# MundyRepo/MuNDy

Hardware: AMD Instinct MI355X
Metric: timesteps/sec, 10^6 spherocylinders, frictionless LCP contact (BBPGD) (higher is better)
Workload: dtype f64; 1 GPU; configs[2]: 1M spherocylinders r=0.5 L=2 at 40% volume fraction, random packing, AABB+0.1 neighbour list, frictionless LCP tol 1e-05; bodies_per_gpu=1000000, bodies_total=1000000, contacts_per_gpu=7621833, contacts_total=7621833, parallelism=single GPU (N > 1: the same system, hilbert domain decomposition with RCCL halo)

## Files before the change

include/mundy_hip.h:

```cpp
#ifndef MUNDY_HIP_H_
#define MUNDY_HIP_H_

#include <stddef.h>
#include <stdint.h>

#ifdef __cplusplus
extern "C" {
#endif

typedef void* mhip_stream_t;

enum {
  MHIP_SUCCESS = 0,
  MHIP_ERR_INVALID_ARGUMENT = 1,
  MHIP_ERR_LOGIC = 2,
  MHIP_ERR_RUNTIME = 3,
  MHIP_ERR_HIP = 4,
  MHIP_ERR_NO_DEVICE = 5
};

const char* mhip_last_error(void);
int mhip_version(void);
int mhip_set_tracing(int enable);
int mhip_device_info(int* device_count, char* arch_name, size_t arch_name_len);
// ... 105 lines not shown
                                mhip_stream_t stream);
int mhip_crosslinkers_renumber(mhip_crosslinkers_t handle, const int32_t* new_of_old, mhip_stream_t stream);
int mhip_crosslinkers_destroy(mhip_crosslinkers_t handle);

#define MHIP_PERIPHERY_SPHERE 0
#define MHIP_PERIPHERY_ELLIPSOID 1
#define MHIP_PERIPHERY_ELLIPSOID_FAST 2
typedef struct mhip_periphery {
  int shape;
  double center[3];
  double quat[4];
  double radii[3];
  double k;
} mhip_periphery;
int mhip_periphery_force(const mhip_periphery* periphery, size_t n, const double* center, const double* radius,
                         double* force, int accumulate, int* colliding ,
                         double* max_overlap , mhip_stream_t stream);

typedef struct mhip_active_springs* mhip_active_springs_t;
int mhip_active_springs_create(mhip_active_springs_t* handle, size_t n, size_t m, const int32_t* pairs ,
                               double sigma, double kon, double koff, const uint64_t* keys ,
                               const uint64_t* counters , mhip_stream_t stream);
int mhip_active_springs_sample(mhip_active_springs_t handle, int* switches , mhip_stream_t stream);
int mhip_active_springs_force(mhip_active_springs_t handle, const double* center, double* force, int accumulate,
                              int* active , mhip_stream_t stream);
int mhip_active_springs_advance(mhip_active_springs_t handle, double dt, mhip_stream_t stream);
int mhip_active_springs_get_state(mhip_active_springs_t handle, int32_t* state, double* next_time, double* elapsed,
                                  uint64_t* counters, mhip_stream_t stream);
int mhip_active_springs_set_state(mhip_active_springs_t handle, const int32_t* state, const double* next_time,
                                  const double* elapsed, const uint64_t* counters, mhip_stream_t stream);
int mhip_active_springs_renumber(mhip_active_springs_t handle, const int32_t* new_of_old, mhip_stream_t stream);
int mhip_active_springs_destroy(mhip_active_springs_t handle);

int mhip_compute_aabb_mixed(size_t n, const int32_t* kind, const double* center, const double* quat,
                            const double* shape, double* aabb, double* bounding_radius, mhip_stream_t stream);
int mhip_compute_aabb_mixed_conservative(size_t n, const int32_t* kind, const double* center, const double* quat,
                                         const double* shape, double* aabb, double* bounding_radius,
                                         mhip_stream_t stream);
int mhip_contact_mixed(size_t c, const int32_t* pairs, const int32_t* kind, const double* center, const double* quat,
                       const double* shape, double* sep, double* normal, double* cp1, double* cp2, double* ra,
                       double* rb, size_t* class_counts , mhip_stream_t stream);
int mhip_contact_mixed_set_contraction(int on);
int mhip_contact_mixed_set_sphere_ellipsoid_route(int route);
int mhip_contact_mixed_last_evaluations(unsigned long long evaluations[3] , mhip_stream_t stream);
int mhip_ellipsoid_last_evaluations(unsigned long long* evaluations , mhip_stream_t stream);
int mhip_contact_mixed_periodic(size_t c, const int32_t* pairs, const int32_t* kind, const double* center,
                                const double* quat, const double* shape, const double* box , double* sep,
                                double* normal, double* cp1, double* cp2, double* ra, double* rb,
                                size_t* class_counts , mhip_stream_t stream);

enum { MHIP_SEARCH_SPHERES = 0, MHIP_SEARCH_AABB = 1 };
enum { MHIP_SEARCH_METHOD_AUTO = 0, MHIP_SEARCH_METHOD_GRID = 1, MHIP_SEARCH_METHOD_MORTON_LBVH = 2 };

typedef struct mhip_broadphase* mhip_broadphase_t;

typedef struct {
  int search_kind;
  int symmetric;
  double buffer;
  int periodic;
  double box[3];
  int method;
  int include_self;
  double cell[9];
} mhip_broadphase_config;

int mhip_broadphase_create(mhip_broadphase_t* handle);
int mhip_broadphase_destroy(mhip_broadphase_t handle);
int mhip_broadphase_build(mhip_broadphase_t handle, const mhip_broadphase_config* config , size_t n,
                          const double* aabb, const double* center, const double* bounding_radius,
                          size_t* num_pairs , mhip_stream_t stream);
int mhip_broadphase_get_pairs(mhip_broadphase_t handle, int32_t* pairs, int32_t* row_ptr, int32_t* col,
                              mhip_stream_t stream);
int mhip_broadphase_set_sets(mhip_broadphase_t handle, size_t n, const unsigned char* is_source,
                             const unsigned char* is_target, mhip_stream_t stream);
int mhip_broadphase_set_exclusions(mhip_broadphase_t handle, size_t n, const int32_t* ex_ptr, const int32_t* ex_idx,
                                   size_t num_entries, mhip_stream_t stream);
int mhip_broadphase_set_identities(mhip_broadphase_t handle, size_t n, const uint64_t* entity_id,
                                   const int32_t* owner_rank, mhip_stream_t stream);
int mhip_broadphase_get_ident_pairs(mhip_broadphase_t handle, uint64_t* source_id, int32_t* source_proc,
                                    uint64_t* target_id, int32_t* target_proc, mhip_stream_t stream);
int mhip_broadphase_method_used(mhip_broadphase_t handle, int* method );
int mhip_broadphase_minimum_image_complete(mhip_broadphase_t handle, int* complete );
int mhip_links_export_coo(mhip_broadphase_t handle, uint64_t first_link_id, int source_rank, int target_rank,
                          uint64_t* link_id, uint64_t* linked_entity_ids, unsigned char* linked_entity_ranks,
                          mhip_stream_t stream);
int mhip_links_export_crs(mhip_broadphase_t handle, uint64_t first_link_id, unsigned bucket_capacity,
                          unsigned* num_connected_links, unsigned* sparse_connectivity_offsets,
                          uint64_t* sparse_connectivity, uint64_t* bucket_begin, mhip_stream_t stream);
int mhip_broadphase_needs_rebuild(mhip_broadphase_t handle, size_t n, const double* center, int* flag ,
                                  mhip_stream_t stream);

enum { MHIP_SPACE_UNCONSTRAINED = 0, MHIP_SPACE_LOWER_BOUND = 1, MHIP_SPACE_UPPER_BOUND = 2, MHIP_SPACE_BOUNDED = 3 };
enum { MHIP_RESIDUAL_PROJECTED_DIFF = 0, MHIP_RESIDUAL_PROJECTED_GRADIENT = 1 };

typedef struct {
  int kind;
  double lower_bound, upper_bound;
} mhip_space;

typedef struct {
  unsigned max_iters;
  double tol;
  int residual_kind;
} mhip_pgd_config;

typedef struct {
  unsigned num_iters;
  double residual;
  int converged;
} mhip_solve_result;

int mhip_deep_copy(size_t n, double* dst, const double* src, mhip_stream_t stream);
int mhip_fill(size_t n, double* dst, double value, mhip_stream_t stream);
int mhip_axpby(size_t n, double alpha, const double* x, double beta, double* y, mhip_stream_t stream);
int mhip_wrapped_axpbyz(size_t n, double alpha, const double* x, double beta, const double* y, double* z,
                        const mhip_space* space , mhip_stream_t stream);
int mhip_diff_dot2(size_t n, const double* x, const double* y, double* result , mhip_stream_t stream);
int mhip_diff_dot4(size_t n, const double* x1, const double* x2, const double* y1, const double* y2,
                   double* result , mhip_stream_t stream);
int mhip_residual(size_t n, int residual_kind, const double* x, const double* grad, const mhip_space* space ,
                  double* result , mhip_stream_t stream);
int mhip_bb_step(size_t n, const double* x_old, const double* g_old, const double* x, const double* g,
                 double* result , mhip_stream_t stream);
int mhip_gemv(size_t n, const double* A, const double* x, double* y, mhip_stream_t stream);

typedef struct mhip_contact_op* mhip_contact_op_t;

int mhip_contact_op_create(mhip_contact_op_t* handle, size_t num_constraints, size_t num_bodies, const int32_t* pairs,
                           const double* normal, const double* ra, const double* rb, const double* mob_trans,
                           const double* mob_rot, double dt, const double* priority, mhip_stream_t stream);
int mhip_contact_op_create_rods(mhip_contact_op_t* handle, size_t num_constraints, size_t num_bodies,
                                const int32_t* pairs, const double* normal, const double* arc_s, const double* arc_t,
                                const double* seg, const double* mob_trans, const double* mob_rot, double dt,
                                const double* priority, mhip_stream_t stream);
int mhip_contact_op_refresh(mhip_contact_op_t handle, const double* normal, const double* ra, const double* rb,
                            mhip_stream_t stream);
int mhip_contact_op_refresh_rods(mhip_contact_op_t handle, const double* normal, const double* arc_s,
                                 const double* arc_t, const double* seg, mhip_stream_t stream);
int mhip_contact_op_destroy(mhip_contact_op_t handle);
int mhip_release_cached_workspaces(void);
int mhip_contact_op_apply(mhip_contact_op_t handle, const double* x, double* y, mhip_stream_t stream);
int mhip_contact_op_body_sweep(mhip_contact_op_t handle, const double* x, mhip_stream_t stream);
int mhip_contact_op_body_sweep_vector(mhip_contact_op_t handle, const double* force, mhip_stream_t stream);
int mhip_contact_op_constraint_rate(mhip_contact_op_t handle, const double* velocity, double* sep_dot,
                                    mhip_stream_t stream);
int mhip_contact_op_sizes(mhip_contact_op_t handle, size_t* num_constraints, size_t* num_bodies);
int mhip_contact_op_set_work_mapping(mhip_contact_op_t handle, int xcd_tile, int lanes_per_body);
int mhip_contact_op_set_drift_source(mhip_contact_op_t op, int source);
int mhip_contact_op_get_drift_source(mhip_contact_op_t op, int* source );
int mhip_contact_op_set_tiering(mhip_contact_op_t handle, int mode);
int mhip_contact_op_tier_stats(mhip_contact_op_t handle, size_t* tiered_iterations, double* mean_hot_fraction,
                               size_t* renumberings, size_t* wakeups);
int mhip_contact_op_set_profiling(mhip_contact_op_t handle, int enable);
int mhip_contact_op_get_profile(mhip_contact_op_t handle, double* body_ms, double* constraint_ms, size_t* iterations);
int mhip_contact_op_body_velocity(mhip_contact_op_t handle, const double** velocity );

int mhip_bbpgd_solve_dense(size_t n, const double* A, const double* q, const mhip_space* space ,
                           const mhip_pgd_config* config , double* x, double* g, double* x_tmp,
                           double* g_tmp, mhip_solve_result* result , mhip_stream_t stream);
int mhip_bbpgd_solve_contact(mhip_contact_op_t op, const double* q, const mhip_space* space ,
                             const mhip_pgd_config* config , double* x, double* g, double* x_tmp,
                             double* g_tmp, mhip_solve_result* result , mhip_stream_t stream);

int mhip_bbpgd_solve_contact_friction(mhip_contact_op_t op, const double* sep, double mu,
                                      const mhip_pgd_config* config , double* p, double* g,
                                      mhip_solve_result* result , mhip_stream_t stream);
int mhip_apgd_solve_contact_friction(mhip_contact_op_t op, const double* sep, double mu,
                                      const mhip_pgd_config* config , double* p, double* g,
                                      mhip_solve_result* result , mhip_stream_t stream);
#define MHIP_BBPGD_REDUCTION_WIDTH 5
int mhip_contact_op_set_partition(mhip_contact_op_t handle, size_t body_first, size_t body_count,
                                  const unsigned char* counted_contacts, double* velocity);
int mhip_bbpgd_stage_begin(mhip_contact_op_t op, const double* q, const mhip_space* space ,
                           const mhip_pgd_config* config , double* x, double* g, double* x_tmp,
                           double* g_tmp, mhip_stream_t stream);
int mhip_bbpgd_stage_body(mhip_contact_op_t op, int init, mhip_stream_t stream);
int mhip_bbpgd_stage_constraint(mhip_contact_op_t op, int init, double* local, mhip_stream_t stream);
int mhip_bbpgd_stage_constraint_range(mhip_contact_op_t op, int init, size_t c_first, size_t c_count,
                                      mhip_stream_t stream);
int mhip_bbpgd_stage_reduce(mhip_contact_op_t op, int init, double* local, mhip_stream_t stream);
int mhip_bbpgd_stage_finalize(mhip_contact_op_t op, int init, const double* gathered, int nparts,
                              mhip_stream_t stream);
int mhip_bbpgd_stage_poll(mhip_contact_op_t op, mhip_solve_result* result , int* done ,
                          mhip_stream_t stream);
int mhip_bbpgd_stage_snapshot_active(mhip_contact_op_t op, mhip_stream_t stream);
int mhip_bbpgd_stage_end(mhip_contact_op_t op, mhip_solve_result* result , mhip_stream_t stream);
int mhip_solve_small_cqpp_batch(size_t batch, int n, const double* A, const double* q,
                                const mhip_space* space , const mhip_pgd_config* config ,
                                double* x, double* grad, unsigned* num_iters, double* residual, int* converged,
                                mhip_stream_t stream);
int mhip_scrap_bbpgd_solve_contact(mhip_contact_op_t op, const double* sep, double max_allowable_overlap,
                                   unsigned max_iterations, double* lam, double* lam_tmp, double* g, double* g_tmp,
                                   mhip_solve_result* result , double* max_speed ,
                                   mhip_stream_t stream);
int mhip_bbpgd_solve_contact_unfused(mhip_contact_op_t op, const double* q, const mhip_space* space ,
                                     const mhip_pgd_config* config , double* x, double* g, double* x_tmp,
                                     double* g_tmp, mhip_solve_result* result , mhip_stream_t stream);

int mhip_select_contacts(size_t c, const double* sep, double cutoff, int32_t* kept_index, size_t* count_out ,
                         mhip_stream_t stream);
int mhip_filter_pairs_owned(size_t c, const int32_t* pairs_in, size_t first, size_t count, int32_t* pairs_out,
                            unsigned char* counted_out, size_t* count_out , mhip_stream_t stream);
int mhip_partition_pairs_owned(size_t c, const int32_t* pairs_in, size_t first, size_t count, int32_t* pairs_out,
                               unsigned char* counted_out, size_t* interior_out ,
                               size_t* count_out , mhip_stream_t stream);
int mhip_select_aabb_overlap(size_t n, const double* aabb, double buffer, const double* box6 ,
                             int32_t* idx_out, size_t* count_out , mhip_stream_t stream);
int mhip_aabb_chunk_bounds(size_t n, const double* aabb, double buffer, int nchunks, double* boxes,
                           mhip_stream_t stream);
int mhip_select_aabb_overlap_any(size_t n, const double* aabb, double buffer, int nboxes, const double* boxes,
                                 int32_t* idx_out, size_t* count_out , mhip_stream_t stream);
int mhip_aabb_bounds(size_t n, const double* aabb, double buffer, double* out6 , mhip_stream_t stream);

int mhip_integrate_euler(size_t n, double dt, const double* velocity, double* center, double* quat,
                         mhip_stream_t stream);

int mhip_periodic_sep(size_t n, const double* box, const double* p1, const double* p2, double* out,
                      mhip_stream_t stream);
int mhip_wrap_rigid(size_t n, const double* box, double* center, mhip_stream_t stream);

int mhip_unit_cell_inverse(const double* cell, double* cell_inv);
int mhip_periodic_sep_triclinic(size_t n, const double* cell, const double* p1, const double* p2, double* out,
                                mhip_stream_t stream);
int mhip_wrap_rigid_triclinic(size_t n, const double* cell, double* center, mhip_stream_t stream);
int mhip_shift_image_triclinic(size_t n, const double* cell, const double* p, const int32_t* images, double* out,
                               mhip_stream_t stream);
int mhip_contact_spheres_triclinic(size_t c, const int32_t* pairs, const double* center, const double* radius,
                                   const double* cell, double* sep, double* normal, mhip_stream_t stream);

int mhip_morton_order(size_t n, const double* center, const double* lo , double cell_size, int32_t* perm,
                      mhip_stream_t stream);
int mhip_curve_order(size_t n, const double* center, const double* lo , const double* hi ,
                     int level, const int32_t* key_table, int32_t* perm, mhip_stream_t stream);
int mhip_curve_keys(size_t n, const double* center, const double* lo , const double* hi ,
                    int level, const int32_t* key_table, uint32_t* keys, mhip_stream_t stream);
int mhip_sort_by_key_u64(size_t n, const uint64_t* keys, int32_t* perm, mhip_stream_t stream);
int mhip_gather_rows(size_t n, size_t width, const int32_t* perm, const double* src, double* dst, mhip_stream_t stream);
int mhip_copy_strided(size_t n, size_t width, const double* src, size_t src_stride, double* dst, size_t dst_stride,
                      mhip_stream_t stream);


typedef struct mhip_comm* mhip_comm_t;
#define MHIP_COMM_ID_BYTES 128
typedef int (*mhip_comm_exchange_fn)(void* user, int nsend, const int* send_peer, const double* const* send_buf,
                                     const size_t* send_count, int nrecv, const int* recv_peer, double* const* recv_buf,
                                     const size_t* recv_count);
typedef int (*mhip_comm_all_gather_fn)(void* user, const double* send, size_t count, double* recv );

int mhip_comm_unique_id(unsigned char* id );
int mhip_comm_create_rccl(mhip_comm_t* comm, const unsigned char* id , int rank, int world);
int mhip_comm_create_host(mhip_comm_t* comm, int rank, int world, mhip_comm_exchange_fn exchange,
                          mhip_comm_all_gather_fn all_gather, void* user);
int mhip_comm_destroy(mhip_comm_t comm);
int mhip_comm_info(mhip_comm_t comm, int* rank, int* world, int* is_rccl);
int mhip_comm_mailbox_open(mhip_comm_t comm, int* opened , mhip_stream_t stream);
int mhip_comm_mailbox_close(mhip_comm_t comm);
int mhip_comm_halo_ipc_enable(mhip_comm_t comm, int on);
int mhip_comm_set_exchange_timeout(mhip_comm_t comm, double seconds);
int mhip_comm_inject_fault(mhip_comm_t comm, unsigned at_poll);
int mhip_comm_halo_ipc_active(mhip_comm_t comm, int* active );
int mhip_comm_all_gather(mhip_comm_t comm, const double* send, size_t count, double* recv, mhip_stream_t stream);
int mhip_comm_exchange_start(mhip_comm_t comm, int nsend, const int* send_peer, const double* const* send_buf,
                             const size_t* send_count, int nrecv, const int* recv_peer, double* const* recv_buf,
                             const size_t* recv_count, mhip_stream_t stream);
int mhip_comm_exchange_finish(mhip_comm_t comm, mhip_stream_t stream);

typedef struct mhip_velocity_halo {
  double* velocity;
  int num_send_peers;
  const int* send_peer;
  const size_t* send_rows;
  const int32_t* send_index;
  int num_recv_peers;
  const int* recv_peer;
  const size_t* recv_first_row;
  const size_t* recv_rows;
} mhip_velocity_halo;
typedef struct mhip_ghost_layout {
  size_t num_ghost_lo, num_owned, num_ghost_hi;
  size_t num_sent;
  mhip_velocity_halo halo;
} mhip_ghost_layout;
int mhip_ghost_layout_from_counts(int world, int rank, size_t n_owned, const size_t* counts ,
                                  size_t* num_ghost_lo, size_t* num_ghost_hi, int* num_send, int* send_peer,
                                  size_t* send_rows, int* num_recv, int* recv_peer, size_t* recv_first_row,
                                  size_t* recv_rows);
int mhip_ghost_plan(mhip_comm_t comm, size_t n, const double* aabb, double buffer,
                    mhip_ghost_layout* layout , mhip_stream_t stream);
int mhip_ghost_exchange(mhip_comm_t comm, size_t width, const double* records ,
                        double* local , mhip_stream_t stream);

int mhip_hilbert_key_table(int level, int32_t* table );
int mhip_body_work_weights(size_t c, const int32_t* pairs, size_t first, size_t count, double* weights ,
                           mhip_stream_t stream);
int mhip_compose_keys_u64(size_t n, const uint32_t* major, const double* minor, int shift, uint64_t* out,
                          mhip_stream_t stream);
int mhip_fill_sequence(size_t n, double first, double* dst, mhip_stream_t stream);
int mhip_curve_cut(mhip_comm_t comm, size_t n, const uint32_t* keys, const double* weights , size_t ncell,
                   int64_t* splitters , mhip_stream_t stream);
int mhip_migrate_plan(mhip_comm_t comm, size_t n, const uint32_t* keys, const int64_t* splitters ,
                      size_t* n_new, size_t* num_sent , size_t* num_received ,
                      mhip_stream_t stream);
int mhip_migrate_exchange(mhip_comm_t comm, size_t width, const double* records ,
                          double* out , mhip_stream_t stream);
typedef struct mhip_dist_profile {
// ... 20 lines not shown
```

mundy_amd/capi.py:

```python
import ctypes as C
import os

_HERE = os.path.dirname(os.path.abspath(__file__))
LIB_PATH = os.path.join(_HERE, "lib", "libmundy_hip.so")

SUCCESS, ERR_INVALID_ARGUMENT, ERR_LOGIC, ERR_RUNTIME, ERR_HIP, ERR_NO_DEVICE = range(6)
SEARCH_SPHERES, SEARCH_AABB = 0, 1
SEARCH_METHOD_AUTO, SEARCH_METHOD_GRID, SEARCH_METHOD_MORTON_LBVH = 0, 1, 2
SPACE_UNCONSTRAINED, SPACE_LOWER_BOUND, SPACE_UPPER_BOUND, SPACE_BOUNDED = 0, 1, 2, 3
RESIDUAL_PROJECTED_DIFF, RESIDUAL_PROJECTED_GRADIENT = 0, 1
SPRING_HOOKEAN, SPRING_FENE = 0, 1
PERIPHERY_SPHERE, PERIPHERY_ELLIPSOID, PERIPHERY_ELLIPSOID_FAST = 0, 1, 2


class MhipError(RuntimeError):
    """HIP runtime failure or missing device (MHIP_ERR_HIP / MHIP_ERR_NO_DEVICE)."""


class BroadphaseConfig(C.Structure):
    _fields_ = [("search_kind", C.c_int), ("symmetric", C.c_int), ("buffer", C.c_double), ("periodic", C.c_int),
                ("box", C.c_double * 3), ("method", C.c_int), ("include_self", C.c_int), ("cell", C.c_double * 9)]


class Space(C.Structure):
    _fields_ = [("kind", C.c_int), ("lower_bound", C.c_double), ("upper_bound", C.c_double)]


class PgdConfig(C.Structure):
    _fields_ = [("max_iters", C.c_uint), ("tol", C.c_double), ("residual_kind", C.c_int)]


class SolveResult(C.Structure):
    _fields_ = [("num_iters", C.c_uint), ("residual", C.c_double), ("converged", C.c_int)]


class HertzFrictionParams(C.Structure):
    _fields_ = [("mu", C.c_double), ("normal_damping", C.c_double), ("tangential_damping", C.c_double),
                ("density", C.c_double), ("dt", C.c_double)]


class Periphery(C.Structure):
    _fields_ = [("shape", C.c_int), ("center", C.c_double * 3), ("quat", C.c_double * 4), ("radii", C.c_double * 3),
                ("k", C.c_double)]


class VelocityHalo(C.Structure):
    _fields_ = [("velocity", C.c_void_p), ("num_send_peers", C.c_int), ("send_peer", C.POINTER(C.c_int)),
                ("send_rows", C.POINTER(C.c_size_t)), ("send_index", C.c_void_p), ("num_recv_peers", C.c_int),
                ("recv_peer", C.POINTER(C.c_int)), ("recv_first_row", C.POINTER(C.c_size_t)),
                ("recv_rows", C.POINTER(C.c_size_t))]


class GhostLayout(C.Structure):
    _fields_ = [("num_ghost_lo", C.c_size_t), ("num_owned", C.c_size_t), ("num_ghost_hi", C.c_size_t),
                ("num_sent", C.c_size_t), ("halo", VelocityHalo)]


class DistProfile(C.Structure):
    _fields_ = [("body_ms", C.c_double), ("constraint_ms", C.c_double), ("halo_wait_ms", C.c_double),
                ("timed_iterations", C.c_size_t), ("halo_post_ms", C.c_double), ("record_ms", C.c_double),
                ("halo_path", C.c_int), ("record_path", C.c_int)]


EXCHANGE_FN = C.CFUNCTYPE(C.c_int, C.c_void_p, C.c_int, C.POINTER(C.c_int), C.POINTER(C.c_void_p),
                          C.POINTER(C.c_size_t), C.c_int, C.POINTER(C.c_int), C.POINTER(C.c_void_p),
                          C.POINTER(C.c_size_t))
ALL_GATHER_FN = C.CFUNCTYPE(C.c_int, C.c_void_p, C.c_void_p, C.c_size_t, C.c_void_p)
COMM_ID_BYTES = 128

_vp, _sz, _d, _i = C.c_void_p, C.c_size_t, C.c_double, C.c_int

SIGNATURES = {
    "mhip_device_info": [C.POINTER(C.c_int), C.c_char_p, _sz],
    "mhip_malloc": [C.POINTER(_vp), _sz],
    "mhip_free": [_vp],
    "mhip_memcpy_h2d": [_vp, _vp, _sz, _vp],
    "mhip_memcpy_d2h": [_vp, _vp, _sz, _vp],
    "mhip_stream_synchronize": [_vp],
    "mhip_compute_aabb_spheres": [_sz, _vp, _vp, _vp, _vp],
    "mhip_compute_aabb_spherocylinders": [_sz, _vp, _vp, _vp, _vp, _vp, _vp],
    "mhip_compute_aabb_ellipsoids": [_sz, _vp, _vp, _vp, _vp, _vp],
    "mhip_compute_aabb_ellipsoids_conservative": [_sz, _vp, _vp, _vp, _vp, _vp],
    "mhip_compute_aabb_segments": [_sz, _vp, _vp, _vp],
    "mhip_bounding_radius_spherocylinders": [_sz, _vp, _vp, _vp, _vp],
    "mhip_bounding_radius_ellipsoids": [_sz, _vp, _vp, _vp],
    "mhip_spherocylinder_segments": [_sz, _vp, _vp, _vp, _vp, _vp, _vp],
    "mhip_distance_sphere_sphere": [_sz, _vp, _vp, _vp, _vp, _vp, _vp, _vp],
    "mhip_distance_point_segment": [_sz, _vp, _vp, _vp, _vp, _vp, _vp, _vp, _vp],
    "mhip_distance_point_sphere": [_sz, _vp, _vp, _vp, _vp, _vp, _vp],
    "mhip_distance_segment_sphere": [_sz] + [_vp] * 9,
    "mhip_distance_segment_segment": [_sz, _vp, _vp, _vp, _vp, _vp, _vp, _vp, _vp, _vp, _vp, _vp],
    "mhip_distance_ellipsoid_ellipsoid": [_sz] + [_vp] * 12,
    "mhip_distance_point_ellipsoid": [_sz] + [_vp] * 8,
    "mhip_contact_ellipsoids": [_sz] + [_vp] * 11,
    "mhip_compute_aabb_mixed": [_sz] + [_vp] * 7,
    "mhip_compute_aabb_mixed_conservative": [_sz] + [_vp] * 7,
    "mhip_contact_mixed": [_sz] + [_vp] * 11 + [C.POINTER(_sz), _vp],
    "mhip_contact_mixed_set_contraction": [_i],
    "mhip_contact_mixed_set_sphere_ellipsoid_route": [_i],
    "mhip_contact_mixed_last_evaluations": [C.POINTER(C.c_ulonglong), _vp],
    "mhip_ellipsoid_last_evaluations": [C.POINTER(C.c_ulonglong), _vp],
    "mhip_contact_mixed_periodic": [_sz] + [_vp] * 5 + [C.POINTER(_d)] + [_vp] * 6 + [C.POINTER(_sz), _vp],
    "mhip_contact_spherocylinders_periodic": [_sz, _vp, _vp, _vp, C.POINTER(_d)] + [_vp] * 9,
    "mhip_hertz_contact_force": [_sz, _sz, _vp, _vp, _vp, _vp, _d, _vp, _d, _vp, _vp, _vp],
    "mhip_hertz_friction_force": [_sz, _sz] + [_vp] * 8 + [_d, _vp, _d, _vp, C.POINTER(HertzFrictionParams), _vp, _vp, _vp,
                                  _vp],
    "mhip_contact_history_carry": [_sz, _vp, _vp, _vp, _sz, _sz, _vp, _vp, C.POINTER(_sz), _vp],
    "mhip_select_dividing": [_sz, _vp, _d, _vp, C.POINTER(_sz), _vp],
    "mhip_divide_grow_spherocylinders": [_sz, _sz, _vp, _d, _d, C.POINTER(_d), _vp, _vp, _vp, _vp, _vp],
    "mhip_aabb_moved": [_sz, _vp, _vp, _d, C.POINTER(_i), _vp],
    "mhip_springs_create": [C.POINTER(_vp), _sz, _sz, _vp, _i, _vp, _d, _vp, _d, _vp],
    "mhip_springs_force": [_vp, _vp, _vp, _vp, _vp, _vp],
    "mhip_springs_destroy": [_vp],
    "mhip_crosslinkers_create": [C.POINTER(_vp), _sz, _sz, _vp, _vp, _vp, _i, _d, _d, _d, _d, _d, _d, _vp],
    "mhip_crosslinkers_set_candidates": [_vp, _vp, _vp, _sz, _vp, _vp],
    "mhip_crosslinkers_kmc_step": [_vp, _vp, _d, _vp, _vp, _vp, _vp, _vp],
    "mhip_crosslinkers_force": [_vp, _vp, _vp, _i, _vp, _vp, _vp],
    "mhip_crosslinkers_get_state": [_vp, _vp, _vp, _vp],
    "mhip_crosslinkers_set_state": [_vp, _vp, _vp, _vp],
    "mhip_crosslinkers_renumber": [_vp, _vp, _vp],
    "mhip_crosslinkers_destroy": [_vp],
    "mhip_periphery_force": [C.POINTER(Periphery), _sz, _vp, _vp, _vp, _i, _vp, _vp, _vp],
    "mhip_active_springs_create": [C.POINTER(_vp), _sz, _sz, _vp, _d, _d, _d, _vp, _vp, _vp],
    "mhip_active_springs_sample": [_vp, _vp, _vp],
    "mhip_active_springs_force": [_vp, _vp, _vp, _i, _vp, _vp],
    "mhip_active_springs_advance": [_vp, _d, _vp],
    "mhip_active_springs_get_state": [_vp, _vp, _vp, _vp, _vp, _vp],
    "mhip_active_springs_set_state": [_vp, _vp, _vp, _vp, _vp, _vp],
    "mhip_active_springs_renumber": [_vp, _vp, _vp],
    "mhip_active_springs_destroy": [_vp],
    "mhip_philox4x32_10": [_sz, _vp, _vp, C.c_uint32, _vp, _vp],
    "mhip_brownian_velocity": [_sz, _vp, _vp, _d, _d, _vp, _vp, _vp],
    "mhip_drag_velocity": [_sz, _vp, _vp, _vp, _vp],
    "mhip_contact_spheres": [_sz, _vp, _vp, _vp, C.POINTER(_d), _vp, _vp, _vp],
    "mhip_contact_spherocylinders": [_sz, _vp, _vp, _vp, _vp, _vp, _vp, _vp, _vp, _vp, _vp, _vp, _vp],
    "mhip_broadphase_create": [C.POINTER(_vp)],
    "mhip_broadphase_destroy": [_vp],
    "mhip_broadphase_build": [_vp, C.POINTER(BroadphaseConfig), _sz, _vp, _vp, _vp, C.POINTER(_sz), _vp],
    "mhip_broadphase_get_pairs": [_vp, _vp, _vp, _vp, _vp],
    "mhip_broadphase_needs_rebuild": [_vp, _sz, _vp, C.POINTER(_i), _vp],
    "mhip_select_contacts": [_sz, _vp, _d, _vp, C.POINTER(_sz), _vp],
    "mhip_curve_keys": [_sz, _vp, C.POINTER(_d), C.POINTER(_d), _i, _vp, _vp, _vp],
    "mhip_sort_by_key_u64": [_sz, _vp, _vp, _vp],
    "mhip_broadphase_set_sets": [_vp, _sz, _vp, _vp, _vp],
    "mhip_broadphase_set_exclusions": [_vp, _sz, _vp, _vp, _sz, _vp],
    "mhip_broadphase_set_identities": [_vp, _sz, _vp, _vp, _vp],
    "mhip_broadphase_get_ident_pairs": [_vp, _vp, _vp, _vp, _vp, _vp],
    "mhip_broadphase_method_used": [_vp, C.POINTER(_i)],
    "mhip_broadphase_minimum_image_complete": [_vp, C.POINTER(_i)],
    "mhip_links_export_coo": [_vp, C.c_uint64, _i, _i, _vp, _vp, _vp, _vp],
    "mhip_links_export_crs": [_vp, C.c_uint64, C.c_uint, _vp, _vp, _vp, _vp, _vp],
    "mhip_deep_copy": [_sz, _vp, _vp, _vp],
    "mhip_fill": [_sz, _vp, _d, _vp],
    "mhip_axpby": [_sz, _d, _vp, _d, _vp, _vp],
    "mhip_wrapped_axpbyz": [_sz, _d, _vp, _d, _vp, _vp, C.POINTER(Space), _vp],
    "mhip_diff_dot2": [_sz, _vp, _vp, C.POINTER(_d), _vp],
    "mhip_diff_dot4": [_sz, _vp, _vp, _vp, _vp, C.POINTER(_d), _vp],
    "mhip_residual": [_sz, _i, _vp, _vp, C.POINTER(Space), C.POINTER(_d), _vp],
    "mhip_bb_step": [_sz, _vp, _vp, _vp, _vp, C.POINTER(_d), _vp],
    "mhip_gemv": [_sz, _vp, _vp, _vp, _vp],
    "mhip_contact_op_create": [C.POINTER(_vp), _sz, _sz, _vp, _vp, _vp, _vp, _vp, _vp, _d, _vp, _vp],
    "mhip_contact_op_create_rods": [C.POINTER(_vp), _sz, _sz, _vp, _vp, _vp, _vp, _vp, _vp, _vp, _d, _vp, _vp],
    "mhip_contact_op_refresh": [_vp, _vp, _vp, _vp, _vp],
    "mhip_contact_op_refresh_rods": [_vp, _vp, _vp, _vp, _vp, _vp],
    "mhip_contact_op_destroy": [_vp],
    "mhip_contact_op_apply": [_vp, _vp, _vp, _vp],
    "mhip_contact_op_body_sweep": [_vp, _vp, _vp],
    "mhip_contact_op_body_sweep_vector": [_vp, _vp, _vp],
    "mhip_contact_op_constraint_rate": [_vp, _vp, _vp, _vp],
    "mhip_contact_op_body_velocity": [_vp, C.POINTER(_vp)],
    "mhip_contact_op_set_profiling": [_vp, _i],
    "mhip_contact_op_set_tiering": [_vp, _i],
    "mhip_contact_op_tier_stats": [_vp, C.POINTER(_sz), C.POINTER(_d), C.POINTER(_sz), C.POINTER(_sz)],
    "mhip_contact_op_set_work_mapping": [_vp, _i, _i],
    "mhip_bbpgd_stage_snapshot_active": [_vp, _vp],
    "mhip_contact_op_get_profile": [_vp, C.POINTER(_d), C.POINTER(_d), C.POINTER(_sz)],
    "mhip_bbpgd_solve_dense": [_sz, _vp, _vp, C.POINTER(Space), C.POINTER(PgdConfig), _vp, _vp, _vp, _vp,
                               C.POINTER(SolveResult), _vp],
    "mhip_bbpgd_solve_contact": [_vp, _vp, C.POINTER(Space), C.POINTER(PgdConfig), _vp, _vp, _vp, _vp,
                                 C.POINTER(SolveResult), _vp],
    "mhip_bbpgd_solve_contact_friction": [_vp, _vp, _d, C.POINTER(PgdConfig), _vp, _vp, C.POINTER(SolveResult), _vp],
    "mhip_apgd_solve_contact_friction": [_vp, _vp, _d, C.POINTER(PgdConfig), _vp, _vp, C.POINTER(SolveResult), _vp],
    "mhip_solve_small_cqpp_batch": [_sz, _i, _vp, _vp, C.POINTER(Space), C.POINTER(PgdConfig), _vp, _vp, _vp, _vp,
                                    _vp, _vp],
    "mhip_scrap_bbpgd_solve_contact": [_vp, _vp, _d, C.c_uint, _vp, _vp, _vp, _vp, C.POINTER(SolveResult),
                                       C.POINTER(_d), _vp],
    "mhip_contact_op_set_partition": [_vp, _sz, _sz, _vp, _vp],
    "mhip_bbpgd_stage_begin": [_vp, _vp, C.POINTER(Space), C.POINTER(PgdConfig), _vp, _vp, _vp, _vp, _vp],
    "mhip_bbpgd_stage_body": [_vp, _i, _vp],
    "mhip_bbpgd_stage_constraint": [_vp, _i, _vp, _vp],
    "mhip_bbpgd_stage_constraint_range": [_vp, _i, _sz, _sz, _vp],
    "mhip_bbpgd_stage_reduce": [_vp, _i, _vp, _vp],
    "mhip_bbpgd_stage_finalize": [_vp, _i, _vp, _i, _vp],
    "mhip_bbpgd_stage_poll": [_vp, C.POINTER(SolveResult), C.POINTER(_i), _vp],
    "mhip_bbpgd_stage_end": [_vp, C.POINTER(SolveResult), _vp],
    "mhip_filter_pairs_owned": [_sz, _vp, _sz, _sz, _vp, _vp, C.POINTER(_sz), _vp],
    "mhip_partition_pairs_owned": [_sz, _vp, _sz, _sz, _vp, _vp, C.POINTER(_sz), C.POINTER(_sz), _vp],
    "mhip_select_aabb_overlap": [_sz, _vp, _d, C.POINTER(_d), _vp, C.POINTER(_sz), _vp],
    "mhip_aabb_chunk_bounds": [_sz, _vp, _d, _i, _vp, _vp],
    "mhip_select_aabb_overlap_any": [_sz, _vp, _d, _i, _vp, _vp, C.POINTER(_sz), _vp],
    "mhip_aabb_bounds": [_sz, _vp, _d, C.POINTER(_d), _vp],
    "mhip_bbpgd_solve_contact_unfused": [_vp, _vp, C.POINTER(Space), C.POINTER(PgdConfig), _vp, _vp, _vp, _vp,
                                         C.POINTER(SolveResult), _vp],
    "mhip_periodic_sep": [_sz, C.POINTER(_d), _vp, _vp, _vp, _vp],
    "mhip_wrap_rigid": [_sz, C.POINTER(_d), _vp, _vp],
    "mhip_unit_cell_inverse": [C.POINTER(_d), C.POINTER(_d)],
    "mhip_periodic_sep_triclinic": [_sz, C.POINTER(_d), _vp, _vp, _vp, _vp],
    "mhip_wrap_rigid_triclinic": [_sz, C.POINTER(_d), _vp, _vp],
    "mhip_shift_image_triclinic": [_sz, C.POINTER(_d), _vp, _vp, _vp, _vp],
    "mhip_contact_spheres_triclinic": [_sz, _vp, _vp, _vp, C.POINTER(_d), _vp, _vp, _vp],
    "mhip_integrate_euler": [_sz, _d, _vp, _vp, _vp, _vp],
    "mhip_morton_order": [_sz, _vp, C.POINTER(_d), _d, _vp, _vp],
    "mhip_set_tracing": [_i],
    "mhip_curve_order": [_sz, _vp, C.POINTER(_d), C.POINTER(_d), _i, _vp, _vp, _vp],
    "mhip_gather_rows": [_sz, _sz, _vp, _vp, _vp, _vp],
    "mhip_copy_strided": [_sz, _sz, _vp, _sz, _vp, _sz, _vp],
    "mhip_contact_op_sizes": [_vp, C.POINTER(_sz), C.POINTER(_sz)],
    "mhip_contact_op_set_drift_source": [_vp, _i],
    "mhip_contact_op_get_drift_source": [_vp, C.POINTER(_i)],
    "mhip_comm_unique_id": [C.c_char_p],
    "mhip_comm_create_rccl": [C.POINTER(_vp), C.c_char_p, _i, _i],
    "mhip_comm_create_host": [C.POINTER(_vp), _i, _i, EXCHANGE_FN, ALL_GATHER_FN, _vp],
    "mhip_comm_destroy": [_vp],
    "mhip_comm_info": [_vp, C.POINTER(_i), C.POINTER(_i), C.POINTER(_i)],
    "mhip_comm_mailbox_open": [_vp, C.POINTER(_i), _vp],
    "mhip_comm_mailbox_close": [_vp],
    "mhip_comm_halo_ipc_enable": [_vp, _i],
    "mhip_comm_set_exchange_timeout": [_vp, C.c_double],
    "mhip_comm_inject_fault": [_vp, C.c_uint],
    "mhip_comm_halo_ipc_active": [_vp, C.POINTER(_i)],
    "mhip_comm_all_gather": [_vp, _vp, _sz, _vp, _vp],
    "mhip_comm_exchange_start": [_vp, _i, C.POINTER(_i), C.POINTER(_vp), C.POINTER(_sz), _i, C.POINTER(_i),
                                 C.POINTER(_vp), C.POINTER(_sz), _vp],
    "mhip_comm_exchange_finish": [_vp, _vp],
    "mhip_ghost_layout_from_counts": [_i, _i, _sz, C.POINTER(_sz), C.POINTER(_sz), C.POINTER(_sz), C.POINTER(_i),
                                      C.POINTER(_i), C.POINTER(_sz), C.POINTER(_i), C.POINTER(_i), C.POINTER(_sz),
                                      C.POINTER(_sz)],
    "mhip_ghost_plan": [_vp, _sz, _vp, _d, C.POINTER(GhostLayout), _vp],
    "mhip_ghost_exchange": [_vp, _sz, _vp, _vp, _vp],
    "mhip_hilbert_key_table": [_i, _vp],
    "mhip_body_work_weights": [_sz, _vp, _sz, _sz, _vp, _vp],
    "mhip_compose_keys_u64": [_sz, _vp, _vp, _i, _vp, _vp],
    "mhip_fill_sequence": [_sz, _d, _vp, _vp],
    "mhip_curve_cut": [_vp, _sz, _vp, _vp, _sz, _vp, _vp],
    "mhip_migrate_plan": [_vp, _sz, _vp, _vp, C.POINTER(_sz), C.POINTER(_sz), C.POINTER(_sz), _vp],
    "mhip_migrate_exchange": [_vp, _sz, _vp, _vp, _vp],
    "mhip_bbpgd_solve_contact_distributed": [_vp, _vp, C.POINTER(VelocityHalo), _sz, _vp, C.POINTER(Space),
                                             C.POINTER(PgdConfig), _vp, _vp, _vp, _vp, C.c_uint,
                                             C.POINTER(SolveResult), C.POINTER(DistProfile), _vp],
}
OTHER_SYMBOLS = {"mhip_last_error": ([], C.c_char_p), "mhip_version": ([], C.c_int),
                 "mhip_release_cached_workspaces": ([], C.c_int)}

_lib = None


def load():
    global _lib
    if _lib is None:
        if not os.path.exists(LIB_PATH):
            raise MhipError("%s is missing: run `python -m mundy_amd.build` (or __graft_entry__.build()); "
                            "mundy_amd has no CPU fallback" % LIB_PATH)
        import torch
        lib = C.CDLL(LIB_PATH)
        for name, argtypes in SIGNATURES.items():
            fn = getattr(lib, name)
            fn.argtypes = argtypes
            fn.restype = C.c_int
        for name, (argtypes, restype) in OTHER_SYMBOLS.items():
            fn = getattr(lib, name)
            fn.argtypes = argtypes
            fn.restype = restype
        _lib = lib
    return _lib


def check(status):
    if status == SUCCESS:
        return
    msg = load().mhip_last_error().decode()
    if status == ERR_INVALID_ARGUMENT:
        raise ValueError(msg)
    if status == ERR_LOGIC:
        raise AssertionError(msg)
    if status == ERR_RUNTIME:
        raise RuntimeError(msg)
    raise MhipError(msg)
```

mundy_amd/csrc/convex.hip:

```cpp
#include <cstdlib>
#include <mutex>
#include <type_traits>
#include <vector>

#include "mhip_internal.hpp"

namespace mhip {

constexpr unsigned kProfileStride = 8;
constexpr double kSmallStep = 1e-6;
constexpr double kBBEps = 1e-15 * 10;
constexpr double kLowest = -1.7976931348623157e308;

#ifndef MHIP_STREAM_UNROLL
#define MHIP_STREAM_UNROLL 4
#endif
#ifndef MHIP_STREAM_GRID
#define MHIP_STREAM_GRID 1048576
#endif
constexpr int kStreamUnroll = MHIP_STREAM_UNROLL;
__device__ inline size_t stream_first() { return blockIdx.x * (size_t)(kBlock * kStreamUnroll) + threadIdx.x; }
template <int MODE>
__device__ inline double axpby_value(double alpha, double x, double beta, double y) {
  if (MODE == 0) return alpha * x + beta * y;
// ... 666 lines not shown
                const double2 a2 = pl2[slot];
                dd_add(Tdd, V3{a1.y, a2.x, a2.y});
              }
              if (KIN == KIN_ROD) dd_add(Tdd, a1.y * f);
            }
          }
          __syncthreads();
        }
      } else {
        for (int32_t k0 = ab + sub; k0 < ae; k0 += G * U) {
          int32_t kc[U];
#pragma unroll
          for (int u = 0; u < U; ++u) kc[u] = (k0 + u * G < ae) ? k0 + u * G : -1;
          process(op.aent, op.arec, kc, true);
        }
      }
    }
    const int32_t head = (end - beg < 64) ? end - beg : 64;
    unsigned long long mm = kEarlySnap ? mask_early : op.body_mask[b];
    if (head < 64) mm &= (1ull << head) - 1ull;
    if (op.aptr != nullptr) mm &= ~(kEarlySnap ? snap_early : op.snap_mask[b]);
    if (FLAT && !has_body) mm = 0ull;
    int32_t kk[U];
#pragma unroll
    for (int u = 0; u < U; ++u) kk[u] = -1;
    int rank = 0, nm = 0;
    while (mm) {
      const int bit = __ffsll(static_cast<long long>(mm)) - 1;
      mm &= mm - 1ull;
      if ((rank++ & (G - 1)) != sub) continue;
#pragma unroll
      for (int u = 0; u < U; ++u)
        if (nm == u) kk[u] = beg + bit;
      if (++nm == U) {
        process(op.inc, op.half, kk, true);
        nm = 0;
#pragma unroll
        for (int u = 0; u < U; ++u) kk[u] = -1;
      }
    }
    if (nm) process(op.inc, op.half, kk, true);
    full_from = beg + head;
  }
  if (FLAT && !has_body) return;
  for (int32_t k0 = full_from + sub; k0 < end; k0 += G * U) {
    int32_t kk[U];
#pragma unroll
    for (int u = 0; u < U; ++u) kk[u] = (k0 + u * G < end) ? k0 + u * G : -1;
    process(op.inc, op.half, kk, false);
  }
#pragma unroll
  for (int off = G / 2; off > 0; off >>= 1) {
    dd_add(Fdd.x, dd_shfl_xor(Fdd.x, off));
    dd_add(Fdd.y, dd_shfl_xor(Fdd.y, off));
    dd_add(Fdd.z, dd_shfl_xor(Fdd.z, off));
    if (KIN != KIN_TRANS) {
      dd_add(Tdd.x, dd_shfl_xor(Tdd.x, off));
      dd_add(Tdd.y, dd_shfl_xor(Tdd.y, off));
      dd_add(Tdd.z, dd_shfl_xor(Tdd.z, off));
    }
  }
  if (track_regs) {
#pragma unroll
    for (int off = G / 2; off > 0; off >>= 1) {
      dF = dF + V3{__shfl_xor(dF.x, off, 64), __shfl_xor(dF.y, off, 64), __shfl_xor(dF.z, off, 64)};
      if (KIN != KIN_TRANS) dS = dS + V3{__shfl_xor(dS.x, off, 64), __shfl_xor(dS.y, off, 64), __shfl_xor(dS.z, off, 64)};
    }
  }
  if (sub != 0) return;
  if (track_rows && !kEarlyTail) {
    const double* vel_old = op.vel_alt ? ((vel_new == op.vel) ? op.vel_alt : op.vel) : op.vel;
    const double2* vo = reinterpret_cast<const double2*>(vel_old + 6 * b);
    o0 = vo[0];
    o1 = vo[1];
    o2 = vo[2];
  }
  const V3 F = dd_value(Fdd), T = dd_value(Tdd);
  double2* v = reinterpret_cast<double2*>(vel_new + 6 * b);
  V3 W{0.0, 0.0, 0.0};
  if (KIN == KIN_RIGID) W = V3{mr * T.x, mr * T.y, mr * T.z};
  if (KIN == KIN_ROD) {
    const V3 tq = cross(axis, T);
    const V3 w{mr * tq.x, mr * tq.y, mr * tq.z};
    if (!(MODE == X_SOLVE && PACKED)) store3(op.omega, b, w);
    W = cross(w, axis);
  }
  const V3 Ub{mt * F.x, mt * F.y, mt * F.z};
  v[0] = make_double2(Ub.x, Ub.y);
  v[1] = make_double2(Ub.z, W.x);
  v[2] = make_double2(W.y, W.z);
  if (track) {
    double d;
    if constexpr (track_regs) {
      d = mt * (fabs(dF.x) + fabs(dF.y) + fabs(dF.z));
      if (KIN == KIN_ROD) {
        const V3 tq = cross(axis, dS);
        const V3 dZ = cross(V3{mr * tq.x, mr * tq.y, mr * tq.z}, axis);
        d += 0.5 * (fabs(dZ.x) + fabs(dZ.y) + fabs(dZ.z));
      }
      if (KIN == KIN_RIGID) d += op.arm_max[b] * mr * (fabs(dS.x) + fabs(dS.y) + fabs(dS.z));
    } else {
      d = fabs(Ub.x - o0.x) + fabs(Ub.y - o0.y) + fabs(Ub.z - o1.x);
      const double dw = fabs(W.x - o1.y) + fabs(W.y - o2.x) + fabs(W.z - o2.y);
      if (KIN == KIN_ROD) d += 0.5 * dw;
      if (KIN == KIN_RIGID) d += op.arm_max[b] * dw;
    }
    const double D = (kEarlyTail ? drift_old : op.drift[b]) + op.dt * d;
    op.drift[b] = D;
    if (op.fire_at != nullptr && !(D < (kEarlyTail ? fire_thr : op.fire_at[b])))
      op.fired[atomicAdd(&op.tier_counters[1], 1ull)] = static_cast<int32_t>(b);
  }
}

constexpr int kRed = MHIP_BBPGD_REDUCTION_WIDTH;
static_assert(kRed == 5, "record layout: max, num.hi, num.lo, den.hi, den.lo");
__device__ inline void store_partial(double* __restrict__ p, size_t stride, size_t slot, double rmax, DD num, DD den) {
  p[slot] = rmax;
  p[stride + slot] = num.hi;
  p[2 * stride + slot] = num.lo;
  p[3 * stride + slot] = den.hi;
  p[4 * stride + slot] = den.lo;
}

template <int KIN>
__device__ inline double contact_dt_sdot(const OpView& op, const double* __restrict__ vel, size_t c, int2 ij) {
  const V3 n = load3(op.normal, c);
  const double2* vi2 = reinterpret_cast<const double2*>(vel + 6 * (size_t)ij.x);
  const double2* vj2 = reinterpret_cast<const double2*>(vel + 6 * (size_t)ij.y);
  const double2 a0 = vi2[0], a1 = vi2[1], b0 = vj2[0], b1 = vj2[1];
  V3 vi{a0.x, a0.y, a1.x}, vj{b0.x, b0.y, b1.x};
  if (KIN == KIN_RIGID) {
    const double2 a2 = vi2[2], b2 = vj2[2];
    vi = vi + cross(V3{a1.y, a2.x, a2.y}, load3(op.ra, c));
    vj = vj + cross(V3{b1.y, b2.x, b2.y}, load3(op.rb, c));
  }
  if (KIN == KIN_ROD) {
    const double2 a2 = vi2[2], b2 = vj2[2];
    const double ci = rod_arm_coef(op.arc_s[c]), cj = rod_arm_coef(op.arc_t[c]);
    vi = vi + ci * V3{a1.y, a2.x, a2.y};
    vj = vj + cj * V3{b1.y, b2.x, b2.y};
  }
  const double sdot = -n.x * (vi.x - vj.x) - n.y * (vi.y - vj.y) - n.z * (vi.z - vj.z);
  return op.dt * sdot;
}

struct TierCheck {
  size_t H, I;
  double* wake;
  int32_t* list;
  unsigned long long* counters;
  const int32_t* fired;
  double* fire_at;
  unsigned blocks;
};

template <int KIN>
__device__ __forceinline__ void tier_evaluate(const OpView& op, const double* __restrict__ vel,
                                              const double* __restrict__ xt, double* __restrict__ xn,
                                              const double* __restrict__ q, const Space& sp, double step,
                                              bool step_is_zero, int resid_kind, size_t c, double& rmax, DD& num,
                                              DD& den) {
  const int2 ij = op.pairs[c];
  double x_old = 0.0, g_old = 0.0;
  const double xc = iterate_x<X_SOLVE, true>(c, xt, nullptr, step, step_is_zero, sp, &x_old, &g_old);
  const double y = contact_dt_sdot<KIN>(op, vel, c, ij);
  const double g = 1.0 * q[c] + 1.0 * y;
  reinterpret_cast<double2*>(xn)[c] = make_double2(xc, g);
  if (op.body_mask != nullptr && sp.kind == MHIP_SPACE_LOWER_BOUND && sp.lo == 0.0) {
    const bool was = !(x_old == 0.0 && g_old >= 0.0 && g_old <= 1.7976931348623157e308);
    const bool now = !(xc == 0.0 && g >= 0.0 && g <= 1.7976931348623157e308);
    if (was != now) {
      const unsigned pi = op.pos[2 * c], pj = op.pos[2 * c + 1];
      if (pi < 64u) atomicXor(&op.body_mask[ij.x], 1ull << pi);
      if (pj < 64u) atomicXor(&op.body_mask[ij.y], 1ull << pj);
    }
  }
  if (op.counted == nullptr || op.counted[c]) {
    const double r = residual_term(resid_kind, xc, g, sp);
    if (r > rmax) rmax = r;
    const double dx = xc - x_old;
    dd_add(num, dx * dx);
    dd_add(den, dx * (g - g_old));
  }
}

constexpr int kTierRoundClaims = 8;
constexpr int kTierQueue = kTierRoundClaims * kBlock;
template <int KIN>
__device__ __forceinline__ void tier_service(const OpView& op, const SolverState* __restrict__ st, double* __restrict__ X0,
                                             double* __restrict__ X1, const double* __restrict__ q, const Space& sp,
                                             int resid_kind, double* __restrict__ partials, const TierCheck& tc,
                                             unsigned block, size_t slot, double* scratch, int32_t* queue,
                                             unsigned* queued) {
  if (st->done) return;
  const double* xt = X0;
  double* xn = X1;
  if (st->flips & 1u) {
    xt = X1; xn = X0;
  }
  const double step = st->step;
  const double* vel = op.vel;
  if (op.vel_alt && !(st->flips & 1u)) vel = op.vel_alt;
  const bool step_is_zero = fabs(-step) < kZeroTol;
  double rmax = 0.0;
  DD num{0.0, 0.0}, den{0.0, 0.0};
  const size_t awake = static_cast<size_t>(tc.counters[2]);
  const size_t share = (awake + tc.blocks - 1) / tc.blocks;
  const size_t old_lo = block * share < awake ? block * share : awake;
  unsigned n_old = static_cast<unsigned>((old_lo + share < awake ? old_lo + share : awake) - old_lo);
  const size_t count = static_cast<size_t>(tc.counters[1]);
  const double ninf = -__builtin_huge_val();
  size_t f0 = block * (size_t)blockDim.x;
  for (;;) {
    const bool have = f0 + threadIdx.x < count;
    const size_t b = have ? static_cast<size_t>(tc.fired[f0 + threadIdx.x]) : 0;
    const double D = have ? op.drift[b] : 0.0;
    int32_t k = have ? op.inc_ptr[b] : 0;
    const int32_t kend = have ? op.inc_ptr[b + 1] : 0;
    double left = __builtin_huge_val();
    do {
      if (threadIdx.x == 0) *queued = 0u;
      __syncthreads();
      for (int claims = 0; k < kend && claims < kTierRoundClaims; ++k) {
        const int32_t e = op.inc[k];
        const size_t c = static_cast<size_t>(e >> 1);
        if (c < tc.H || c >= tc.I) continue;
        double* thr = tc.wake + 2 * (c - tc.H);
        const double mine = thr[e & 1];
        if (!(thr[0] > ninf)) continue;
        if (D < mine) {
          if (mine < left) left = mine;
          continue;
        }
        const unsigned long long old = atomicExch(reinterpret_cast<unsigned long long*>(thr),
                                                  static_cast<unsigned long long>(__double_as_longlong(ninf)));
        if (__longlong_as_double(static_cast<long long>(old)) > ninf) {
          thr[1] = ninf;
          tc.list[atomicAdd(&tc.counters[0], 1ull)] = static_cast<int32_t>(c);
          queue[atomicAdd(queued, 1u)] = static_cast<int32_t>(c);
          ++claims;
        }
      }
      __syncthreads();
      const unsigned total = n_old + *queued;
      for (unsigned i = threadIdx.x; i < total; i += blockDim.x) {
        const int32_t c = i < n_old ? tc.list[old_lo + i] : queue[i - n_old];
        tier_evaluate<KIN>(op, vel, xt, xn, q, sp, step, step_is_zero, resid_kind, static_cast<size_t>(c), rmax, num,
                           den);
      }
      n_old = 0;
    } while (__syncthreads_or(k < kend));
    if (have) tc.fire_at[b] = left;
    f0 += (size_t)tc.blocks * blockDim.x;
    if (f0 >= count) break;
  }
  const double m = block_max(rmax, scratch);
  const DD s1 = block_sum(num, scratch);
  const DD s2 = block_sum(den, scratch);
  if (threadIdx.x == 0) store_partial(partials, op.part_stride, slot, m, s1, s2);
}

template <int MODE, int KIN, bool PACKED>
__global__ void __launch_bounds__(kBlock, (KIN == KIN_RIGID ? 6 : 7))
    k_constraint(OpView op, const SolverState* __restrict__ st, double* __restrict__ X0, double* __restrict__ X1,
                 double* __restrict__ G0, double* __restrict__ G1, const double* __restrict__ q, Space sp,
                 int resid_kind, double* __restrict__ partials, TierCheck check = TierCheck{}) {
  __shared__ double scratch[2 * kBlock / 64];
  const unsigned nblk = gridDim.x - check.blocks;
  if (blockIdx.x < check.blocks) {
    if (MODE == X_SOLVE && PACKED) {
      __shared__ int32_t queue[kTierQueue];
      __shared__ unsigned queued;
      tier_service<KIN>(op, st, X0, X1, q, sp, resid_kind, partials, check, blockIdx.x,
                        op.part_offset + nblk + blockIdx.x, scratch, queue, &queued);
    }
    return;
  }
  const unsigned bid = blockIdx.x - check.blocks;
  const double* xt = X0;
  const double* gt = G0;
  double* xn = X1;
  double* gn = G1;
  double step = 0.0;
  if (MODE == X_SOLVE) {
    if (st->done) return;
    if (st->flips & 1u) {
      xt = X1; gt = G1; xn = X0; gn = G0;
    }
    step = st->step;
  }
  if (MODE == X_INIT) gn = G0;
  if (MODE == X_INIT && PACKED) {
    xt = G0;
    xn = X0;
  }
  const double* vel = op.vel;
  if (MODE == X_SOLVE && op.vel_alt && !(st->flips & 1u)) vel = op.vel_alt;
  const bool step_is_zero = fabs(-step) < kZeroTol;
  double rmax = kLowest;
  DD num{0.0, 0.0}, den{0.0, 0.0};
  const size_t ntiles = (op.c_end - op.c_first + kBlock - 1) / kBlock;
  for (size_t lin = bid; lin < ntiles; lin += nblk) {
    const size_t c = op.c_first + xcd_tile(lin, ntiles, op.xcd_aware) * kBlock + threadIdx.x;
    if (c >= op.c_end) continue;
    constexpr bool NTC = (MHIP_NT & 2) != 0 && MODE == X_SOLVE && PACKED;
    const int2 ij = ld_s<NTC>(op.pairs + c);
    const double2 pold = iterate_load<MODE, PACKED, NTC>(c, xt, gt);
    const V3 n = ld_s3<NTC>(op.normal, c);
    double arc_i = 0.0, arc_j = 0.0;
    V3 arm_i{0.0, 0.0, 0.0}, arm_j{0.0, 0.0, 0.0};
    if (KIN == KIN_ROD) {
      arc_i = ld_s<NTC>(op.arc_s + c);
      arc_j = ld_s<NTC>(op.arc_t + c);
    }
    if (KIN == KIN_RIGID) {
      arm_i = ld_s3<NTC>(op.ra, c);
      arm_j = ld_s3<NTC>(op.rb, c);
    }
    const double qc = (MODE != X_APPLY) ? ld_s<NTC>(q + c) : 0.0;
    const double2* vi2 = reinterpret_cast<const double2*>(vel + 6 * (size_t)ij.x);
    const double2* vj2 = reinterpret_cast<const double2*>(vel + 6 * (size_t)ij.y);
    const double2 a0 = vi2[0], a1 = vi2[1], b0 = vj2[0], b1 = vj2[1];
    double2 a2 = make_double2(0.0, 0.0), b2 = make_double2(0.0, 0.0);
    if (KIN != KIN_TRANS) {
      a2 = vi2[2];
      b2 = vj2[2];
    }
    const double x_old = (MODE == X_SOLVE) ? pold.x : 0.0, g_old = (MODE == X_SOLVE) ? pold.y : 0.0;
    const double xc = iterate_value<MODE>(pold, step, step_is_zero, sp);
    V3 vi{a0.x, a0.y, a1.x}, vj{b0.x, b0.y, b1.x};
    if (KIN == KIN_RIGID) {
      vi = vi + cross(V3{a1.y, a2.x, a2.y}, arm_i);
      vj = vj + cross(V3{b1.y, b2.x, b2.y}, arm_j);
    }
    if (KIN == KIN_ROD) {
      const double ci = rod_arm_coef(arc_i), cj = rod_arm_coef(arc_j);
      vi = vi + ci * V3{a1.y, a2.x, a2.y};
      vj = vj + cj * V3{b1.y, b2.x, b2.y};
    }
    const double sdot = -n.x * (vi.x - vj.x) - n.y * (vi.y - vj.y) - n.z * (vi.z - vj.z);
    const double y = op.dt * sdot;
    if (MODE == X_APPLY) {
      gn[c] = y;
    } else {
      const double g = 1.0 * qc + 1.0 * y;
      if (PACKED) {
        reinterpret_cast<double2*>(xn)[c] = make_double2(xc, g);
        if (op.body_mask != nullptr && sp.kind == MHIP_SPACE_LOWER_BOUND && sp.lo == 0.0) {
          const bool was = (MODE == X_INIT) ? false : !(x_old == 0.0 && g_old >= 0.0 && g_old <= 1.7976931348623157e308);
          const bool now = !(xc == 0.0 && g >= 0.0 && g <= 1.7976931348623157e308);
          if (was != now) {
            const unsigned pi = op.pos[2 * c], pj = op.pos[2 * c + 1];
            if (pi < 64u) atomicXor(&op.body_mask[ij.x], 1ull << pi);
            if (pj < 64u) atomicXor(&op.body_mask[ij.y], 1ull << pj);
          }
        }
      } else {
        gn[c] = g;
        if (MODE == X_SOLVE) xn[c] = xc;
      }
      if (op.counted == nullptr || op.counted[c]) {
        const double r = residual_term(resid_kind, xc, g, sp);
        if (r > rmax) rmax = r;
        if (MODE == X_SOLVE) {
          const double dx = xc - x_old;
          dd_add(num, dx * dx);
          dd_add(den, dx * (g - g_old));
        }
      }
    }
  }
  if (MODE != X_APPLY) {
    const double m = block_max(rmax, scratch);
    const DD s1 = block_sum(num, scratch);
    const DD s2 = block_sum(den, scratch);
    if (threadIdx.x == 0) {
      const size_t stride = op.part_stride ? op.part_stride : nblk;
      store_partial(partials, stride, op.part_offset + bid, m, s1, s2);
    }
  }
}

constexpr int kFinalBlock = 1024;
__device__ inline void reduce_records(int nparts, const double* __restrict__ partials, size_t si, size_t sk,
                                      double* scratch, double& rmax, DD& num, DD& den) {
  rmax = kLowest;
  num = DD{0.0, 0.0};
  den = DD{0.0, 0.0};
  for (int i = threadIdx.x; i < nparts; i += blockDim.x) {
    const double* r = partials + i * si;
    if (r[0] > rmax) rmax = r[0];
    dd_add(num, DD{r[sk], r[2 * sk]});
    dd_add(den, DD{r[3 * sk], r[4 * sk]});
  }
  rmax = block_max(rmax, scratch);
  num = block_sum(num, scratch);
  den = block_sum(den, scratch);
}

constexpr int kFoldGroups = 64;
__global__ void __launch_bounds__(kBlock) k_fold_partials(int nparts, size_t stride,
                                                         const double* __restrict__ partials,
                                                         const SolverState* __restrict__ st, int check_done,
                                                         double* __restrict__ folded) {
  __shared__ double scratch[2 * kBlock / 64];
  if (check_done && st->done) return;
  const int per = (nparts + gridDim.x - 1) / gridDim.x;
  const int lo = blockIdx.x * per, hi = (lo + per < nparts) ? lo + per : nparts;
  double rmax;
  DD num, den;
  reduce_records(hi > lo ? hi - lo : 0, partials + lo, 1, stride, scratch, rmax, num, den);
  if (threadIdx.x == 0) store_partial(folded, gridDim.x, blockIdx.x, rmax, num, den);
}

template <int MODE>
__device__ inline void finalize_state(SolverState* __restrict__ st, double rmax, DD numdd, DD dendd, int resid_kind,
                                      double tol, unsigned max_iters, int tiered,
                                      unsigned long long* __restrict__ tier_counters);
template <int MODE>
__global__ void __launch_bounds__(kFinalBlock) k_finalize(int nparts, const double* __restrict__ partials, size_t si,
                                                         size_t sk, SolverState* __restrict__ st, int resid_kind,
                                                         double tol, unsigned max_iters, int tiered = 0,
                                                         unsigned long long* __restrict__ tier_counters = nullptr) {
  __shared__ double scratch[2 * kFinalBlock / 64];
  if (MODE == X_SOLVE && st->done) return;
  double rmax;
  DD numdd, dendd;
  reduce_records(nparts, partials, si, sk, scratch, rmax, numdd, dendd);
  if (threadIdx.x != 0) return;
  finalize_state<MODE>(st, rmax, numdd, dendd, resid_kind, tol, max_iters, tiered, tier_counters);
}
template <int MODE>
__device__ inline void finalize_state(SolverState* __restrict__ st, double rmax, DD numdd, DD dendd, int resid_kind,
                                      double tol, unsigned max_iters, int tiered,
                                      unsigned long long* __restrict__ tier_counters) {
  if (tier_counters) {
    tier_counters[1] = 0;
    tier_counters[2] = tier_counters[0];
  }
  const double num = dd_value(numdd);
  double den = dd_value(dendd);
  const double res = (resid_kind == MHIP_RESIDUAL_PROJECTED_DIFF) ? rmax / kSmallStep : rmax;
  st->residual = res;
  if (MODE == X_INIT) {
    st->step = 1.0 / res;
    st->iter = 0;
    st->flips = 0;
    st->converged = (res <= tol) ? 1 : 0;
    st->converged_at_init = st->converged;
    st->done = (st->converged || max_iters == 0) ? 1 : 0;
    st->num = 0.0;
    st->den = 0.0;
  } else {
    if (res <= tol) {
      st->converged = 1;
      st->done = 1;
      return;
    }
// ... 777 lines not shown
    if (c >= op.C) continue;
    const int2 ij = op.pairs[c];
    const V3 n = load3(op.normal, c);
    V3 y, gy, pk;
    const V3 p = apgd_iterate(B, a, c, n, mu, &y, &gy, &pk);
    const double2* vi2 = reinterpret_cast<const double2*>(op.vel + 6 * (size_t)ij.x);
    const double2* vj2 = reinterpret_cast<const double2*>(op.vel + 6 * (size_t)ij.y);
    const double2 a0 = vi2[0], a1 = vi2[1], a2 = vi2[2], b0 = vj2[0], b1 = vj2[1], b2 = vj2[2];
    const V3 vi = V3{a0.x, a0.y, a1.x} + cross(V3{a1.y, a2.x, a2.y}, load3(op.ra, c));
    const V3 vj = V3{b0.x, b0.y, b1.x} + cross(V3{b1.y, b2.x, b2.y}, load3(op.rb, c));
    const double q = sep[c];
    const V3 g{op.dt * (vj.x - vi.x) + q * n.x, op.dt * (vj.y - vi.y) + q * n.y, op.dt * (vj.z - vi.z) + q * n.z};
    store_pg(Pn, c, p, g);
    if (op.counted == nullptr || op.counted[c]) {
      const V3 w = project_cone(V3{p.x - kSmallStep * g.x, p.y - kSmallStep * g.y, p.z - kSmallStep * g.z}, n, mu);
      const double r = fmax(fabs(p.x - w.x), fmax(fabs(p.y - w.y), fabs(p.z - w.z)));
      if (r > rmax) rmax = r;
      const V3 d = p - y;
      dd_add(sa, dot(d, g - gy));
      dd_add(sb, dot(d, d));
      dd_add(sr, dot(gy, p - pk));
    }
  }
  const double m = block_max(rmax, scratch);
  const DD s1 = block_sum(sa, scratch);
  const DD s2 = block_sum(sb, scratch);
  const DD s3 = block_sum(sr, scratch);
  if (threadIdx.x == 0) {
    const size_t stride = gridDim.x, slot = blockIdx.x;
    partials[slot] = m;
    partials[stride + slot] = s1.hi;
    partials[2 * stride + slot] = s1.lo;
    partials[3 * stride + slot] = s2.hi;
    partials[4 * stride + slot] = s2.lo;
    partials[5 * stride + slot] = s3.hi;
    partials[6 * stride + slot] = s3.lo;
  }
}
__global__ void k_apgd_begin(const SolverState* __restrict__ st, ApgdState* __restrict__ as) {
  as->L = st->residual;
  if (!(as->L > 0.0)) as->L = 1.0;
  as->theta = 1.0;
  as->beta = 0.0;
  as->cur = 0;
  as->prev = 0;
  as->nxt = 1;
  as->rejected = 0;
}
__global__ void __launch_bounds__(kFinalBlock)
    k_apgd_finalize(int nparts, const double* __restrict__ partials, SolverState* __restrict__ st,
                    ApgdState* __restrict__ as, double tol, unsigned max_iters) {
  __shared__ double scratch[2 * kFinalBlock / 64];
  if (st->done) return;
  double rmax = kLowest;
  DD sa{0.0, 0.0}, sb{0.0, 0.0}, sr{0.0, 0.0};
  for (int i = threadIdx.x; i < nparts; i += blockDim.x) {
    if (partials[i] > rmax) rmax = partials[i];
    dd_add(sa, DD{partials[(size_t)nparts + i], partials[2 * (size_t)nparts + i]});
    dd_add(sb, DD{partials[3 * (size_t)nparts + i], partials[4 * (size_t)nparts + i]});
    dd_add(sr, DD{partials[5 * (size_t)nparts + i], partials[6 * (size_t)nparts + i]});
  }
  rmax = block_max(rmax, scratch);
  sa = block_sum(sa, scratch);
  sb = block_sum(sb, scratch);
  sr = block_sum(sr, scratch);
  if (threadIdx.x != 0) return;
  const double A = dd_value(sa), Bq = dd_value(sb), R = dd_value(sr);
  st->iter += 1;
  if (A > as->L * Bq) {
    as->L *= 2.0;
    as->rejected += 1;
    if (st->iter >= max_iters) st->done = 1;
    return;
  }
  const double res = rmax / kSmallStep;
  st->residual = res;
  st->step = 1.0 / as->L;
  const int accepted = as->nxt;
  if (res <= tol) {
    st->converged = 1;
    st->done = 1;
    as->cur = accepted;
    return;
  }
  const double th = as->theta;
  double th1 = (-(th * th) + th * sqrt(th * th + 4.0)) / 2.0;
  double beta = th * (1.0 - th) / (th * th + th1);
  if (R > 0.0) {
    beta = 0.0;
    th1 = 1.0;
  }
  as->theta = th1;
  as->beta = beta;
  as->L *= 0.9;
  const int old_cur = as->cur;
  as->prev = old_cur;
  as->cur = accepted;
  as->nxt = 3 - old_cur - accepted;
  st->flips += 1;
  if (st->iter >= max_iters) st->done = 1;
}
__global__ void __launch_bounds__(kBlock)
    k_finish_friction_apgd(size_t C, const SolverState* __restrict__ st, const ApgdState* __restrict__ as, ApgdBufs B,
                           double* __restrict__ p, double* __restrict__ g) {
  const double* cur = st->converged_at_init ? B.P[0] : B.P[as->cur];
  for (size_t c = blockIdx.x * (size_t)blockDim.x + threadIdx.x; c < C; c += (size_t)gridDim.x * blockDim.x) {
    const PG s = load_pg(cur, c);
    store3(p, c, s.p);
    store3(g, c, s.g);
  }
}

}

using namespace mhip;

struct mhip_contact_op {
  OpView view{};
  bool rot = false;
  int kin = KIN_TRANS;
  hipStream_t last_stream = nullptr;
  DeviceBuffer inc_ptr, inc, cursor, vel, partials, state, scanws, half, axis, omega, vel_out;
  DeviceBuffer iterate;
  DeviceBuffer rate_rows;
  DeviceBuffer body_mask, pos;
  DeviceBuffer sort_tmp, sort_list;
  DeviceBuffer aptr, aent, arec, snap_mask, acnt;
  int device = -1;
  int tiering = 1;
  int drift_source = 0;
  int lanes_per_body = 2;
  SolverState* host_state = nullptr;
  struct Stage {
    const double* q = nullptr;
    double *x = nullptr, *g = nullptr, *x_tmp = nullptr, *g_tmp = nullptr;
    Space sp{0, 0, 0};
    mhip_pgd_config cfg{0, 0, 0};
    bool active = false;
    unsigned part_used = 0;
    double *P0 = nullptr, *P1 = nullptr;
    const double* q_cur = nullptr;
    size_t interior = 0;
    bool interior_known = false, pause_on_bad_step = false;
    unsigned polls = 0, iter_at_poll = 0, snap_at = 0;
  } stage;
  struct Tier {
    bool active = false;
    bool tracking = false;
    bool disabled = false;
    unsigned polled_at = 0;
    double* saved_vel = nullptr;
    int set = 0;
    size_t H = 0;
    size_t I = 0;
    bool pingpong = false;
    DeviceBuffer geo[2], iter[2], misc, vel2, drift, arm, xprev;
    OpView saved{};
    size_t tiered_iterations = 0, retiers = 0, wakeups = 0;
    unsigned service_blocks = 32;
    double hot_sum = 0.0;
  } tier;
  bool profile = false;
  std::vector<hipEvent_t> events;
  double body_ms = 0.0, constraint_ms = 0.0;
  size_t timed_iterations = 0;
};

namespace {

template <int V> using Const = std::integral_constant<int, V>;
template <int V, int... Rest, class F>
void pick(int v, F&& f) {
  if constexpr (sizeof...(Rest) == 0) f(Const<V>{});
  else if (v == V) f(Const<V>{});
  else pick<Rest...>(v, f);
}
template <class F>
void with_kin(const mhip_contact_op* op, F&& f) { pick<KIN_ROD, KIN_RIGID, KIN_TRANS>(op->kin, f); }

constexpr size_t kRowDriftMaxBodies = 1750000;
static int op_drift_source(const mhip_contact_op* op) {
  if (op->kin == KIN_RIGID || op->lanes_per_body != 2) return 1;
  if (op->drift_source == 1 || op->drift_source == 2) return op->drift_source;
  return op->view.N > kRowDriftMaxBodies ? 2 : 1;
}
int op_launch_body(mhip_contact_op* op, int mode, const double* X0, const double* X1, const double* G0,
                   const double* G1, Space sp, hipStream_t s, bool packed = false) {
  if (op->view.N == 0) return MHIP_SUCCESS;
  const int G = (op->lanes_per_body == 1 || op->lanes_per_body == 2 || op->lanes_per_body == 8 || op->lanes_per_body == 16) ? op->lanes_per_body : 4;
  if (op->view.body_count == 0) return MHIP_SUCCESS;
  const unsigned grid = (grid_exact(op->view.body_count * (size_t)G) + 7u) & ~7u;
  op->last_stream = s;
  const SolverState* st = op->state.as<SolverState>();
  int flatp = MHIP_KBODY_FLAT;
  if (MHIP_KBODY_FLAT == 2 && packed && mode == X_SOLVE && op->view.aptr != nullptr) {
    const int32_t known = op->host_state ? *reinterpret_cast<const int32_t*>(op->host_state + 1) : 0;
    const double entries = known > 0 ? static_cast<double>(known) : 2.0 * static_cast<double>(op->view.C);
    const double per_group = entries / static_cast<double>(op->view.body_count) * (kBlock / (double)G);
    if (per_group > MHIP_KBODY_FLAT3_ABOVE * 2 * kBlock) flatp = 3;
  }
  const bool regs = op_drift_source(op) == 2;
  pick<X_APPLY, X_INIT, X_SOLVE>(mode, [&](auto m) { with_kin(op, [&](auto kin) { pick<1, 2, 8, 16, 4>(G, [&](auto g) {
    constexpr int M = decltype(m)::value, K = decltype(kin)::value, GG = decltype(g)::value;
    constexpr int UU = (GG == 4 || GG == 8) ? 4 : 2;
    auto launch = [&](auto pk, auto track, auto fp) {
      k_body<M, K, GG, UU, decltype(pk)::value, decltype(track)::value, decltype(fp)::value>
          <<<grid, kBlock, 0, s>>>(op->view, st, X0, X1, G0, G1, sp);
    };
    if constexpr (M == X_SOLVE) {
      if (packed) {
        pick<0, MHIP_KBODY_FLAT, 3>(op->view.aptr != nullptr ? flatp : 0, [&](auto fp) {
          if (op->view.drift == nullptr) return launch(std::true_type{}, Const<0>{}, fp);
          if constexpr (GG == 2 && K != KIN_RIGID) {
            if (regs) return launch(std::true_type{}, Const<2>{}, fp);
          }
          launch(std::true_type{}, Const<1>{}, fp);
        });
        return;
      }
    }
    launch(std::false_type{}, Const<0>{}, Const<0>{});
  }); }); });
  MHIP_LAUNCH_CHECK();
  return MHIP_SUCCESS;
}

int op_launch_constraint(mhip_contact_op* op, int mode, double* X0, double* X1, double* G0, double* G1,
                         const double* q, Space sp, int resid_kind, unsigned grid, hipStream_t s,
                         bool packed = false) {
  if (op->view.C == 0) return MHIP_SUCCESS;
  const SolverState* st = op->state.as<SolverState>();
  double* parts = op->partials.as<double>();
  pick<X_APPLY, X_INIT, X_SOLVE>(mode, [&](auto m) { with_kin(op, [&](auto kin) {
    constexpr int M = decltype(m)::value, K = decltype(kin)::value;
    auto launch = [&](auto pk) {
      k_constraint<M, K, decltype(pk)::value>
          <<<grid, kBlock, 0, s>>>(op->view, st, X0, X1, G0, G1, q, sp, resid_kind, parts);
    };
    if constexpr (M != X_APPLY) {
      if (packed) return launch(std::true_type{});
    }
    launch(std::false_type{});
  }); });
  MHIP_LAUNCH_CHECK();
  return MHIP_SUCCESS;
}

#ifndef MHIP_FOLD_ABOVE
#define MHIP_FOLD_ABOVE 4096
#endif
#ifndef MHIP_FOLD_BLOCK
#define MHIP_FOLD_BLOCK 128
#endif
inline void fold_partials(unsigned& nparts, size_t& stride, double*& parts, const SolverState* st, int check_done,
                          hipStream_t s) {
  if (nparts <= MHIP_FOLD_ABOVE) return;
  double* folded = parts + kRed * stride;
  k_fold_partials<<<kFoldGroups, kBlock, 0, s>>>((int)nparts, stride, parts, st, check_done, folded);
  parts = folded;
  nparts = kFoldGroups;
  stride = kFoldGroups;
}
inline unsigned final_block(size_t n) { return n <= 256 ? 64u : (n <= 2048 ? 256u : (unsigned)kFinalBlock); }
constexpr unsigned kStageStride = 2 * 32768;
constexpr int kMaxConstraintGrid = 32768;
unsigned constraint_grid(size_t C) {
  const size_t g = (C + kBlock - 1) / kBlock;
  return static_cast<unsigned>(g == 0 ? 1 : (g > (size_t)kMaxConstraintGrid ? kMaxConstraintGrid : g));
}

int op_snapshot_active(mhip_contact_op* op, hipStream_t s) {
  OpView& v = op->view;
  if (v.body_mask == nullptr || v.C == 0 || v.body_count == 0) return MHIP_SUCCESS;
  const size_t N = v.N, C = v.C, cnt = v.body_count;
  const int hw = (op->kin == KIN_RIGID) ? 6 : (op->kin == KIN_ROD ? 4 : 3);
  if (int e = op->aptr.reserve((N + 2) * sizeof(int32_t))) return e;
  if (int e = op->acnt.reserve((N + 2) * sizeof(int32_t))) return e;
  if (int e = op->aent.reserve((2 * C + 2) * sizeof(int32_t))) return e;
  if (int e = op->arec.reserve((2 * C + 2) * hw * sizeof(double))) return e;
  if (int e = op->snap_mask.reserve((N + 2) * sizeof(unsigned long long))) return e;
  int32_t* local = op->cursor.as<int32_t>();
  k_active_count<<<grid_for(cnt), kBlock, 0, s>>>(v.body_first, cnt, v.inc_ptr, v.body_mask, op->acnt.as<int32_t>());
  MHIP_LAUNCH_CHECK();
  if (int e = exclusive_scan_i32(op->acnt.as<int32_t>(), local, cnt, op->scanws.ptr, s)) return e;
  pick<6, 4, 3>(hw, [&](auto h) {
    k_active_fill_flat<decltype(h)::value><<<grid_exact(cnt), kBlock, 0, s>>>(
        v.body_first, cnt, v.inc_ptr, v.inc, v.half, v.body_mask, local, op->aptr.as<int32_t>(), op->aent.as<int32_t>(),
        op->arec.as<double>(), op->snap_mask.as<unsigned long long>());
  });
  MHIP_LAUNCH_CHECK();
  if (op->host_state != nullptr)
    MHIP_HIP(hipMemcpyAsync(reinterpret_cast<int32_t*>(op->host_state + 1), op->aptr.as<int32_t>() + v.body_first + cnt,
                            sizeof(int32_t), hipMemcpyDeviceToHost, s));
  v.aptr = op->aptr.as<int32_t>();
  v.aent = op->aent.as<int32_t>();
  v.arec = op->arec.as<double>();
  v.snap_mask = op->snap_mask.as<unsigned long long>();
  return MHIP_SUCCESS;
}
constexpr unsigned kSnapshotAfter = 8;

constexpr double kTierMinGap = 1e-9;
constexpr size_t kTierMinContacts = 1500000;
#ifndef MHIP_TIER_RETIER_PERCENT
#define MHIP_TIER_RETIER_PERCENT 4
#endif
constexpr unsigned kTierHorizon = 64;
#ifndef MHIP_TIER_SHARE
#define MHIP_TIER_SHARE 0.45
#endif
constexpr double kTierShare = MHIP_TIER_SHARE;
#ifndef MHIP_TIER_SERVICE_BLOCKS
#define MHIP_TIER_SERVICE_BLOCKS 32
#endif
constexpr unsigned kTierFireBlocks = MHIP_TIER_SERVICE_BLOCKS;

struct TierGeo {
  int2* pairs;
  double *normal, *arc_s, *arc_t, *q, *ra, *rb;
  int32_t* orig;
  unsigned char* pos;
};
inline size_t tier_align(size_t b) { return (b + 255) & ~static_cast<size_t>(255); }
inline size_t tier_geo_bytes(size_t C, bool arms) {
  return tier_align(C * 8) + tier_align(3 * C * 8) + 3 * tier_align(C * 8) + tier_align(C * 4) + tier_align(2 * C) +
         (arms ? 2 * tier_align(3 * C * 8) : 0) + 256;
}
inline TierGeo tier_geo_at(void* base, size_t C) {
  char* p = static_cast<char*>(base);
  TierGeo g;
  g.pairs = reinterpret_cast<int2*>(p); p += tier_align(C * 8);
  g.normal = reinterpret_cast<double*>(p); p += tier_align(3 * C * 8);
  g.arc_s = reinterpret_cast<double*>(p); p += tier_align(C * 8);
  g.arc_t = reinterpret_cast<double*>(p); p += tier_align(C * 8);
  g.q = reinterpret_cast<double*>(p); p += tier_align(C * 8);
  g.orig = reinterpret_cast<int32_t*>(p); p += tier_align(C * 4);
  g.pos = reinterpret_cast<unsigned char*>(p); p += tier_align(2 * C);
  g.ra = reinterpret_cast<double*>(p); p += tier_align(3 * C * 8);
  g.rb = reinterpret_cast<double*>(p);
  return g;
}
struct TierMisc {
  int32_t *flags, *rank, *new_of, *list, *fired;
  double* wake[2];
  double *budget, *drift_prev, *fire_at;
  unsigned long long* counters;
};
inline size_t tier_misc_bytes(size_t C, size_t N) {
  return 4 * tier_align((C + 2) * 4) + tier_align((N + 2) * 4) + 2 * tier_align((2 * C + 4) * 8) +
         3 * tier_align((N + 2) * 8) + 256;
}
inline TierMisc tier_misc_at(void* base, size_t C, size_t N) {
  char* p = static_cast<char*>(base);
  TierMisc m;
  m.flags = reinterpret_cast<int32_t*>(p); p += tier_align((C + 2) * 4);
  m.rank = reinterpret_cast<int32_t*>(p); p += tier_align((C + 2) * 4);
  m.new_of = reinterpret_cast<int32_t*>(p); p += tier_align((C + 2) * 4);
  m.list = reinterpret_cast<int32_t*>(p); p += tier_align((C + 2) * 4);
  m.fired = reinterpret_cast<int32_t*>(p); p += tier_align((N + 2) * 4);
  m.wake[0] = reinterpret_cast<double*>(p); p += tier_align((2 * C + 4) * 8);
  m.wake[1] = reinterpret_cast<double*>(p); p += tier_align((2 * C + 4) * 8);
  m.budget = reinterpret_cast<double*>(p); p += tier_align((N + 2) * 8);
  m.drift_prev = reinterpret_cast<double*>(p); p += tier_align((N + 2) * 8);
  m.fire_at = reinterpret_cast<double*>(p); p += tier_align((N + 2) * 8);
  m.counters = reinterpret_cast<unsigned long long*>(p);
  return m;
}

__global__ void __launch_bounds__(kBlock) k_tier_budget(size_t N, const double* __restrict__ drift,
                                                       double* __restrict__ drift_prev, double scale,
                                                       double* __restrict__ budget) {
  for (size_t b = blockIdx.x * (size_t)blockDim.x + threadIdx.x; b < N; b += (size_t)gridDim.x * blockDim.x) {
    const double d = drift[b];
    budget[b] = scale * (d - drift_prev[b]);
    drift_prev[b] = d;
  }
}
__global__ void __launch_bounds__(kBlock) k_tier_arm_max(size_t N, const int32_t* __restrict__ inc_ptr,
                                                        const double* __restrict__ half, double* __restrict__ arm_max) {
  for (size_t b = blockIdx.x * (size_t)blockDim.x + threadIdx.x; b < N; b += (size_t)gridDim.x * blockDim.x) {
    double m = 0.0;
    for (int32_t k = inc_ptr[b]; k < inc_ptr[b + 1]; ++k) {
      const double* H = half + static_cast<size_t>(k) * 6;
      const double r = sqrt(H[3] * H[3] + H[4] * H[4] + H[5] * H[5]);
      if (r > m) m = r;
    }
    arm_max[b] = m * (1.0 + 1e-12);
  }
}
__global__ void __launch_bounds__(kBlock)
    k_tier_classify(size_t C, const int2* __restrict__ pairs, const double2* __restrict__ Pcur,
                    const double2* __restrict__ Pprev, const double* __restrict__ budget,
                    const double* __restrict__ drift, const double* __restrict__ wake_old, size_t H_old,
                    int32_t* __restrict__ flags) {
  for (size_t c = blockIdx.x * (size_t)blockDim.x + threadIdx.x; c < C; c += (size_t)gridDim.x * blockDim.x) {
    const int2 ij = pairs[c];
    const double need_i = budget[ij.x], need_j = budget[ij.y];
    bool cold;
    if (c >= H_old && wake_old[2 * (c - H_old)] > -1.7976931348623157e308) {
      cold = wake_old[2 * (c - H_old)] - drift[ij.x] > need_i && wake_old[2 * (c - H_old) + 1] - drift[ij.y] > need_j;
    } else {
      const double2 a = Pcur[c], b = Pprev[c];
      cold = a.x == 0.0 && b.x == 0.0 && a.y > kTierMinGap && a.y <= 1.7976931348623157e308 && kTierShare * a.y > need_i &&
             kTierShare * a.y > need_j;
    }
    flags[c] = cold ? 0 : 1;
  }
}
template <int KIN>
__global__ void __launch_bounds__(kBlock)
    k_tier_permute(size_t C, size_t I, size_t H, int cur_is_p1, const int2* __restrict__ pairs, const double* __restrict__ normal,
                   const double* __restrict__ arc_s, const double* __restrict__ arc_t, const double* __restrict__ ra,
                   const double* __restrict__ rb, const double* __restrict__ q, const int32_t* __restrict__ orig,
                   const unsigned char* __restrict__ pos, TierGeo dst,
                   const double2* __restrict__ P0s, const double2* __restrict__ P1s, double2* __restrict__ P0d,
                   double2* __restrict__ P1d, const int32_t* __restrict__ flags, const int32_t* __restrict__ rank,
                   int32_t* __restrict__ new_of, const double* __restrict__ wake_old, size_t H_old,
                   double* __restrict__ wake_new, const double* __restrict__ drift, double* __restrict__ fire_at) {
  for (size_t c = blockIdx.x * (size_t)blockDim.x + threadIdx.x; c < C; c += (size_t)gridDim.x * blockDim.x) {
    const bool fixed = c >= I;
    const bool hot = fixed || flags[c] != 0;
    const size_t r = fixed ? 0 : static_cast<size_t>(rank[c]);
    const size_t nc = fixed ? c : (hot ? r : H + (c - r));
    new_of[c] = static_cast<int32_t>(nc);
    const int2 ij = pairs[c];
    dst.pairs[nc] = ij;
    store3(dst.normal, nc, load3(normal, c));
    if (KIN == KIN_ROD) {
      dst.arc_s[nc] = arc_s[c];
      dst.arc_t[nc] = arc_t[c];
    }
    if (KIN == KIN_RIGID) {
      store3(dst.ra, nc, load3(ra, c));
      store3(dst.rb, nc, load3(rb, c));
    }
    dst.q[nc] = q[c];
    dst.orig[nc] = orig ? orig[c] : static_cast<int32_t>(c);
    dst.pos[2 * nc] = pos[2 * c];
    dst.pos[2 * nc + 1] = pos[2 * c + 1];
    double2 a0 = P0s[c], a1 = P1s[c];
    if (!hot) {
      const bool asleep = c >= H_old && wake_old[2 * (c - H_old)] > -1.7976931348623157e308;
      double ti, tj;
      if (asleep) {
        ti = wake_old[2 * (c - H_old)];
        tj = wake_old[2 * (c - H_old) + 1];
      } else {
        const double g = cur_is_p1 ? a1.y : a0.y;
        ti = drift[ij.x] + kTierShare * g;
        tj = drift[ij.y] + kTierShare * g;
        a0 = a1 = make_double2(0.0, g);
      }
      wake_new[2 * (nc - H)] = ti;
      wake_new[2 * (nc - H) + 1] = tj;
      atomicMin(reinterpret_cast<unsigned long long*>(fire_at + ij.x), static_cast<unsigned long long>(__double_as_longlong(ti)));
      atomicMin(reinterpret_cast<unsigned long long*>(fire_at + ij.y), static_cast<unsigned long long>(__double_as_longlong(tj)));
    }
    P0d[nc] = a0;
    P1d[nc] = a1;
  }
}
__global__ void __launch_bounds__(kBlock) k_tier_remap_inc(size_t n, int32_t* __restrict__ inc,
                                                          const int32_t* __restrict__ map) {
  for (size_t k = blockIdx.x * (size_t)blockDim.x + threadIdx.x; k < n; k += (size_t)gridDim.x * blockDim.x) {
    const int32_t e = inc[k];
    inc[k] = (map[e >> 1] << 1) | (e & 1);
  }
}
template <int KIN>
__global__ void __launch_bounds__(kBlock)
    k_tier_refresh_sleepers(OpView op , size_t H, size_t I, int cur_is_1, const double* __restrict__ vcur,
                            const double* __restrict__ vprev, const double* __restrict__ q,
                            const double* __restrict__ wake, double2* __restrict__ P0, double2* __restrict__ P1) {
  double2* Pcur = cur_is_1 ? P1 : P0;
  double2* Pprev = cur_is_1 ? P0 : P1;
  for (size_t c = H + blockIdx.x * (size_t)blockDim.x + threadIdx.x; c < I; c += (size_t)gridDim.x * blockDim.x) {
    if (!(wake[2 * (c - H)] > -1.7976931348623157e308)) continue;
    const int2 ij = op.pairs[c];
    Pcur[c] = make_double2(0.0, 1.0 * q[c] + 1.0 * contact_dt_sdot<KIN>(op, vcur, c, ij));
    Pprev[c] = make_double2(0.0, 1.0 * q[c] + 1.0 * contact_dt_sdot<KIN>(op, vprev, c, ij));
  }
}
__global__ void __launch_bounds__(kBlock) k_tier_prev_x(size_t n, const double2* __restrict__ Pprev,
                                                       double* __restrict__ x) {
  for (size_t i = blockIdx.x * (size_t)blockDim.x + threadIdx.x; i < n; i += (size_t)gridDim.x * blockDim.x) x[i] = Pprev[i].x;
}
__global__ void __launch_bounds__(kBlock)
    k_tier_finish(size_t n, const SolverState* __restrict__ st, const double2* __restrict__ P0,
                  const double2* __restrict__ P1, const int32_t* __restrict__ orig, double* __restrict__ x,
                  double* __restrict__ g, double* __restrict__ x_tmp, double* __restrict__ g_tmp) {
  const bool p = st->flips & 1u;
  const double2 *cur, *old;
  if (st->converged_at_init) { cur = P0; old = P0; }
  else if (st->converged) { cur = p ? P0 : P1; old = p ? P1 : P0; }
  else { cur = p ? P1 : P0; old = cur; }
  for (size_t i = blockIdx.x * (size_t)blockDim.x + threadIdx.x; i < n; i += (size_t)gridDim.x * blockDim.x) {
    const double2 a = cur[i], b = old[i];
    const size_t o = static_cast<size_t>(orig[i]);
    x[o] = a.x; g[o] = a.y; x_tmp[o] = b.x; g_tmp[o] = b.y;
  }
}
__global__ void __launch_bounds__(kBlock)
    k_tier_scatter_pairs(size_t n, const double2* __restrict__ P0, const double2* __restrict__ P1,
                         const int32_t* __restrict__ orig, double2* __restrict__ Q0, double2* __restrict__ Q1) {
  for (size_t i = blockIdx.x * (size_t)blockDim.x + threadIdx.x; i < n; i += (size_t)gridDim.x * blockDim.x) {
    const size_t o = static_cast<size_t>(orig[i]);
    Q0[o] = P0[i];
    Q1[o] = P1[i];
  }
}

bool tier_problem_kind(const Space& sp, int resid_kind) {
  return sp.kind == MHIP_SPACE_LOWER_BOUND && sp.lo == 0.0 && resid_kind == MHIP_RESIDUAL_PROJECTED_DIFF;
}
bool tier_eligible(const mhip_contact_op* op, const Space& sp, int resid_kind) {
  const OpView& v = op->view;
  return (v.C >= kTierMinContacts || op->tiering >= 2) && v.body_mask != nullptr && v.counted == nullptr &&
         v.body_first == 0 && v.body_count == v.N && tier_problem_kind(sp, resid_kind);
}

unsigned tier_service_blocks(size_t awake) {
  const size_t want = kTierFireBlocks + 8 * (awake / (8 * 2 * kBlock));
  return static_cast<unsigned>(want < 256 ? want : 256);
}

struct TierPairs {
  double *P0, *P1;
  const double* q;
};

int tier_update(mhip_contact_op* op, TierPairs& cur, unsigned iters_done, unsigned next_period, size_t I, bool pingpong,
                hipStream_t s) {
  mhip_contact_op::Tier& t = op->tier;
  OpView& v = op->view;
  const size_t C = v.C, N = v.N;
  if (I > C) I = C;
  if (int e = t.misc.reserve(tier_misc_bytes(C, N))) return e;
  if (int e = op->scanws.reserve(scan_workspace_bytes(C + 2) + 64)) return e;
  const TierMisc m = tier_misc_at(t.misc.ptr, C, N);
  const bool cur_is_p1 = op->host_state->flips & 1u;
  if (!t.tracking) {
    if (int e = t.vel2.reserve((6 * N + 8) * sizeof(double))) return e;
    if (int e = t.drift.reserve((N + 8) * sizeof(double))) return e;
    MHIP_HIP(hipMemsetAsync(t.drift.ptr, 0, N * sizeof(double), s));
    MHIP_HIP(hipMemsetAsync(m.drift_prev, 0, N * sizeof(double), s));
    if (pingpong && cur_is_p1)
      MHIP_HIP(hipMemcpyAsync(t.vel2.ptr, v.vel, 6 * N * sizeof(double), hipMemcpyDeviceToDevice, s));
    if (op->kin == KIN_RIGID) {
      if (int e = t.arm.reserve((N + 8) * sizeof(double))) return e;
      k_tier_arm_max<<<grid_for(N), kBlock, 0, s>>>(N, v.inc_ptr, v.half, t.arm.as<double>());
      MHIP_LAUNCH_CHECK();
      v.arm_max = t.arm.as<double>();
    }
    t.saved_vel = v.vel;
    t.pingpong = pingpong;
    v.vel_alt = pingpong ? t.vel2.as<double>() : nullptr;
    v.drift = t.drift.as<double>();
    t.tracking = true;
    t.polled_at = iters_done;
    return MHIP_SUCCESS;
  }
  const unsigned last_period = iters_done - t.polled_at;
  const unsigned min_window = iters_done / 2 < kTierHorizon / 2 ? iters_done / 2 : kTierHorizon / 2;
  if (last_period == 0 || last_period < min_window) return MHIP_SUCCESS;
  t.polled_at = iters_done;
  const unsigned horizon = next_period > kTierHorizon ? next_period : kTierHorizon;
  const double scale = static_cast<double>(horizon) / static_cast<double>(last_period);
  k_tier_budget<<<grid_for(N), kBlock, 0, s>>>(N, t.drift.as<double>(), m.drift_prev, scale, m.budget);
  MHIP_LAUNCH_CHECK();
  const double2* Pc = reinterpret_cast<const double2*>(cur_is_p1 ? cur.P1 : cur.P0);
  const double2* Pp = reinterpret_cast<const double2*>(cur_is_p1 ? cur.P0 : cur.P1);
  const double* wake_old = t.active ? m.wake[t.set] : m.wake[0];
  const size_t H_old = t.active ? t.H : C;
  if (I == 0) return MHIP_SUCCESS;
  k_tier_classify<<<grid_for(I), kBlock, 0, s>>>(I, v.pairs, Pc, Pp, m.budget, t.drift.as<double>(), wake_old, H_old,
                                                 m.flags);
  MHIP_LAUNCH_CHECK();
  if (int e = exclusive_scan_i32(m.flags, m.rank, I, op->scanws.ptr, s)) return e;
  int32_t H32 = 0;
  unsigned long long awake = 0;
  MHIP_HIP(hipMemcpyAsync(&H32, m.rank + I, sizeof(int32_t), hipMemcpyDeviceToHost, s));
  if (t.active) MHIP_HIP(hipMemcpyAsync(&awake, m.counters, sizeof(awake), hipMemcpyDeviceToHost, s));
  MHIP_HIP(hipStreamSynchronize(s));
  const size_t H = static_cast<size_t>(H32);
#ifdef MHIP_TIER_DEBUG
  fprintf(stderr, "compact active entries at the last snapshot but one: %d of %zu half edges\n",
          *reinterpret_cast<const int32_t*>(op->host_state + 1), 2 * C);
  fprintf(stderr, "tier_update: iter %u last_period %u next %u scale %.2f  H %zu of I %zu (%.3f)  active %d awake %llu\n",
          iters_done, last_period, next_period, scale, H, I, (double)H / (double)I, (int)t.active, awake);
#endif
  if (t.active) {
    t.service_blocks = tier_service_blocks(static_cast<size_t>(awake));
    if (100 * H >= (100 - MHIP_TIER_RETIER_PERCENT) * (t.H + static_cast<size_t>(awake))) return MHIP_SUCCESS;
  } else if (10 * H > 9 * I) {
    return MHIP_SUCCESS;
  }
  const int dst_set = t.active ? (t.set ^ 1) : 0;
  if (int e = t.geo[dst_set].reserve(tier_geo_bytes(C, op->kin == KIN_RIGID))) return e;
  if (int e = t.iter[dst_set].reserve(2 * (C + 1) * sizeof(double2))) return e;
  const TierGeo dst = tier_geo_at(t.geo[dst_set].ptr, C);
  double2* P0d = t.iter[dst_set].as<double2>();
  double2* P1d = P0d + C;
  const int32_t* orig_src = nullptr;
  if (t.active)
    orig_src = tier_geo_at(t.geo[t.set].ptr, C).orig;
  else
    t.saved = v;
  if (int e = mhip_fill(N, m.fire_at, __builtin_huge_val(), reinterpret_cast<mhip_stream_t>(s))) return e;
  with_kin(op, [&](auto kin) {
    k_tier_permute<decltype(kin)::value><<<grid_for(C), kBlock, 0, s>>>(
        C, I, H, cur_is_p1 ? 1 : 0, v.pairs, v.normal, v.arc_s, v.arc_t, v.ra, v.rb, cur.q, orig_src, v.pos, dst,
        reinterpret_cast<const double2*>(cur.P0), reinterpret_cast<const double2*>(cur.P1), P0d, P1d, m.flags, m.rank,
        m.new_of, wake_old, H_old, m.wake[dst_set], t.drift.as<double>(), m.fire_at);
  });
  MHIP_LAUNCH_CHECK();
  k_tier_remap_inc<<<grid_for(2 * C), kBlock, 0, s>>>(2 * C, op->inc.as<int32_t>(), m.new_of);
  MHIP_LAUNCH_CHECK();
  MHIP_HIP(hipMemsetAsync(m.counters, 0, 4 * sizeof(unsigned long long), s));
  v.pairs = dst.pairs;
  v.normal = dst.normal;
  v.arc_s = dst.arc_s;
  v.arc_t = dst.arc_t;
  if (op->kin == KIN_RIGID) {
    v.ra = dst.ra;
    v.rb = dst.rb;
  }
  v.pos = dst.pos;
  v.fire_at = m.fire_at;
  v.fired = m.fired;
  v.tier_counters = m.counters;
  cur.P0 = reinterpret_cast<double*>(P0d);
  cur.P1 = reinterpret_cast<double*>(P1d);
  cur.q = dst.q;
  t.wakeups += static_cast<size_t>(awake);
  t.active = true;
  t.service_blocks = kTierFireBlocks;
  t.set = dst_set;
  t.H = H;
  t.I = I;
  t.retiers += 1;
  return MHIP_SUCCESS;
}

int tier_stop_tracking(mhip_contact_op* op, hipStream_t s) {
  mhip_contact_op::Tier& t = op->tier;
  if (!t.tracking) return MHIP_SUCCESS;
  const SolverState& hs = *op->host_state;
  const unsigned curv = (hs.converged && !hs.converged_at_init) ? ((hs.flips + 1u) & 1u) : (hs.flips & 1u);
  if (t.pingpong && curv == 1u)
    MHIP_HIP(hipMemcpyAsync(t.saved_vel, t.vel2.ptr, 6 * op->view.N * sizeof(double), hipMemcpyDeviceToDevice, s));
  op->view.vel_alt = nullptr;
  op->view.drift = nullptr;
  t.tracking = false;
  return MHIP_SUCCESS;
}

int tier_release(mhip_contact_op* op, TierPairs& cur, bool final, double* P0, double* P1, const double* q_caller,
                 double* x, double* g, double* x_tmp, double* g_tmp, hipStream_t s) {
  mhip_contact_op::Tier& t = op->tier;
  if (!t.active) return tier_stop_tracking(op, s);
  OpView& v = op->view;
  const size_t C = v.C, N = v.N;
  const TierMisc m = tier_misc_at(t.misc.ptr, C, N);
  const TierGeo geo = tier_geo_at(t.geo[t.set].ptr, C);
  const SolverState* st = op->state.as<SolverState>();
  double2* T0 = reinterpret_cast<double2*>(cur.P0);
  double2* T1 = reinterpret_cast<double2*>(cur.P1);
  if (t.H < t.I) {
    const SolverState& hs = *op->host_state;
    const bool conv = hs.converged && !hs.converged_at_init;
    const unsigned cur1 = conv ? ((hs.flips + 1u) & 1u) : (hs.flips & 1u);
    const double *vcur, *vprev;
    if (t.pingpong) {
      vcur = cur1 ? v.vel_alt : v.vel;
      vprev = cur1 ? v.vel : v.vel_alt;
    } else {
      if (int e = t.vel2.reserve((10 * N + 16) * sizeof(double))) return e;
      if (int e = t.xprev.reserve((C + 2) * sizeof(double))) return e;
      k_tier_prev_x<<<grid_for(C), kBlock, 0, s>>>(C, cur1 ? T0 : T1, t.xprev.as<double>());
      MHIP_LAUNCH_CHECK();
      double* rows = t.vel2.as<double>();
      double* const keep_vel = v.vel;
      double* const keep_omega = v.omega;
      double* const keep_drift = v.drift;
      const int32_t* const keep_aptr = v.aptr;
      v.vel = rows;
      v.omega = rows + 6 * N;
      v.drift = nullptr;
      v.aptr = nullptr;
      const int e = op_launch_body(op, X_APPLY, t.xprev.as<double>(), t.xprev.as<double>(), nullptr, nullptr,
                                   Space{MHIP_SPACE_UNCONSTRAINED, 0.0, 0.0}, s);
      v.vel = keep_vel;
      v.omega = keep_omega;
      v.drift = keep_drift;
      v.aptr = keep_aptr;
      if (e) return e;
      vcur = v.vel;
      vprev = rows;
    }
    const unsigned grid = grid_for(t.I - t.H);
    with_kin(op, [&](auto kin) {
      k_tier_refresh_sleepers<decltype(kin)::value>
          <<<grid, kBlock, 0, s>>>(v, t.H, t.I, static_cast<int>(cur1), vcur, vprev, cur.q, m.wake[t.set], T0, T1);
    });
    MHIP_LAUNCH_CHECK();
  }
  if (final)
    k_tier_finish<<<grid_for(C), kBlock, 0, s>>>(C, st, T0, T1, geo.orig, x, g, x_tmp, g_tmp);
  else
    k_tier_scatter_pairs<<<grid_for(C), kBlock, 0, s>>>(C, T0, T1, geo.orig, reinterpret_cast<double2*>(P0),
                                                        reinterpret_cast<double2*>(P1));
  MHIP_LAUNCH_CHECK();
  k_tier_remap_inc<<<grid_for(2 * C), kBlock, 0, s>>>(2 * C, op->inc.as<int32_t>(), geo.orig);
  MHIP_LAUNCH_CHECK();
  unsigned long long awake = 0;
  MHIP_HIP(hipMemcpyAsync(&awake, m.counters, sizeof(awake), hipMemcpyDeviceToHost, s));
  MHIP_HIP(hipStreamSynchronize(s));
  t.wakeups += static_cast<size_t>(awake);
  const OpView keep = v;
  v = t.saved;
  v.xcd_aware = keep.xcd_aware;
  v.vel_alt = keep.vel_alt;
  v.drift = keep.drift;
  v.fire_at = nullptr;
  v.fired = nullptr;
  v.tier_counters = nullptr;
  v.aptr = nullptr;
  t.active = false;
  cur.P0 = P0;
  cur.P1 = P1;
  cur.q = q_caller;
  return tier_stop_tracking(op, s);
}

int op_launch_constraint_tiered(mhip_contact_op* op, const TierPairs& cur, Space sp, int resid_kind, unsigned* nparts,
                                hipStream_t s) {
  mhip_contact_op::Tier& t = op->tier;
  const size_t C = op->view.C, N = op->view.N;
  const SolverState* st = op->state.as<SolverState>();
  double* parts = op->partials.as<double>();
  const TierMisc m = tier_misc_at(t.misc.ptr, C, N);
  const unsigned ghot = t.H ? constraint_grid(t.H) : 0u;
  const unsigned gcheck = t.H < t.I ? t.service_blocks : 0u;
  OpView hot = op->view;
  hot.c_first = 0; hot.c_end = t.H; hot.part_offset = 0; hot.part_stride = kStageStride;
  const TierCheck tc{t.H, t.I, m.wake[t.set], m.list, m.counters, m.fired, m.fire_at, gcheck};
  if (ghot + gcheck) {
    with_kin(op, [&](auto kin) {
      k_constraint<X_SOLVE, decltype(kin)::value, true><<<ghot + gcheck, kBlock, 0, s>>>(
          hot, st, cur.P0, cur.P1, nullptr, nullptr, cur.q, sp, resid_kind, parts, tc);
    });
    MHIP_LAUNCH_CHECK();
  }
  *nparts = ghot + gcheck;
  return MHIP_SUCCESS;
}

int check_config(const mhip_pgd_config* cfg) {
  MHIP_REQUIRE(cfg != nullptr, MHIP_ERR_INVALID_ARGUMENT, "config must not be null");
  MHIP_REQUIRE(cfg->residual_kind == MHIP_RESIDUAL_PROJECTED_DIFF ||
                   cfg->residual_kind == MHIP_RESIDUAL_PROJECTED_GRADIENT,
               MHIP_ERR_INVALID_ARGUMENT, "unknown residual kind %d", cfg->residual_kind);
  return MHIP_SUCCESS;
}

template <int M>
void finalize_sweep(mhip_contact_op* op, unsigned cgrid, const mhip_pgd_config* cfg, hipStream_t s) {
  SolverState* st = op->state.as<SolverState>();
  unsigned np = cgrid;
  size_t ps = cgrid;
  double* pp = op->partials.as<double>();
  fold_partials(np, ps, pp, st, M == X_INIT ? 0 : 1, s);
  k_finalize<M><<<1, final_block(np), 0, s>>>((int)np, pp, 1, ps, st, cfg->residual_kind, cfg->tol, cfg->max_iters);
}

template <class Iteration>
int poll_loop(mhip_contact_op* op, unsigned max_iters, hipStream_t s, const Iteration& iteration) {
  unsigned enqueued = 0, chunk = 8;
  for (;;) {
    MHIP_HIP(hipMemcpyAsync(op->host_state, op->state.ptr, sizeof(SolverState), hipMemcpyDeviceToHost, s));
    MHIP_HIP(hipStreamSynchronize(s));
    if (op->host_state->done || enqueued >= max_iters) return MHIP_SUCCESS;
    const unsigned todo = (max_iters - enqueued < chunk) ? max_iters - enqueued : chunk;
    for (unsigned k = 0; k < todo; ++k)
      if (int e = iteration(enqueued + k)) return e;
    MHIP_LAUNCH_CHECK();
    enqueued += todo;
    if (chunk < 64) chunk *= 2;
  }
}

int solve_result(mhip_contact_op* op, hipStream_t s, mhip_solve_result* result) {
  MHIP_HIP(hipStreamSynchronize(s));
  result->num_iters = op->host_state->iter;
  result->residual = op->host_state->residual;
  result->converged = op->host_state->converged;
  return MHIP_SUCCESS;
}

int check_friction_args(mhip_contact_op* op, const double* sep, double mu, const mhip_pgd_config* config, const double* p,
                        const double* g, mhip_solve_result* result) {
  MHIP_REQUIRE(op != nullptr && result != nullptr, MHIP_ERR_INVALID_ARGUMENT, "null handle / result");
  if (int e = check_config(config)) return e;
  MHIP_REQUIRE(config->residual_kind == MHIP_RESIDUAL_PROJECTED_DIFF, MHIP_ERR_INVALID_ARGUMENT,
               "the friction extension supports the projected-difference residual only");
  MHIP_REQUIRE(mu >= 0.0 && mu == mu, MHIP_ERR_INVALID_ARGUMENT, "friction coefficient must be >= 0, got %g", mu);
  MHIP_REQUIRE(op->kin == KIN_RIGID, MHIP_ERR_INVALID_ARGUMENT,
               "friction needs the vector-arm operator (mhip_contact_op_create with ra, rb, mob_rot)");
  if (op->view.C == 0) {
    result->num_iters = 0;
    result->residual = kLowest / kSmallStep;
    result->converged = 1;
    return MHIP_SUCCESS;
  }
  MHIP_REQUIRE(sep && p && g, MHIP_ERR_INVALID_ARGUMENT, "solver vectors must not be null");
  MHIP_REQUIRE(p != g, MHIP_ERR_INVALID_ARGUMENT, "solver vectors must not alias");
  MHIP_REQUIRE((reinterpret_cast<uintptr_t>(op->view.half) & 15) == 0, MHIP_ERR_RUNTIME, "misaligned records");
  return MHIP_SUCCESS;
}

template <class Apply>
int solve_generic(size_t n, const Apply& apply, const double* q, Space sp, const mhip_pgd_config* cfg, double* x,
                  double* g, double* x_tmp, double* g_tmp, mhip_solve_result* result, hipStream_t s) {
  double res = 0.0;
  if (int e = launch_copy(n, x_tmp, x, s)) return e;
  if (int e = apply(x_tmp, g_tmp)) return e;
  if (int e = launch_axpby(n, 1.0, q, 1.0, g_tmp, s)) return e;
  if (int e = reduce_to_host<2>(n, x_tmp, g_tmp, nullptr, nullptr, cfg->residual_kind, sp, &res, s)) return e;
  if (cfg->residual_kind == MHIP_RESIDUAL_PROJECTED_DIFF) res = res / kSmallStep;
  double step = 1.0 / res;
  unsigned iter = 0;
  bool converged = (res <= cfg->tol);
  if (converged)
    if (int e = launch_copy(n, g, g_tmp, s)) return e;
  while (!(converged || iter >= cfg->max_iters)) {
    if (int e = launch_wrapped_axpbyz(n, 1.0, x_tmp, -step, g_tmp, x, sp, s)) return e;
    if (int e = apply(x, g)) return e;
    if (int e = launch_axpby(n, 1.0, q, 1.0, g, s)) return e;
    if (int e = reduce_to_host<2>(n, x, g, nullptr, nullptr, cfg->residual_kind, sp, &res, s)) return e;
    if (cfg->residual_kind == MHIP_RESIDUAL_PROJECTED_DIFF) res = res / kSmallStep;
    if (res <= cfg->tol) {
      converged = true;
      break;
    }
    double num = 0.0, den = 0.0;
    if (int e = reduce_to_host<0>(n, x, x_tmp, nullptr, nullptr, 0, sp, &num, s)) return e;
    if (int e = reduce_to_host<1>(n, x, x_tmp, g, g_tmp, 0, sp, &den, s)) return e;
    den += kBBEps * (fabs(den) < kBBEps);
    step = num / den;
    if (int e = launch_copy(n, x_tmp, x, s)) return e;
    if (int e = launch_copy(n, g_tmp, g, s)) return e;
    ++iter;
  }
  MHIP_HIP(hipStreamSynchronize(s));
  result->num_iters = iter;
  result->residual = res;
  result->converged = converged ? 1 : 0;
  return MHIP_SUCCESS;
}

}

#define REQ(p) MHIP_REQUIRE((p) != nullptr || n == 0, MHIP_ERR_INVALID_ARGUMENT, "%s: %s is null", __func__, #p)

namespace mhip {
void stage_state_words(mhip_contact_op_t op, const unsigned** flips, const int** done) {
  const SolverState* st = op->state.as<SolverState>();
  *flips = &st->flips;
  *done = &st->done;
}
int stage_reduce_exchange_finalize(mhip_contact_op_t op, int init, const MailboxArgs& mb, hipStream_t s) {
  MHIP_REQUIRE(op != nullptr && op->stage.active, MHIP_ERR_RUNTIME, "mhip_bbpgd_stage_begin has not been called");
  MHIP_REQUIRE(mb.peers != nullptr && mb.width == kRed && mb.world >= 1 && mb.world <= kMailboxMaxWorld,
               MHIP_ERR_INVALID_ARGUMENT, "mailbox of %d ranks, record width %d", mb.world, mb.width);
  const unsigned np = op->stage.part_used;
  const size_t ps = kStageStride;
  double* pp = op->partials.as<double>();
  const auto& cfg = op->stage.cfg;
  SolverState* st = op->state.as<SolverState>();
  unsigned* ticket = reinterpret_cast<unsigned*>(op->state.as<char>() + sizeof(SolverState) + 16);
  if (init)
    k_fold_finalize<X_INIT><<<kFoldGroups, MHIP_FOLD_BLOCK, 0, s>>>((int)np, ps, pp, pp + kRed * ps, ticket, st,
                                                                     cfg.residual_kind, cfg.tol, cfg.max_iters, 0,
                                                                     nullptr, mb);
  else
    k_fold_finalize<X_SOLVE><<<kFoldGroups, MHIP_FOLD_BLOCK, 0, s>>>(
        (int)np, ps, pp, pp + kRed * ps, ticket, st, cfg.residual_kind, cfg.tol, cfg.max_iters,
        op->stage.pause_on_bad_step ? ((op->tiering == 2 && op->stage.polls >= 10) ? 2 : 1) : 0,
        op->tier.active ? op->view.tier_counters : nullptr, mb);
  MHIP_LAUNCH_CHECK();
  op->stage.part_used = 0;
  return MHIP_SUCCESS;
}
int stage_reduce_exchange(mhip_contact_op_t op, int init, double* local, const MailboxArgs& mb, hipStream_t s) {
  MHIP_REQUIRE(op != nullptr && op->stage.active, MHIP_ERR_RUNTIME, "mhip_bbpgd_stage_begin has not been called");
  MHIP_REQUIRE(local != nullptr, MHIP_ERR_INVALID_ARGUMENT, "local record is null");
  unsigned np = op->stage.part_used;
  size_t ps = kStageStride;
  double* pp = op->partials.as<double>();
// ... 363 lines not shown
  const Space none{MHIP_SPACE_UNCONSTRAINED, 0, 0};
  return op_launch_body(op, X_APPLY, x, x, nullptr, nullptr, none, as_stream(stream));
}

int mhip_contact_op_body_sweep_vector(mhip_contact_op_t op, const double* force, mhip_stream_t stream) {
  MHIP_REQUIRE(op != nullptr, MHIP_ERR_INVALID_ARGUMENT, "operator handle is null");
  MHIP_REQUIRE(op->view.C == 0 || force, MHIP_ERR_INVALID_ARGUMENT, "force must not be null");
  MHIP_REQUIRE(!op->stage.active, MHIP_ERR_RUNTIME, "a staged solve is in progress");
  if (op->view.N == 0 || op->view.body_count == 0) return MHIP_SUCCESS;
  hipStream_t s = as_stream(stream);
  op->last_stream = s;
  constexpr int G = 4;
  const unsigned grid = grid_exact(op->view.body_count * (size_t)G);
  with_kin(op, [&](auto kin) { k_body_vector<decltype(kin)::value, G><<<grid, kBlock, 0, s>>>(op->view, force); });
  MHIP_LAUNCH_CHECK();
  return MHIP_SUCCESS;
}

int mhip_contact_op_constraint_rate(mhip_contact_op_t op, const double* velocity, double* sep_dot,
                                    mhip_stream_t stream) {
  MHIP_REQUIRE(op != nullptr, MHIP_ERR_INVALID_ARGUMENT, "operator handle is null");
  MHIP_REQUIRE(op->view.C == 0 || (velocity && sep_dot), MHIP_ERR_INVALID_ARGUMENT, "velocity / sep_dot must not be null");
  MHIP_REQUIRE(!op->stage.active, MHIP_ERR_RUNTIME, "a staged solve is in progress");
  if (op->view.C == 0) return MHIP_SUCCESS;
  hipStream_t s = as_stream(stream);
  op->last_stream = s;
  OpView v = op->view;
  v.dt = 1.0;
  v.vel = const_cast<double*>(velocity);
  if (op->kin == KIN_ROD) {
    const size_t N = op->view.N;
    if (int e = op->rate_rows.reserve((6 * N + 2) * sizeof(double))) return e;
    k_rate_rows<<<grid_for(N), kBlock, 0, s>>>(N, velocity, op->axis.as<double>(), op->rate_rows.as<double>());
    v.vel = op->rate_rows.as<double>();
  }
  const Space none{MHIP_SPACE_UNCONSTRAINED, 0, 0};
  double* x0 = op->half.as<double>();
  const SolverState* st = op->state.as<SolverState>();
  double* parts = op->partials.as<double>();
  const unsigned grid = grid_for(op->view.C);
  with_kin(op, [&](auto kin) {
    k_constraint<X_APPLY, decltype(kin)::value, false>
        <<<grid, kBlock, 0, s>>>(v, st, x0, nullptr, nullptr, sep_dot, nullptr, none, 0, parts);
  });
  MHIP_LAUNCH_CHECK();
  return MHIP_SUCCESS;
}

int mhip_contact_op_sizes(mhip_contact_op_t op, size_t* num_constraints, size_t* num_bodies) {
  MHIP_REQUIRE(op != nullptr, MHIP_ERR_INVALID_ARGUMENT, "operator handle is null");
  if (num_constraints) *num_constraints = op->view.C;
  if (num_bodies) *num_bodies = op->view.N;
  return MHIP_SUCCESS;
}

int mhip_contact_op_set_work_mapping(mhip_contact_op_t op, int xcd_tile, int lanes_per_body) {
  MHIP_REQUIRE(op != nullptr, MHIP_ERR_INVALID_ARGUMENT, "operator handle is null");
  MHIP_REQUIRE(xcd_tile >= -1 && xcd_tile <= 4096, MHIP_ERR_INVALID_ARGUMENT,
               "xcd_tile must be in [0, 4096] (or -1 to keep the current value), got %d", xcd_tile);
  MHIP_REQUIRE(lanes_per_body == -1 || lanes_per_body == 1 || lanes_per_body == 2 || lanes_per_body == 4 ||
                   lanes_per_body == 8 || lanes_per_body == 16,
               MHIP_ERR_INVALID_ARGUMENT, "lanes_per_body must be 1, 2, 4, 8 or 16 (or -1 to keep), got %d", lanes_per_body);
  MHIP_REQUIRE(!op->stage.active, MHIP_ERR_RUNTIME, "a staged solve is in progress");
  if (xcd_tile >= 0) op->view.xcd_aware = xcd_tile;
  if (lanes_per_body > 0) op->lanes_per_body = lanes_per_body;
  return MHIP_SUCCESS;
}

int mhip_contact_op_set_drift_source(mhip_contact_op_t op, int source) {
  MHIP_REQUIRE(op != nullptr, MHIP_ERR_INVALID_ARGUMENT, "operator handle is null");
  MHIP_REQUIRE(source >= 0 && source <= 2, MHIP_ERR_INVALID_ARGUMENT, "drift source must be 0 (by size), 1 (rows) or 2 (registers), got %d", source);
  op->drift_source = source;
  return MHIP_SUCCESS;
}

int mhip_contact_op_get_drift_source(mhip_contact_op_t op, int* source) {
  MHIP_REQUIRE(op != nullptr && source != nullptr, MHIP_ERR_INVALID_ARGUMENT, "null argument");
  *source = op_drift_source(op);
  return MHIP_SUCCESS;
}

int mhip_contact_op_set_profiling(mhip_contact_op_t op, int enable) {
  MHIP_REQUIRE(op != nullptr, MHIP_ERR_INVALID_ARGUMENT, "operator handle is null");
  op->profile = enable != 0;
  op->body_ms = op->constraint_ms = 0.0;
  op->timed_iterations = 0;
  return MHIP_SUCCESS;
}

int mhip_contact_op_get_profile(mhip_contact_op_t op, double* body_ms, double* constraint_ms, size_t* iterations) {
  MHIP_REQUIRE(op != nullptr, MHIP_ERR_INVALID_ARGUMENT, "operator handle is null");
  if (body_ms) *body_ms = op->body_ms;
  if (constraint_ms) *constraint_ms = op->constraint_ms;
  if (iterations) *iterations = op->timed_iterations;
  return MHIP_SUCCESS;
}

int mhip_contact_op_body_velocity(mhip_contact_op_t op, const double** velocity) {
  MHIP_REQUIRE(op != nullptr && velocity != nullptr, MHIP_ERR_INVALID_ARGUMENT, "null argument");
  if (op->kin == KIN_ROD) {
    const size_t N = op->view.N;
    if (int e = op->vel_out.reserve((6 * N + 2) * sizeof(double))) return e;
    if (N > 0) {
      k_assemble_velocity<<<grid_for(N), kBlock, 0, op->last_stream>>>(N, op->view.vel, op->omega.as<double>(),
                                                                      op->vel_out.as<double>());
      MHIP_LAUNCH_CHECK();
    }
    *velocity = op->vel_out.as<double>();
    return MHIP_SUCCESS;
  }
  *velocity = op->view.vel;
  return MHIP_SUCCESS;
}

int mhip_bbpgd_solve_contact(mhip_contact_op_t op, const double* q, const mhip_space* space,
                             const mhip_pgd_config* config, double* x, double* g, double* x_tmp, double* g_tmp,
                             mhip_solve_result* result, mhip_stream_t stream) {
  TraceRange trace_range("solve_cqpp (fused BBPGD)");
  MHIP_REQUIRE(op != nullptr && result != nullptr, MHIP_ERR_INVALID_ARGUMENT, "null handle / result");
  if (int e = check_config(config)) return e;
  Space sp;
  if (int e = to_space(space, &sp)) return e;
  const size_t C = op->view.C;
  hipStream_t s = as_stream(stream);
  if (C == 0) {
    result->num_iters = 0;
    result->residual = config->residual_kind == MHIP_RESIDUAL_PROJECTED_DIFF ? kLowest / kSmallStep : kLowest;
    result->converged = 1;
    return MHIP_SUCCESS;
  }
  MHIP_REQUIRE(q && x && g && x_tmp && g_tmp, MHIP_ERR_INVALID_ARGUMENT, "solver vectors must not be null");
  MHIP_REQUIRE(x != x_tmp && g != g_tmp && x != g, MHIP_ERR_INVALID_ARGUMENT, "solver vectors must not alias");
  SolverState* st = op->state.as<SolverState>();
  double* parts = op->partials.as<double>();
  const unsigned cgrid = constraint_grid(C);
  const int rk = config->residual_kind;
  if (int e = op->iterate.reserve(2 * (C + 1) * sizeof(double2))) return e;
  double* P0 = op->iterate.as<double>();
  double* P1 = P0 + 2 * C;
  if (op->view.body_mask) MHIP_HIP(hipMemsetAsync(op->view.body_mask, 0x00, op->view.N * sizeof(unsigned long long), s));
  op->view.aptr = nullptr;
  if (int e = op_launch_body(op, X_INIT, x, x, nullptr, nullptr, sp, s)) return e;
  if (int e = op_launch_constraint(op, X_INIT, P0, P1, x, nullptr, q, sp, rk, cgrid, s, true)) return e;
  finalize_sweep<X_INIT>(op, cgrid, config, s);
  MHIP_LAUNCH_CHECK();
  unsigned enqueued = 0, chunk = 8, last_todo = 0, iter_before = 0;
  const bool prof = op->profile;
  if (prof && op->events.empty()) {
    op->events.resize(3 * 64);
    for (auto& ev : op->events) MHIP_HIP(hipEventCreate(&ev));
  }
  mhip_contact_op::Tier& tier = op->tier;
  tier.disabled = !tier_eligible(op, sp, rk) || op->tiering == 0;
  tier.tiered_iterations = tier.retiers = tier.wakeups = 0;
  tier.hot_sum = 0.0;
  TierPairs cur{P0, P1, q};
  struct TierGuard {
    mhip_contact_op* op;
    ~TierGuard() {
      if (!op->tier.active) {
        op->view.vel_alt = nullptr;
        op->view.drift = nullptr;
        op->tier.tracking = false;
        return;
      }
      op->tier.tracking = false;
      const size_t C2 = op->view.C;
      const TierGeo geo = tier_geo_at(op->tier.geo[op->tier.set].ptr, C2);
      k_tier_remap_inc<<<grid_for(2 * C2), kBlock, 0, op->last_stream>>>(2 * C2, op->inc.as<int32_t>(), geo.orig);
      (void)hipStreamSynchronize(op->last_stream);
      const int xa = op->view.xcd_aware;
      op->view = op->tier.saved;
      op->view.xcd_aware = xa;
      op->view.aptr = nullptr;
      op->tier.active = false;
    }
  } tier_guard{op};
  PollPlan plan;
  for (;;) {
    MHIP_HIP(hipMemcpyAsync(op->host_state, st, sizeof(SolverState), hipMemcpyDeviceToHost, s));
    MHIP_HIP(hipStreamSynchronize(s));
    if (prof && last_todo) {
      unsigned eff = op->host_state->iter - iter_before + ((op->host_state->converged && op->host_state->iter < config->max_iters) ? 1u : 0u);
      if (eff > last_todo) eff = last_todo;
      for (unsigned k = 0; k < eff; k += kProfileStride) {
        float a = 0.f, b = 0.f;
        MHIP_HIP(hipEventElapsedTime(&a, op->events[3 * k], op->events[3 * k + 1]));
        MHIP_HIP(hipEventElapsedTime(&b, op->events[3 * k + 1], op->events[3 * k + 2]));
        op->body_ms += a;
        op->constraint_ms += b;
        op->timed_iterations += 1;
      }
    }
    if (tier.active && last_todo) {
      unsigned ran = op->host_state->iter - iter_before + ((op->host_state->converged && op->host_state->iter < config->max_iters) ? 1u : 0u);
      if (ran > last_todo) ran = last_todo;
      tier.tiered_iterations += ran;
      tier.hot_sum += ran * (static_cast<double>(tier.H) / static_cast<double>(C));
    }
    if (op->host_state->done == 2) {
      if (int e = tier_release(op, cur, false, P0, P1, q, nullptr, nullptr, nullptr, nullptr, s)) return e;
      tier.disabled = true;
      op->host_state->done = 0;
      MHIP_HIP(hipMemcpyAsync(&st->done, &op->host_state->done, sizeof(int), hipMemcpyHostToDevice, s));
      enqueued = op->host_state->iter;
    }
    if (op->host_state->done || enqueued >= config->max_iters) break;
    if (enqueued == 0)
      if (int e = op_snapshot_active(op, s)) return e;
    const bool light = plan.light_poll();
    if (!light) {
      const size_t retiers_before = tier.retiers;
      if (!tier.disabled && (enqueued >= kSnapshotAfter || !tier.tracking)) {
        const unsigned left = config->max_iters - enqueued;
        if (int e = tier_update(op, cur, op->host_state->iter, left < chunk ? left : chunk, C, true, s)) return e;
      }
      if (enqueued >= kSnapshotAfter)
        if (int e = op_snapshot_active(op, s)) return e;
      plan.full_poll_done(enqueued, *reinterpret_cast<const int32_t*>(op->host_state + 1),
                          tier.retiers != retiers_before, !tier.disabled && !tier.active);
    }
    iter_before = op->host_state->iter;
    const unsigned stretch = plan.stretch(chunk, op->host_state->iter, op->host_state->residual, config->tol, C);
    const unsigned todo = (config->max_iters - enqueued < stretch) ? config->max_iters - enqueued : stretch;
#ifdef MHIP_TIER_DEBUG
    fprintf(stderr, "poll: iter %u residual %.3e light %d quiet %u stretch %u (regular %u) snapshot entries %d\n",
            op->host_state->iter, op->host_state->residual, (int)light, plan.quiet, stretch, chunk,
            *reinterpret_cast<const int32_t*>(op->host_state + 1));
#endif
    for (unsigned k = 0; k < todo; ++k) {
      const bool pk = prof && (k % kProfileStride == 0);
      if (pk) MHIP_HIP(hipEventRecord(op->events[3 * k], s));
      if (int e = op_launch_body(op, X_SOLVE, cur.P0, cur.P1, nullptr, nullptr, sp, s, true)) return e;
      if (pk) MHIP_HIP(hipEventRecord(op->events[3 * k + 1], s));
      unsigned np = cgrid;
      size_t ps = cgrid;
      if (tier.active) {
        if (int e = op_launch_constraint_tiered(op, cur, sp, rk, &np, s)) return e;
        ps = kStageStride;
      } else {
        if (int e = op_launch_constraint(op, X_SOLVE, cur.P0, cur.P1, nullptr, nullptr, q, sp, rk, cgrid, s, true)) return e;
      }
      if (pk) MHIP_HIP(hipEventRecord(op->events[3 * k + 2], s));
      double* pp = parts;
      if (np > MHIP_FOLD_ABOVE) {
        k_fold_finalize<X_SOLVE><<<kFoldGroups, MHIP_FOLD_BLOCK, 0, s>>>(
            (int)np, ps, pp, pp + kRed * ps, reinterpret_cast<unsigned*>(op->state.as<char>() + sizeof(SolverState) + 16),
            st, rk, config->tol, config->max_iters, tier.active ? op->tiering : 0,
            tier.active ? op->view.tier_counters : nullptr);
      } else {
        k_finalize<X_SOLVE><<<1, final_block(np), 0, s>>>((int)np, pp, 1, ps, st, rk, config->tol, config->max_iters,
                                                          tier.active ? op->tiering : 0,
                                                          tier.active ? op->view.tier_counters : nullptr);
      }
      MHIP_LAUNCH_CHECK();
    }
    enqueued += todo;
    last_todo = todo;
    if (chunk < 64) chunk *= 2;
  }
  if (tier.active) {
    if (int e = tier_release(op, cur, true, P0, P1, q, x, g, x_tmp, g_tmp, s)) return e;
  } else {
    if (int e = tier_stop_tracking(op, s)) return e;
    k_finish_packed<<<grid_for(C), kBlock, 0, s>>>(C, st, reinterpret_cast<const double2*>(P0),
                                                   reinterpret_cast<const double2*>(P1), x, g, x_tmp, g_tmp);
    MHIP_LAUNCH_CHECK();
  }
  if (op->kin == KIN_ROD)
    if (int e = op_launch_body(op, X_APPLY, x, nullptr, nullptr, nullptr, sp, s)) return e;
  return solve_result(op, s, result);
}

int mhip_contact_op_tier_stats(mhip_contact_op_t op, size_t* tiered_iterations, double* mean_hot_fraction,
                               size_t* renumberings, size_t* wakeups) {
  MHIP_REQUIRE(op != nullptr, MHIP_ERR_INVALID_ARGUMENT, "operator handle is null");
  const mhip_contact_op::Tier& t = op->tier;
  if (tiered_iterations) *tiered_iterations = t.tiered_iterations;
  if (mean_hot_fraction) *mean_hot_fraction = t.tiered_iterations ? t.hot_sum / static_cast<double>(t.tiered_iterations) : 0.0;
  if (renumberings) *renumberings = t.retiers;
  if (wakeups) *wakeups = t.wakeups;
  return MHIP_SUCCESS;
}

int mhip_contact_op_set_tiering(mhip_contact_op_t op, int mode) {
  MHIP_REQUIRE(op != nullptr, MHIP_ERR_INVALID_ARGUMENT, "operator handle is null");
  MHIP_REQUIRE(mode >= 0 && mode <= 3, MHIP_ERR_INVALID_ARGUMENT, "tiering mode must be 0 ... 3, got %d", mode);
  op->tiering = mode;
  return MHIP_SUCCESS;
}

int mhip_bbpgd_solve_contact_friction(mhip_contact_op_t op, const double* sep, double mu,
                                      const mhip_pgd_config* config, double* p, double* g,
                                      mhip_solve_result* result, mhip_stream_t stream) {
  TraceRange trace_range("solve_friction_contact (extension)");
  if (int e = check_friction_args(op, sep, mu, config, p, g, result)) return e;
  const size_t C = op->view.C;
  if (C == 0) return MHIP_SUCCESS;
  hipStream_t s = as_stream(stream);
  if (int e = op->iterate.reserve(2 * (6 * C + 2) * sizeof(double))) return e;
  double* P0 = op->iterate.as<double>();
  double* P1 = P0 + 6 * C;
  SolverState* st = op->state.as<SolverState>();
  double* parts = op->partials.as<double>();
  const unsigned cgrid = constraint_grid(C);
  const int G = 8;
  const unsigned bgrid = grid_exact(op->view.body_count * (size_t)G);
  op->last_stream = s;
  if (op->view.body_count > 0) k_body_friction<true, 8, 2><<<bgrid, kBlock, 0, s>>>(op->view, st, P0, P1, p, mu);
  k_constraint_friction<true><<<cgrid, kBlock, 0, s>>>(op->view, st, P0, P1, p, sep, mu, parts);
  finalize_sweep<X_INIT>(op, cgrid, config, s);
  MHIP_LAUNCH_CHECK();
  if (int e = poll_loop(op, config->max_iters, s, [&](unsigned) -> int {
        if (op->view.body_count > 0)
          k_body_friction<false, 8, 2><<<bgrid, kBlock, 0, s>>>(op->view, st, P0, P1, nullptr, mu);
        k_constraint_friction<false><<<cgrid, kBlock, 0, s>>>(op->view, st, P0, P1, nullptr, sep, mu, parts);
        finalize_sweep<X_SOLVE>(op, cgrid, config, s);
        return MHIP_SUCCESS;
      }))
    return e;
  k_finish_friction<<<grid_for(C), kBlock, 0, s>>>(C, st, P0, P1, p, g);
  MHIP_LAUNCH_CHECK();
  return solve_result(op, s, result);
}

int mhip_apgd_solve_contact_friction(mhip_contact_op_t op, const double* sep, double mu, const mhip_pgd_config* config,
                                     double* p, double* g, mhip_solve_result* result, mhip_stream_t stream) {
  TraceRange trace_range("solve_friction_contact, APGD (extension)");
  if (int e = check_friction_args(op, sep, mu, config, p, g, result)) return e;
  const size_t C = op->view.C;
  if (C == 0) return MHIP_SUCCESS;
  hipStream_t s = as_stream(stream);
  if (int e = op->iterate.reserve((3 * (6 * C + 2) + 16) * sizeof(double))) return e;
  ApgdBufs B;
  B.P[0] = op->iterate.as<double>();
  B.P[1] = B.P[0] + 6 * C + 2;
  B.P[2] = B.P[1] + 6 * C + 2;
  ApgdState* as = reinterpret_cast<ApgdState*>(B.P[2] + 6 * C + 2);
  SolverState* st = op->state.as<SolverState>();
  double* parts = op->partials.as<double>();
  const unsigned cgrid = constraint_grid(C);
  static_assert(kApgdRed * kMaxConstraintGrid <= kRed * (int)kStageStride, "partials buffer holds the APGD records");
  const int G = 8;
  const unsigned bgrid = grid_exact(op->view.body_count * (size_t)G);
  op->last_stream = s;
  if (op->view.body_count > 0) k_body_friction<true, 8, 2><<<bgrid, kBlock, 0, s>>>(op->view, st, B.P[0], B.P[1], p, mu);
  k_constraint_friction<true><<<cgrid, kBlock, 0, s>>>(op->view, st, B.P[0], B.P[1], p, sep, mu, parts);
  finalize_sweep<X_INIT>(op, cgrid, config, s);
  k_apgd_begin<<<1, 1, 0, s>>>(st, as);
  MHIP_LAUNCH_CHECK();
  if (int e = poll_loop(op, config->max_iters, s, [&](unsigned) -> int {
        if (op->view.body_count > 0) k_body_friction_apgd<8, 2><<<bgrid, kBlock, 0, s>>>(op->view, st, as, B, mu);
        k_constraint_friction_apgd<<<cgrid, kBlock, 0, s>>>(op->view, st, as, B, sep, mu, parts);
        k_apgd_finalize<<<1, kFinalBlock, 0, s>>>((int)cgrid, parts, st, as, config->tol, config->max_iters);
        return MHIP_SUCCESS;
      }))
    return e;
  k_finish_friction_apgd<<<grid_for(C), kBlock, 0, s>>>(C, st, as, B, p, g);
  MHIP_LAUNCH_CHECK();
  return solve_result(op, s, result);
}

int mhip_solve_small_cqpp_batch(size_t batch, int n, const double* A, const double* q, const mhip_space* space,
                                const mhip_pgd_config* config, double* x, double* grad, unsigned* num_iters,
                                double* residual, int* converged, mhip_stream_t stream) {
  if (int e = check_config(config)) return e;
  Space sp;
  if (int e = to_space(space, &sp)) return e;
  MHIP_REQUIRE(n >= 1 && n <= kSmallMax, MHIP_ERR_INVALID_ARGUMENT, "small-problem size must be in [1, %d], got %d",
               kSmallMax, n);
  if (batch == 0) return MHIP_SUCCESS;
  MHIP_REQUIRE(A && q && x && grad && num_iters && residual && converged, MHIP_ERR_INVALID_ARGUMENT,
               "null argument");
  k_small_cqpp<<<grid_exact(batch, 64), 64, 0, as_stream(stream)>>>(batch, n, A, q, sp, config->residual_kind,
                                                                   config->max_iters, config->tol, x, grad, num_iters,
                                                                   residual, converged);
  MHIP_LAUNCH_CHECK();
  return MHIP_SUCCESS;
}

int mhip_scrap_bbpgd_solve_contact(mhip_contact_op_t op, const double* sep, double max_allowable_overlap,
                                   unsigned max_iterations, double* lam, double* lam_tmp, double* g, double* g_tmp,
                                   mhip_solve_result* result, double* max_speed, mhip_stream_t stream) {
  TraceRange trace_range("resolve_collisions");
  MHIP_REQUIRE(op != nullptr && result != nullptr, MHIP_ERR_INVALID_ARGUMENT, "null handle / result");
  const size_t C = op->view.C;
  hipStream_t s = as_stream(stream);
  result->num_iters = 0;
  result->residual = -1.0;
  result->converged = 1;
  if (max_speed) *max_speed = 0.0;
  if (C == 0) return MHIP_SUCCESS;
  MHIP_REQUIRE(sep && lam && lam_tmp && g && g_tmp, MHIP_ERR_INVALID_ARGUMENT, "solver vectors must not be null");
  MHIP_REQUIRE(lam != lam_tmp && g != g_tmp && lam != g, MHIP_ERR_INVALID_ARGUMENT, "solver vectors must not alias");
  SolverState* st = op->state.as<SolverState>();
  double* parts = op->partials.as<double>();
  const unsigned cgrid = grid_for(C);
  const Space lcp{MHIP_SPACE_LOWER_BOUND, 0.0, 0.0};
  if (int e = op->iterate.reserve(2 * (C + 1) * sizeof(double2))) return e;
  double* D0 = op->iterate.as<double>();
  double* D1 = D0 + C;
  auto constraint = [&](auto init) {
    with_kin(op, [&](auto kin) {
      k_scrap_constraint<decltype(kin)::value, decltype(init)::value><<<cgrid, kBlock, 0, s>>>(
          op->view, st, lam_tmp, lam, g_tmp, g, D0, D1, sep, parts);
    });
  };
  if (int e = launch_copy(C, lam_tmp, lam, s)) return e;
  MHIP_HIP(hipMemsetAsync(st, 0, sizeof(SolverState), s));
  if (int e = op_launch_body(op, X_INIT, lam_tmp, lam, g_tmp, g, lcp, s)) return e;
  constraint(std::true_type{});
  MHIP_LAUNCH_CHECK();
  k_scrap_finalize<true><<<1, kBlock, 0, s>>>((int)cgrid, parts, st, max_allowable_overlap, max_iterations);
  MHIP_LAUNCH_CHECK();
  if (int e = poll_loop(op, max_iterations, s, [&](unsigned k) -> int {
        const double* gbody = (k == 0) ? sep : g_tmp;
        if (int e = op_launch_body(op, X_SOLVE, lam_tmp, lam, gbody, g, lcp, s)) return e;
        constraint(std::false_type{});
        MHIP_LAUNCH_CHECK();
        k_scrap_finalize<false><<<1, kBlock, 0, s>>>((int)cgrid, parts, st, max_allowable_overlap, max_iterations);
        MHIP_LAUNCH_CHECK();
        return MHIP_SUCCESS;
      }))
    return e;
  k_finish<<<grid_for(C), kBlock, 0, s>>>(C, st, lam_tmp, lam, g_tmp, g);
  MHIP_LAUNCH_CHECK();
  if (max_speed && op->view.N > 0) {
    ReduceScratch& rs = reduce_scratch();
    if (int e = rs.ensure()) return e;
    double* mp = rs.dev.as<double>();
    const unsigned g2 = grid_for(op->view.N);
    k_max_speed<<<g2, kBlock, 0, s>>>(op->view.N, op->view.vel, mp);
    MHIP_LAUNCH_CHECK();
    k_reduce_final<2><<<1, kBlock, 0, s>>>((int)g2, mp, mp + 2 * kMaxGrid);
    MHIP_LAUNCH_CHECK();
    MHIP_HIP(hipMemcpyAsync(rs.host, mp + 2 * kMaxGrid, sizeof(double), hipMemcpyDeviceToHost, s));
    MHIP_HIP(hipStreamSynchronize(s));
    *max_speed = rs.host[0] < 0.0 ? 0.0 : rs.host[0];
  }
  return solve_result(op, s, result);
}

int mhip_contact_op_set_partition(mhip_contact_op_t op, size_t body_first, size_t body_count,
                                  const unsigned char* counted_contacts, double* velocity) {
  MHIP_REQUIRE(op != nullptr, MHIP_ERR_INVALID_ARGUMENT, "operator handle is null");
  MHIP_REQUIRE(body_first + body_count <= op->view.N, MHIP_ERR_INVALID_ARGUMENT,
               "owned body range [%zu, %zu) exceeds the %zu local bodies", body_first, body_first + body_count,
               op->view.N);
  op->view.aptr = nullptr;
  op->view.body_first = body_first;
  op->view.body_count = body_count;
  op->view.counted = counted_contacts;
  op->view.vel = velocity ? velocity : op->vel.as<double>();
  return MHIP_SUCCESS;
}

int mhip_bbpgd_stage_begin(mhip_contact_op_t op, const double* q, const mhip_space* space,
                           const mhip_pgd_config* config, double* x, double* g, double* x_tmp, double* g_tmp,
                           mhip_stream_t stream) {
  MHIP_REQUIRE(op != nullptr, MHIP_ERR_INVALID_ARGUMENT, "operator handle is null");
  if (int e = check_config(config)) return e;
  Space sp;
  if (int e = to_space(space, &sp)) return e;
  const size_t C = op->view.C;
  MHIP_REQUIRE(C == 0 || (q && x && g && x_tmp && g_tmp), MHIP_ERR_INVALID_ARGUMENT,
               "solver vectors must not be null");
  MHIP_REQUIRE(C == 0 || (x != x_tmp && g != g_tmp && x != g), MHIP_ERR_INVALID_ARGUMENT,
               "solver vectors must not alias");
  op->stage.q = q; op->stage.x = x; op->stage.g = g; op->stage.x_tmp = x_tmp; op->stage.g_tmp = g_tmp;
  op->stage.sp = sp;
  op->stage.cfg = *config;
  op->stage.active = true;
  op->stage.part_used = 0;
  op->view.aptr = nullptr;
  if (op->view.body_mask)
    MHIP_HIP(hipMemsetAsync(op->view.body_mask, 0x00, op->view.N * sizeof(unsigned long long), as_stream(stream)));
  if (int e = op->iterate.reserve(2 * (C + 1) * sizeof(double2))) return e;
  MHIP_HIP(hipMemsetAsync(op->state.ptr, 0, sizeof(SolverState), as_stream(stream)));
  op->stage.P0 = op->iterate.as<double>();
  op->stage.P1 = op->stage.P0 + 2 * C;
  op->stage.q_cur = q;
  op->stage.interior = 0;
  op->stage.interior_known = false;
  op->stage.polls = 0;
  op->stage.iter_at_poll = 0;
  op->stage.snap_at = 0;
  op->stage.pause_on_bad_step = op->tiering != 0 && tier_problem_kind(sp, config->residual_kind);
  mhip_contact_op::Tier& tier = op->tier;
  if (tier.active) {
    const TierGeo geo = tier_geo_at(tier.geo[tier.set].ptr, C);
    k_tier_remap_inc<<<grid_for(2 * C), kBlock, 0, as_stream(stream)>>>(2 * C, op->inc.as<int32_t>(), geo.orig);
    MHIP_LAUNCH_CHECK();
    op->view.pairs = tier.saved.pairs;
    op->view.normal = tier.saved.normal;
    op->view.ra = tier.saved.ra;
    op->view.rb = tier.saved.rb;
    op->view.arc_s = tier.saved.arc_s;
    op->view.arc_t = tier.saved.arc_t;
    op->view.pos = tier.saved.pos;
    op->view.aptr = nullptr;
  }
  op->view.vel_alt = nullptr;
  op->view.drift = nullptr;
  op->view.fire_at = nullptr;
  op->view.fired = nullptr;
  op->view.tier_counters = nullptr;
  tier.active = tier.tracking = false;
  tier.disabled = !op->stage.pause_on_bad_step || op->view.body_mask == nullptr ||
                  !(C >= kTierMinContacts || op->tiering >= 2);
  tier.tiered_iterations = tier.retiers = tier.wakeups = 0;
  tier.hot_sum = 0.0;
  return MHIP_SUCCESS;
}

int mhip_bbpgd_stage_body(mhip_contact_op_t op, int init, mhip_stream_t stream) {
  MHIP_REQUIRE(op != nullptr && op->stage.active, MHIP_ERR_RUNTIME, "mhip_bbpgd_stage_begin has not been called");
  auto& st = op->stage;
  if (init) return op_launch_body(op, X_INIT, st.x, st.x, nullptr, nullptr, st.sp, as_stream(stream));
  return op_launch_body(op, X_SOLVE, st.P0, st.P1, nullptr, nullptr, st.sp, as_stream(stream), true);
}

int mhip_bbpgd_stage_constraint_range(mhip_contact_op_t op, int init, size_t c_first, size_t c_count,
                                      mhip_stream_t stream) {
  MHIP_REQUIRE(op != nullptr && op->stage.active, MHIP_ERR_RUNTIME, "mhip_bbpgd_stage_begin has not been called");
  MHIP_REQUIRE(c_first + c_count <= op->view.C, MHIP_ERR_INVALID_ARGUMENT,
               "constraint range [%zu, %zu) exceeds the %zu constraints", c_first, c_first + c_count, op->view.C);
  auto& st = op->stage;
  if (c_first == 0 && !st.interior_known) {
    st.interior = c_count;
    st.interior_known = true;
  }
  mhip_contact_op::Tier& tier = op->tier;
  if (tier.active) {
    MHIP_REQUIRE(!init && ((c_first == 0 && c_count == tier.I) || (c_first == tier.I && c_first + c_count == op->view.C)),
                 MHIP_ERR_RUNTIME, "constraint range [%zu, %zu) does not match the ranges of the tiered solve", c_first,
                 c_first + c_count);
    hipStream_t s = as_stream(stream);
    const SolverState* sst = op->state.as<SolverState>();
    double* parts = op->partials.as<double>();
    const TierMisc m = tier_misc_at(tier.misc.ptr, op->view.C, op->view.N);
    OpView vw = op->view;
    vw.part_offset = st.part_used;
    vw.part_stride = kStageStride;
    unsigned grid = 0, extra = 0;
    TierCheck tc{};
    if (c_first == 0) {
      vw.c_first = 0;
      vw.c_end = tier.H;
      grid = tier.H ? constraint_grid(tier.H) : 0u;
      if (tier.H < tier.I) {
        extra = tier.service_blocks;
        tc = TierCheck{tier.H, tier.I, m.wake[tier.set], m.list, m.counters, m.fired, m.fire_at, extra};
      }
    } else {
      if (c_count == 0) return MHIP_SUCCESS;
      vw.c_first = c_first;
      vw.c_end = c_first + c_count;
      grid = constraint_grid(c_count);
    }
    if (grid + extra == 0) return MHIP_SUCCESS;
    MHIP_REQUIRE(st.part_used + grid + extra <= kStageStride, MHIP_ERR_RUNTIME, "too many constraint sweeps in one iteration");
    with_kin(op, [&](auto kin) {
      k_constraint<X_SOLVE, decltype(kin)::value, true><<<grid + extra, kBlock, 0, s>>>(
          vw, sst, st.P0, st.P1, nullptr, nullptr, st.q_cur, st.sp, st.cfg.residual_kind, parts, tc);
    });
    MHIP_LAUNCH_CHECK();
    st.part_used += grid + extra;
    return MHIP_SUCCESS;
  }
  if (c_count == 0) return MHIP_SUCCESS;
  const unsigned grid = constraint_grid(c_count);
  MHIP_REQUIRE(st.part_used + grid <= kStageStride, MHIP_ERR_RUNTIME, "too many constraint sweeps in one iteration");
  op->view.c_first = c_first;
  op->view.c_end = c_first + c_count;
  op->view.part_offset = st.part_used;
  op->view.part_stride = kStageStride;
  const int e = op_launch_constraint(op, init ? X_INIT : X_SOLVE, st.P0, st.P1, init ? st.x : nullptr, nullptr, st.q_cur,
                                     st.sp, st.cfg.residual_kind, grid, as_stream(stream), true);
  op->view.c_first = 0;
  op->view.c_end = op->view.C;
  op->view.part_offset = 0;
  op->view.part_stride = 0;
  if (e) return e;
  st.part_used += grid;
  return MHIP_SUCCESS;
}

int mhip_bbpgd_stage_reduce(mhip_contact_op_t op, int init, double* local, mhip_stream_t stream) {
  return mhip::stage_reduce_exchange(op, init, local, mhip::MailboxArgs{}, as_stream(stream));
}

int mhip_bbpgd_stage_constraint(mhip_contact_op_t op, int init, double* local, mhip_stream_t stream) {
  MHIP_REQUIRE(op != nullptr && op->stage.active, MHIP_ERR_RUNTIME, "mhip_bbpgd_stage_begin has not been called");
  op->stage.part_used = 0;
  if (int e = mhip_bbpgd_stage_constraint_range(op, init, 0, op->view.C, stream)) return e;
  return mhip_bbpgd_stage_reduce(op, init, local, stream);
}

int mhip_bbpgd_stage_finalize(mhip_contact_op_t op, int init, const double* gathered, int nparts,
                              mhip_stream_t stream) {
  MHIP_REQUIRE(op != nullptr && op->stage.active, MHIP_ERR_RUNTIME, "mhip_bbpgd_stage_begin has not been called");
  MHIP_REQUIRE(gathered != nullptr && nparts >= 1, MHIP_ERR_INVALID_ARGUMENT, "gathered records missing");
  const auto& cfg = op->stage.cfg;
  SolverState* st = op->state.as<SolverState>();
  if (init)
    k_finalize<X_INIT><<<1, final_block(nparts), 0, as_stream(stream)>>>(nparts, gathered, kRed, 1, st, cfg.residual_kind,
                                                                         cfg.tol, cfg.max_iters);
  else
    k_finalize<X_SOLVE><<<1, final_block(nparts), 0, as_stream(stream)>>>(
        nparts, gathered, kRed, 1, st, cfg.residual_kind, cfg.tol, cfg.max_iters,
        op->stage.pause_on_bad_step ? ((op->tiering == 2 && op->stage.polls >= 10) ? 2 : 1) : 0,
        op->tier.active ? op->view.tier_counters : nullptr);
  MHIP_LAUNCH_CHECK();
  return MHIP_SUCCESS;
}

int mhip_bbpgd_stage_poll(mhip_contact_op_t op, mhip_solve_result* result, int* done, mhip_stream_t stream) {
  MHIP_REQUIRE(op != nullptr && result != nullptr && done != nullptr, MHIP_ERR_INVALID_ARGUMENT, "null argument");
  hipStream_t s = as_stream(stream);
  MHIP_HIP(hipMemcpyAsync(op->host_state, op->state.ptr, sizeof(SolverState), hipMemcpyDeviceToHost, s));
  MHIP_HIP(hipStreamSynchronize(s));
  if (op->stage.active) {
    if (op->tier.active && op->host_state->iter > op->stage.iter_at_poll) {
      const unsigned ran = op->host_state->iter - op->stage.iter_at_poll;
      op->tier.tiered_iterations += ran;
      op->tier.hot_sum += ran * (static_cast<double>(op->tier.H + (op->view.C - op->tier.I)) / static_cast<double>(op->view.C));
    }
    op->stage.iter_at_poll = op->host_state->iter;
  }
  if (op->host_state->done == 2 && op->stage.active) {
    mhip_contact_op::Tier& tier = op->tier;
    if (tier.active) {
      TierPairs cur{op->stage.P0, op->stage.P1, op->stage.q_cur};
      double* P0 = op->iterate.as<double>();
      if (int e = tier_release(op, cur, false, P0, P0 + 2 * op->view.C, op->stage.q, nullptr, nullptr, nullptr, nullptr, s))
        return e;
      op->stage.P0 = cur.P0;
      op->stage.P1 = cur.P1;
      op->stage.q_cur = cur.q;
    } else if (int e = tier_stop_tracking(op, s)) {
      return e;
    }
    tier.disabled = true;
    op->stage.pause_on_bad_step = false;
    op->host_state->done = 0;
    MHIP_HIP(hipMemcpyAsync(&op->state.as<SolverState>()->done, &op->host_state->done, sizeof(int), hipMemcpyHostToDevice, s));
    MHIP_HIP(hipStreamSynchronize(s));
  }
  result->num_iters = op->host_state->iter;
  result->residual = op->host_state->residual;
  result->converged = op->host_state->converged;
  *done = op->host_state->done;
  return MHIP_SUCCESS;
}

int mhip_bbpgd_stage_snapshot_active(mhip_contact_op_t op, mhip_stream_t stream) {
  MHIP_REQUIRE(op != nullptr && op->stage.active, MHIP_ERR_RUNTIME, "mhip_bbpgd_stage_begin has not been called");
  hipStream_t s = as_stream(stream);
  auto& st = op->stage;
  st.polls += 1;
  mhip_contact_op::Tier& tier = op->tier;
  const size_t retiers_before = tier.retiers;
  if (!tier.disabled && st.interior_known && !op->host_state->done) {
    TierPairs cur{st.P0, st.P1, st.q_cur};
// ... 68 lines not shown
```

mundy_amd/ops.py:

```python
import ctypes as C
import math
from dataclasses import dataclass

import numpy as np
import torch

from . import capi
from .capi import (RESIDUAL_PROJECTED_DIFF, RESIDUAL_PROJECTED_GRADIENT, SEARCH_AABB, SEARCH_METHOD_AUTO,
                   SEARCH_METHOD_GRID, SEARCH_METHOD_MORTON_LBVH, SEARCH_SPHERES, SPACE_BOUNDED, SPACE_LOWER_BOUND, SPACE_UNCONSTRAINED, SPACE_UPPER_BOUND)


def _stream():
    return C.c_void_p(torch.cuda.current_stream().cuda_stream)


def _ptr(t, dtype=torch.float64, cols=None, name="tensor", allow_none=False):
    if t is None:
        if allow_none:
            return None
        raise ValueError("%s must not be None" % name)
    if not t.is_cuda:
        raise ValueError("%s must live on the GPU (mundy_amd has no CPU path)" % name)
    if t.dtype != dtype:
        raise ValueError("%s must be %s, got %s" % (name, dtype, t.dtype))
# ... 527 lines not shown
    max_iters: int = 1000
    tol: float = 1e-8
    residual_kind: int = RESIDUAL_PROJECTED_DIFF


@dataclass
class SolveResult:
    num_iters: int = 0
    residual: float = 0.0
    converged: bool = False


def _space(space):
    kind, lo, hi = space
    return capi.Space(int(kind), float(lo), float(hi))


def _cfg(cfg):
    return capi.PgdConfig(int(cfg.max_iters), float(cfg.tol), int(cfg.residual_kind))


LCP_SPACE = (SPACE_LOWER_BOUND, 0.0, 0.0)


def axpby(alpha, x, beta, y):
    capi.check(capi.load().mhip_axpby(x.shape[0], alpha, _ptr(x), beta, _ptr(y), _stream()))


def wrapped_axpbyz(alpha, x, beta, y, z, space):
    sp = _space(space)
    capi.check(capi.load().mhip_wrapped_axpbyz(x.shape[0], alpha, _ptr(x), beta, _ptr(y), _ptr(z), C.byref(sp),
                                               _stream()))


def diff_dot(x, y, x2=None, y2=None):
    r = C.c_double()
    if x2 is None:
        capi.check(capi.load().mhip_diff_dot2(x.shape[0], _ptr(x), _ptr(y), C.byref(r), _stream()))
    else:
        capi.check(capi.load().mhip_diff_dot4(x.shape[0], _ptr(x), _ptr(y), _ptr(x2), _ptr(y2), C.byref(r), _stream()))
    return r.value


def residual(kind, x, grad, space):
    r = C.c_double()
    sp = _space(space)
    capi.check(capi.load().mhip_residual(x.shape[0], kind, _ptr(x), _ptr(grad), C.byref(sp), C.byref(r), _stream()))
    return r.value


def bb_step(x_old, g_old, x, g):
    r = C.c_double()
    capi.check(capi.load().mhip_bb_step(x.shape[0], _ptr(x_old), _ptr(g_old), _ptr(x), _ptr(g), C.byref(r), _stream()))
    return r.value


def gemv(A, x):
    y = torch.empty_like(x)
    capi.check(capi.load().mhip_gemv(x.shape[0], _ptr(A), _ptr(x), _ptr(y), _stream()))
    return y


class ContactOperator(_Handle):
    _destroy = "mhip_contact_op_destroy"

    def __init__(self, pairs, normal, mob_trans, dt, ra=None, rb=None, mob_rot=None, rod=None, priority=None):
        self.num_constraints = pairs.shape[0]
        self.num_bodies = mob_trans.shape[0]
        self._keep = (pairs, normal, ra, rb, mob_trans, mob_rot, rod, priority)
        prio = _ptr(priority, allow_none=True, name="priority")
        h = C.c_void_p()
        if rod is not None:
            arc_s, arc_t, seg = rod
            capi.check(capi.load().mhip_contact_op_create_rods(
                C.byref(h), self.num_constraints, self.num_bodies, _ptr(pairs, torch.int32, 2), _ptr(normal, cols=3),
                _ptr(arc_s), _ptr(arc_t), _ptr(seg, cols=8), _ptr(mob_trans), _ptr(mob_rot), float(dt), prio, _stream()))
        else:
            capi.check(capi.load().mhip_contact_op_create(
                C.byref(h), self.num_constraints, self.num_bodies, _ptr(pairs, torch.int32, 2), _ptr(normal, cols=3),
                _ptr(ra, allow_none=True, name="ra"), _ptr(rb, allow_none=True, name="rb"), _ptr(mob_trans),
                _ptr(mob_rot, allow_none=True, name="mob_rot"), float(dt), prio, _stream()))
        self._h = h
        self._device = normal.device

    def refresh(self, normal, ra=None, rb=None, rod=None):
        pairs, _, _, _, mob_trans, mob_rot, old_rod, priority = self._keep
        if (rod is None) != (old_rod is None):
            raise ValueError("refresh must keep the operator's kinematics")
        if rod is not None:
            arc_s, arc_t, seg = rod
            capi.check(capi.load().mhip_contact_op_refresh_rods(self._h, _ptr(normal, cols=3), _ptr(arc_s), _ptr(arc_t),
                                                                _ptr(seg, cols=8), _stream()))
        else:
            capi.check(capi.load().mhip_contact_op_refresh(self._h, _ptr(normal, cols=3),
                                                           _ptr(ra, allow_none=True, name="ra"),
                                                           _ptr(rb, allow_none=True, name="rb"), _stream()))
        self._keep = (pairs, normal, ra, rb, mob_trans, mob_rot, rod, priority)

    def apply(self, x, y=None):
        y = torch.empty_like(x) if y is None else y
        capi.check(capi.load().mhip_contact_op_apply(self._h, _ptr(x), _ptr(y), _stream()))
        return y

    def body_sweep(self, x):
        if tuple(x.shape) != (self.num_constraints,):
            raise ValueError("x must have shape [%d], got %s" % (self.num_constraints, tuple(x.shape)))
        capi.check(capi.load().mhip_contact_op_body_sweep(self._h, _ptr(x, name="x"), _stream()))

    def body_sweep_vector(self, force):
        if tuple(force.shape) != (self.num_constraints, 3):
            raise ValueError("force must have shape [%d, 3], got %s" % (self.num_constraints, tuple(force.shape)))
        capi.check(capi.load().mhip_contact_op_body_sweep_vector(self._h, _ptr(force, name="force"), _stream()))

    def constraint_rate(self, velocity, out=None):
        if tuple(velocity.shape) != (self.num_bodies, 6):
            raise ValueError("velocity must have shape [%d, 6], got %s" % (self.num_bodies, tuple(velocity.shape)))
        y = torch.empty(self.num_constraints, dtype=torch.float64, device=self._device) if out is None else out
        capi.check(capi.load().mhip_contact_op_constraint_rate(self._h, _ptr(velocity, cols=6, name="velocity"),
                                                               _ptr(y, name="out"), _stream()))
        return y

    def body_velocity_of(self, x):
        self.body_sweep(x)
        return self.body_velocity()

    def body_velocity(self):
        p = C.c_void_p()
        capi.check(capi.load().mhip_contact_op_body_velocity(self._h, C.byref(p)))
        n = self.num_bodies
        if n == 0:
            return torch.empty((0, 6), dtype=torch.float64, device=self._device)
        out = torch.empty((n, 6), dtype=torch.float64, device=self._device)
        capi.check(capi.load().mhip_deep_copy(6 * n, _ptr(out), p, _stream()))
        return out

    def set_work_mapping(self, xcd_tile=-1, lanes_per_body=-1):
        capi.check(capi.load().mhip_contact_op_set_work_mapping(self._h, int(xcd_tile), int(lanes_per_body)))

    def set_tiering(self, mode=1):
        capi.check(capi.load().mhip_contact_op_set_tiering(self._h, int(mode)))

    def set_drift_source(self, source=0):
        capi.check(capi.load().mhip_contact_op_set_drift_source(self._h, int(source)))

    def drift_source(self):
        v = C.c_int(0)
        capi.check(capi.load().mhip_contact_op_get_drift_source(self._h, C.byref(v)))
        return int(v.value)

    def tier_stats(self):
        it, rn, wk, hot = C.c_size_t(0), C.c_size_t(0), C.c_size_t(0), C.c_double(0.0)
        capi.check(capi.load().mhip_contact_op_tier_stats(self._h, C.byref(it), C.byref(hot), C.byref(rn), C.byref(wk)))
        return dict(tiered_iterations=it.value, mean_hot_fraction=hot.value, renumberings=rn.value, wakeups=wk.value)

    def set_profiling(self, enable=True):
        capi.check(capi.load().mhip_contact_op_set_profiling(self._h, 1 if enable else 0))

    def get_profile(self):
        a, b, n = C.c_double(), C.c_double(), C.c_size_t()
        capi.check(capi.load().mhip_contact_op_get_profile(self._h, C.byref(a), C.byref(b), C.byref(n)))
        return a.value, b.value, int(n.value)


def _state(x0, state):
    if state is not None:
        return state
    x = x0.clone()
    return x, torch.empty_like(x), torch.empty_like(x), torch.empty_like(x)


def solve_cqpp(A, q, space, x0, cfg=None, state=None, fused=True):
    cfg = cfg or PGDConfig()
    x, g, x_tmp, g_tmp = _state(x0, state)
    res, sp, pc = capi.SolveResult(), _space(space), _cfg(cfg)
    lib = capi.load()
    if isinstance(A, ContactOperator):
        fn = lib.mhip_bbpgd_solve_contact if fused else lib.mhip_bbpgd_solve_contact_unfused
        capi.check(fn(A._h, _ptr(q), C.byref(sp), C.byref(pc), _ptr(x), _ptr(g), _ptr(x_tmp), _ptr(g_tmp),
                      C.byref(res), _stream()))
    else:
        n = q.shape[0]
        if A.dim() != 2 or A.shape[0] != n or A.shape[1] != n:
            raise ValueError("gemv: dimension mismatch A vs x")
        capi.check(lib.mhip_bbpgd_solve_dense(n, _ptr(A), _ptr(q), C.byref(sp), C.byref(pc), _ptr(x), _ptr(g),
                                              _ptr(x_tmp), _ptr(g_tmp), C.byref(res), _stream()))
    return x, g, SolveResult(int(res.num_iters), float(res.residual), bool(res.converged))


def solve_friction_contact(A, sep, mu, p0=None, cfg=None, method="bbpgd"):
    cfg = cfg or PGDConfig()
    c = sep.shape[0]
    p = torch.zeros((c, 3), dtype=torch.float64, device=sep.device) if p0 is None else p0.clone()
    g = torch.empty_like(p)
    res, pc = capi.SolveResult(), _cfg(cfg)
    if method not in ("bbpgd", "apgd"):
        raise ValueError("method must be 'bbpgd' or 'apgd'")
    fn = capi.load().mhip_bbpgd_solve_contact_friction if method == "bbpgd" else capi.load().mhip_apgd_solve_contact_friction
    capi.check(fn(A._h, _ptr(sep), float(mu), C.byref(pc), _ptr(p, cols=3), _ptr(g, cols=3), C.byref(res), _stream()))
    return p, g, SolveResult(int(res.num_iters), float(res.residual), bool(res.converged))


def surface_lever_arms(pairs, normal, ra, rb, radius):
    ri = radius[pairs[:, 0].long()][:, None]
    rj = radius[pairs[:, 1].long()][:, None]
    return (ra + ri * normal).contiguous(), (rb - rj * normal).contiguous()


def solve_small_cqpp_batch(A, q, space, x0, cfg=None):
    cfg = cfg or PGDConfig()
    b, n = q.shape
    if A.shape != (b, n, n):
        raise ValueError("A must be [batch, n, n]")
    x = x0.clone()
    g = torch.empty_like(x)
    it = torch.empty(b, dtype=torch.int32, device=q.device)
    res = torch.empty(b, dtype=torch.float64, device=q.device)
    conv = torch.empty(b, dtype=torch.int32, device=q.device)
    sp, pc = _space(space), _cfg(cfg)
    capi.check(capi.load().mhip_solve_small_cqpp_batch(b, n, _ptr(A), _ptr(q), C.byref(sp), C.byref(pc), _ptr(x),
                                                       _ptr(g), _ptr(it, torch.int32), _ptr(res),
                                                       _ptr(conv, torch.int32), _stream()))
    return x, g, it, res, conv.bool()


@dataclass
class CollisionResult:
    max_abs_projected_sep: float = 0.0
    ite_count: int = 0
    max_displacement: float = 0.0


def resolve_collisions(op, sep, lam, dt, max_allowable_overlap=1e-5, max_col_iterations=10000):
    lam_tmp, g, g_tmp = torch.empty_like(lam), torch.empty_like(lam), torch.empty_like(lam)
    res, spd = capi.SolveResult(), C.c_double(0.0)
    capi.check(capi.load().mhip_scrap_bbpgd_solve_contact(
        op._h, _ptr(sep), float(max_allowable_overlap), int(max_col_iterations), _ptr(lam), _ptr(lam_tmp), _ptr(g),
        _ptr(g_tmp), C.byref(res), C.byref(spd), _stream()))
    return lam, g, CollisionResult(float(res.residual), int(res.num_iters), float(spd.value) * float(dt))


def solve_lcp(A, q, x0, cfg=None, state=None, fused=True):
    return solve_cqpp(A, q, LCP_SPACE, x0, cfg, state, fused)


def morton_order(center, lo, cell_size):
    n = center.shape[0]
    perm = torch.empty(n, dtype=torch.int32, device=center.device)
    lop = (C.c_double * 3)(*[float(v) for v in lo])
    capi.check(capi.load().mhip_morton_order(n, _ptr(center, cols=3), lop, float(cell_size), _ptr(perm, torch.int32),
                                             _stream()))
    return perm


def curve_order(center, lo, hi, level, key_table):
    n = center.shape[0]
    perm = torch.empty(n, dtype=torch.int32, device=center.device)
    lop = (C.c_double * 3)(*[float(v) for v in lo])
    hip = (C.c_double * 3)(*[float(v) for v in hi])
    capi.check(capi.load().mhip_curve_order(n, _ptr(center, cols=3), lop, hip, int(level),
                                            _ptr(key_table.reshape(-1), torch.int32), _ptr(perm, torch.int32), _stream()))
    return perm


def curve_keys(center, lo, hi, level, key_table):
    n = center.shape[0]
    keys = torch.empty(n, dtype=torch.int32, device=center.device)
    lop = (C.c_double * 3)(*[float(v) for v in lo])
    hip = (C.c_double * 3)(*[float(v) for v in hi])
    capi.check(capi.load().mhip_curve_keys(n, _ptr(center, cols=3), lop, hip, int(level),
                                           _ptr(key_table.reshape(-1), torch.int32), _ptr(keys, torch.int32), _stream()))
    return keys


def hilbert_key_table(level):
    n = 1 << int(level)
    table = np.empty((n, n, n), dtype=np.int32)
    capi.check(capi.load().mhip_hilbert_key_table(int(level), C.c_void_p(table.ctypes.data)))
    return table


def sort_by_key(keys):
    perm = torch.empty(keys.shape[0], dtype=torch.int32, device=keys.device)
    capi.check(capi.load().mhip_sort_by_key_u64(keys.shape[0], _ptr(keys, torch.int64), _ptr(perm, torch.int32), _stream()))
    return perm


def select_contacts(sep, cutoff):
    kept = torch.empty(sep.shape[0], dtype=torch.int32, device=sep.device)
    cnt = C.c_size_t(0)
    capi.check(capi.load().mhip_select_contacts(sep.shape[0], _ptr(sep), float(cutoff), _ptr(kept, torch.int32),
                                                C.byref(cnt), _stream()))
    return kept[:int(cnt.value)]


def select_dividing(length, division_length):
    D = _finite_nonneg(division_length, "division_length")
    parent_of = torch.empty(length.shape[0], dtype=torch.int32, device=length.device)
    cnt = C.c_size_t(0)
    capi.check(capi.load().mhip_select_dividing(length.shape[0], _ptr(length, name="length"), D,
                                                _ptr(parent_of, torch.int32), C.byref(cnt), _stream()))
    nb = int(cnt.value)
    return parent_of[:nb], nb


def divide_grow_spherocylinders(n, parent_of, dt, growth_rate, center, quat, radius, length, box=None):
    dt = _finite_nonneg(dt, "dt")
# ... 462 lines not shown
```

Before: 8.346 timesteps/s.

## Add watched tier for inactive contacts evaluated with a cheap gap check

```diff
diff --git a/include/mundy_hip.h b/include/mundy_hip.h
--- a/include/mundy_hip.h
+++ b/include/mundy_hip.h
@@ -281,6 +281,7 @@
 int mhip_contact_op_set_tiering(mhip_contact_op_t handle, int mode);
 int mhip_contact_op_tier_stats(mhip_contact_op_t handle, size_t* tiered_iterations, double* mean_hot_fraction,
                                size_t* renumberings, size_t* wakeups);
+int mhip_contact_op_tier_watch_stats(mhip_contact_op_t handle, double* mean_watched_fraction, size_t* watched_wakeups);
 int mhip_contact_op_set_profiling(mhip_contact_op_t handle, int enable);
 int mhip_contact_op_get_profile(mhip_contact_op_t handle, double* body_ms, double* constraint_ms, size_t* iterations);
 int mhip_contact_op_body_velocity(mhip_contact_op_t handle, const double** velocity );
diff --git a/mundy_amd/capi.py b/mundy_amd/capi.py
--- a/mundy_amd/capi.py
+++ b/mundy_amd/capi.py
@@ -172,6 +172,7 @@
     "mhip_contact_op_set_profiling": [_vp, _i],
     "mhip_contact_op_set_tiering": [_vp, _i],
     "mhip_contact_op_tier_stats": [_vp, C.POINTER(_sz), C.POINTER(_d), C.POINTER(_sz), C.POINTER(_sz)],
+    "mhip_contact_op_tier_watch_stats": [_vp, C.POINTER(_d), C.POINTER(_sz)],
     "mhip_contact_op_set_work_mapping": [_vp, _i, _i],
     "mhip_bbpgd_stage_snapshot_active": [_vp, _vp],
     "mhip_contact_op_get_profile": [_vp, C.POINTER(_d), C.POINTER(_d), C.POINTER(_sz)],
diff --git a/mundy_amd/csrc/convex.hip b/mundy_amd/csrc/convex.hip
--- a/mundy_amd/csrc/convex.hip
+++ b/mundy_amd/csrc/convex.hip
@@ -842,7 +842,62 @@
   const int32_t* fired;
   double* fire_at;
   unsigned blocks;
+  size_t A = ~static_cast<size_t>(0);
+  unsigned char* woken = nullptr;
 };
+
+template <int KIN, bool NT>
+__device__ __forceinline__ void tier_watch(const OpView& op, const double* __restrict__ vel, double* __restrict__ xn,
+                                           const double* __restrict__ q, const Space& sp, int resid_kind,
+                                           const TierCheck& tc, size_t c, double& rmax, DD& den) {
+  if (rmax < 0.0) rmax = 0.0;
+  if (tc.woken[c]) return;
+  const int2 ij = ld_s<NT>(op.pairs + c);
+  const V3 n = ld_s3<NT>(op.normal, c);
+  double arc_i = 0.0, arc_j = 0.0;
+  V3 arm_i{0.0, 0.0, 0.0}, arm_j{0.0, 0.0, 0.0};
+  if (KIN == KIN_ROD) {
+    arc_i = ld_s<NT>(op.arc_s + c);
+    arc_j = ld_s<NT>(op.arc_t + c);
+  }
+  if (KIN == KIN_RIGID) {
+    arm_i = ld_s3<NT>(op.ra, c);
+    arm_j = ld_s3<NT>(op.rb, c);
+  }
+  const double qc = ld_s<NT>(q + c);
+  const double2* vi2 = reinterpret_cast<const double2*>(vel + 6 * (size_t)ij.x);
+  const double2* vj2 = reinterpret_cast<const double2*>(vel + 6 * (size_t)ij.y);
+  const double2 a0 = vi2[0], a1 = vi2[1], b0 = vj2[0], b1 = vj2[1];
+  double2 a2 = make_double2(0.0, 0.0), b2 = make_double2(0.0, 0.0);
+  if (KIN != KIN_TRANS) {
+    a2 = vi2[2];
+    b2 = vj2[2];
+  }
+  V3 vi{a0.x, a0.y, a1.x}, vj{b0.x, b0.y, b1.x};
+  if (KIN == KIN_RIGID) {
+    vi = vi + cross(V3{a1.y, a2.x, a2.y}, arm_i);
+    vj = vj + cross(V3{b1.y, b2.x, b2.y}, arm_j);
+  }
+  if (KIN == KIN_ROD) {
+    const double ci = rod_arm_coef(arc_i), cj = rod_arm_coef(arc_j);
+    vi = vi + ci * V3{a1.y, a2.x, a2.y};
+    vj = vj + cj * V3{b1.y, b2.x, b2.y};
+  }
+  const double sdot = -n.x * (vi.x - vj.x) - n.y * (vi.y - vj.y) - n.z * (vi.z - vj.z);
+  const double y = op.dt * sdot;
+  const double g = 1.0 * qc + 1.0 * y;
+  if (g >= 0.0 && g <= 1.7976931348623157e308) return;
+  reinterpret_cast<double2*>(xn)[c] = make_double2(0.0, g);
+  const unsigned pi = op.pos[2 * c], pj = op.pos[2 * c + 1];
+  if (pi < 64u) atomicXor(&op.body_mask[ij.x], 1ull << pi);
+  if (pj < 64u) atomicXor(&op.body_mask[ij.y], 1ull << pj);
+  tc.woken[c] = 1;
+  tc.list[atomicAdd(&tc.counters[0], 1ull)] = static_cast<int32_t>(c);
+  atomicAdd(&tc.counters[3], 1ull);
+  const double r = residual_term(resid_kind, 0.0, g, sp);
+  if (r > rmax) rmax = r;
+  dd_add(den, 0.0 * (g - g));
+}
 
 template <int KIN>
 __device__ __forceinline__ void tier_evaluate(const OpView& op, const double* __restrict__ vel,
@@ -994,6 +1049,12 @@
     const size_t c = op.c_first + xcd_tile(lin, ntiles, op.xcd_aware) * kBlock + threadIdx.x;
     if (c >= op.c_end) continue;
     constexpr bool NTC = (MHIP_NT & 2) != 0 && MODE == X_SOLVE && PACKED;
+    if (MODE == X_SOLVE && PACKED) {
+      if (c - threadIdx.x >= check.A) {
+        tier_watch<KIN, NTC>(op, vel, xn, q, sp, resid_kind, check, c, rmax, den);
+        continue;
+      }
+    }
     const int2 ij = ld_s<NTC>(op.pairs + c);
     const double2 pold = iterate_load<MODE, PACKED, NTC>(c, xt, gt);
     const V3 n = ld_s3<NTC>(op.normal, c);
@@ -2077,13 +2138,15 @@
     double* saved_vel = nullptr;
     int set = 0;
     size_t H = 0;
+    size_t A = 0;
     size_t I = 0;
     bool pingpong = false;
     DeviceBuffer geo[2], iter[2], misc, vel2, drift, arm, xprev;
     OpView saved{};
-    size_t tiered_iterations = 0, retiers = 0, wakeups = 0;
+    size_t tiered_iterations = 0, retiers = 0, wakeups = 0, watched_wakeups = 0;
     unsigned service_blocks = 32;
     double hot_sum = 0.0;
+    double watch_sum = 0.0;
   } tier;
   bool profile = false;
   std::vector<hipEvent_t> events;
@@ -2267,13 +2330,15 @@
 }
 struct TierMisc {
   int32_t *flags, *rank, *new_of, *list, *fired;
+  int32_t *wflags, *wrank;
+  unsigned char* woken;
   double* wake[2];
   double *budget, *drift_prev, *fire_at;
   unsigned long long* counters;
 };
 inline size_t tier_misc_bytes(size_t C, size_t N) {
-  return 4 * tier_align((C + 2) * 4) + tier_align((N + 2) * 4) + 2 * tier_align((2 * C + 4) * 8) +
-         3 * tier_align((N + 2) * 8) + 256;
+  return 6 * tier_align((C + 2) * 4) + tier_align((N + 2) * 4) + 2 * tier_align((2 * C + 4) * 8) +
+         3 * tier_align((N + 2) * 8) + tier_align(C + 2) + 256;
 }
 inline TierMisc tier_misc_at(void* base, size_t C, size_t N) {
   char* p = static_cast<char*>(base);
@@ -2288,7 +2353,10 @@
   m.budget = reinterpret_cast<double*>(p); p += tier_align((N + 2) * 8);
   m.drift_prev = reinterpret_cast<double*>(p); p += tier_align((N + 2) * 8);
   m.fire_at = reinterpret_cast<double*>(p); p += tier_align((N + 2) * 8);
-  m.counters = reinterpret_cast<unsigned long long*>(p);
+  m.counters = reinterpret_cast<unsigned long long*>(p); p += 256;
+  m.wflags = reinterpret_cast<int32_t*>(p); p += tier_align((C + 2) * 4);
+  m.wrank = reinterpret_cast<int32_t*>(p); p += tier_align((C + 2) * 4);
+  m.woken = reinterpret_cast<unsigned char*>(p);
   return m;
 }
 
@@ -2317,24 +2385,29 @@
     k_tier_classify(size_t C, const int2* __restrict__ pairs, const double2* __restrict__ Pcur,
                     const double2* __restrict__ Pprev, const double* __restrict__ budget,
                     const double* __restrict__ drift, const double* __restrict__ wake_old, size_t H_old,
-                    int32_t* __restrict__ flags) {
+                    int32_t* __restrict__ flags, int32_t* __restrict__ wflags) {
   for (size_t c = blockIdx.x * (size_t)blockDim.x + threadIdx.x; c < C; c += (size_t)gridDim.x * blockDim.x) {
     const int2 ij = pairs[c];
     const double need_i = budget[ij.x], need_j = budget[ij.y];
-    bool cold;
+    bool cold, inactive;
     if (c >= H_old && wake_old[2 * (c - H_old)] > -1.7976931348623157e308) {
       cold = wake_old[2 * (c - H_old)] - drift[ij.x] > need_i && wake_old[2 * (c - H_old) + 1] - drift[ij.y] > need_j;
+      inactive = true;
     } else {
       const double2 a = Pcur[c], b = Pprev[c];
+      inactive = a.x == 0.0 && b.x == 0.0 && a.y >= 0.0 && a.y <= 1.7976931348623157e308;
       cold = a.x == 0.0 && b.x == 0.0 && a.y > kTierMinGap && a.y <= 1.7976931348623157e308 && kTierShare * a.y > need_i &&
              kTierShare * a.y > need_j;
     }
-    flags[c] = cold ? 0 : 1;
+    const bool watched = wflags != nullptr && !cold && inactive;
+    flags[c] = (cold || watched) ? 0 : 1;
+    if (wflags) wflags[c] = watched ? 1 : 0;
   }
 }
 template <int KIN>
 __global__ void __launch_bounds__(kBlock)
-    k_tier_permute(size_t C, size_t I, size_t H, int cur_is_p1, const int2* __restrict__ pairs, const double* __restrict__ normal,
+    k_tier_permute(size_t C, size_t I, size_t H, size_t A, size_t A_raw, const int32_t* __restrict__ wflags,
+                   const int32_t* __restrict__ wrank, int cur_is_p1, const int2* __restrict__ pairs, const double* __restrict__ normal,
                    const double* __restrict__ arc_s, const double* __restrict__ arc_t, const double* __restrict__ ra,
                    const double* __restrict__ rb, const double* __restrict__ q, const int32_t* __restrict__ orig,
                    const unsigned char* __restrict__ pos, TierGeo dst,
@@ -2344,9 +2417,11 @@
                    double* __restrict__ wake_new, const double* __restrict__ drift, double* __restrict__ fire_at) {
   for (size_t c = blockIdx.x * (size_t)blockDim.x + threadIdx.x; c < C; c += (size_t)gridDim.x * blockDim.x) {
     const bool fixed = c >= I;
-    const bool hot = fixed || flags[c] != 0;
+    const bool watched = !fixed && wflags != nullptr && wflags[c] != 0;
     const size_t r = fixed ? 0 : static_cast<size_t>(rank[c]);
-    const size_t nc = fixed ? c : (hot ? r : H + (c - r));
+    const size_t w = (fixed || wflags == nullptr) ? 0 : static_cast<size_t>(wrank[c]);
+    const size_t nc = fixed ? c : (watched ? A_raw + w : (flags[c] != 0 ? r : H + (c - r - w)));
+    const bool hot = fixed || nc < A;
     new_of[c] = static_cast<int32_t>(nc);
     const int2 ij = pairs[c];
     dst.pairs[nc] = ij;
@@ -2364,7 +2439,10 @@
     dst.pos[2 * nc] = pos[2 * c];
     dst.pos[2 * nc + 1] = pos[2 * c + 1];
     double2 a0 = P0s[c], a1 = P1s[c];
-    if (!hot) {
+    if (!hot && nc < H) {
+      const double g = cur_is_p1 ? a1.y : a0.y;
+      a0 = a1 = make_double2(0.0, g);
+    } else if (!hot) {
       const bool asleep = c >= H_old && wake_old[2 * (c - H_old)] > -1.7976931348623157e308;
       double ti, tj;
       if (asleep) {
@@ -2394,13 +2472,22 @@
 }
 template <int KIN>
 __global__ void __launch_bounds__(kBlock)
-    k_tier_refresh_sleepers(OpView op , size_t H, size_t I, int cur_is_1, const double* __restrict__ vcur,
-                            const double* __restrict__ vprev, const double* __restrict__ q,
-                            const double* __restrict__ wake, double2* __restrict__ P0, double2* __restrict__ P1) {
+    k_tier_refresh_sleepers(OpView op , size_t first, size_t H, size_t I, int cur_is_1,
+                            const double* __restrict__ vcur, const double* __restrict__ vprev,
+                            const double* __restrict__ q, const double* __restrict__ wake,
+                            const unsigned char* __restrict__ woken, double2* __restrict__ P0,
+                            double2* __restrict__ P1) {
   double2* Pcur = cur_is_1 ? P1 : P0;
   double2* Pprev = cur_is_1 ? P0 : P1;
-  for (size_t c = H + blockIdx.x * (size_t)blockDim.x + threadIdx.x; c < I; c += (size_t)gridDim.x * blockDim.x) {
-    if (!(wake[2 * (c - H)] > -1.7976931348623157e308)) continue;
+  for (size_t c = first + blockIdx.x * (size_t)blockDim.x + threadIdx.x; c < I; c += (size_t)gridDim.x * blockDim.x) {
+    if (c < H) {
+      if (woken[c]) {
+        if (Pprev[c].x == 0.0) Pprev[c].y = 1.0 * q[c] + 1.0 * contact_dt_sdot<KIN>(op, vprev, c, op.pairs[c]);
+        continue;
+      }
+    } else if (!(wake[2 * (c - H)] > -1.7976931348623157e308)) {
+      continue;
+    }
     const int2 ij = op.pairs[c];
     Pcur[c] = make_double2(0.0, 1.0 * q[c] + 1.0 * contact_dt_sdot<KIN>(op, vcur, c, ij));
     Pprev[c] = make_double2(0.0, 1.0 * q[c] + 1.0 * contact_dt_sdot<KIN>(op, vprev, c, ij));
@@ -2443,6 +2530,12 @@
   return (v.C >= kTierMinContacts || op->tiering >= 2) && v.body_mask != nullptr && v.counted == nullptr &&
          v.body_first == 0 && v.body_count == v.N && tier_problem_kind(sp, resid_kind);
 }
+
+double tier_watch_weight(int kin) { return kin == KIN_ROD ? 56.0 / 88.0 : (kin == KIN_RIGID ? 88.0 / 120.0 : 40.0 / 72.0); }
+double tier_swept(const mhip_contact_op* op, size_t A, size_t H) {
+  return static_cast<double>(A) + tier_watch_weight(op->kin) * static_cast<double>(H - A);
+}
+constexpr unsigned kTierWatchFrom = 24;
 
 unsigned tier_service_blocks(size_t awake) {
   const size_t want = kTierFireBlocks + 8 * (awake / (8 * 2 * kBlock));
@@ -2498,26 +2591,46 @@
   const double* wake_old = t.active ? m.wake[t.set] : m.wake[0];
   const size_t H_old = t.active ? t.H : C;
   if (I == 0) return MHIP_SUCCESS;
+  const bool watch = t.pingpong;
+  if (t.active && t.A < t.H) {
+    with_kin(op, [&](auto kin) {
+      k_tier_refresh_sleepers<decltype(kin)::value><<<grid_for(t.H - t.A), kBlock, 0, s>>>(
+          v, t.A, t.H, t.H, cur_is_p1 ? 1 : 0, cur_is_p1 ? v.vel_alt : v.vel, cur_is_p1 ? v.vel : v.vel_alt, cur.q,
+          m.wake[t.set], m.woken, reinterpret_cast<double2*>(cur.P0), reinterpret_cast<double2*>(cur.P1));
+    });
+    MHIP_LAUNCH_CHECK();
+  }
   k_tier_classify<<<grid_for(I), kBlock, 0, s>>>(I, v.pairs, Pc, Pp, m.budget, t.drift.as<double>(), wake_old, H_old,
-                                                 m.flags);
+                                                 m.flags, watch ? m.wflags : nullptr);
   MHIP_LAUNCH_CHECK();
   if (int e = exclusive_scan_i32(m.flags, m.rank, I, op->scanws.ptr, s)) return e;
-  int32_t H32 = 0;
-  unsigned long long awake = 0;
-  MHIP_HIP(hipMemcpyAsync(&H32, m.rank + I, sizeof(int32_t), hipMemcpyDeviceToHost, s));
-  if (t.active) MHIP_HIP(hipMemcpyAsync(&awake, m.counters, sizeof(awake), hipMemcpyDeviceToHost, s));
+  if (watch)
+    if (int e = exclusive_scan_i32(m.wflags, m.wrank, I, op->scanws.ptr, s)) return e;
+  int32_t A32 = 0, W32 = 0;
+  unsigned long long counters[4] = {0, 0, 0, 0};
+  MHIP_HIP(hipMemcpyAsync(&A32, m.rank + I, sizeof(int32_t), hipMemcpyDeviceToHost, s));
+  if (watch) MHIP_HIP(hipMemcpyAsync(&W32, m.wrank + I, sizeof(int32_t), hipMemcpyDeviceToHost, s));
+  if (t.active) MHIP_HIP(hipMemcpyAsync(counters, m.counters, sizeof(counters), hipMemcpyDeviceToHost, s));
   MHIP_HIP(hipStreamSynchronize(s));
-  const size_t H = static_cast<size_t>(H32);
+  const unsigned long long awake = counters[0];
+  const size_t A_raw = static_cast<size_t>(A32);
+  const size_t H = A_raw + static_cast<size_t>(W32);
+  const size_t A = watch ? (((A_raw + kBlock - 1) / kBlock * kBlock < H) ? (A_raw + kBlock - 1) / kBlock * kBlock : H) : H;
 #ifdef MHIP_TIER_DEBUG
   fprintf(stderr, "compact active entries at the last snapshot but one: %d of %zu half edges\n",
           *reinterpret_cast<const int32_t*>(op->host_state + 1), 2 * C);
   fprintf(stderr, "tier_update: iter %u last_period %u next %u scale %.2f  H %zu of I %zu (%.3f)  active %d awake %llu\n",
           iters_done, last_period, next_period, scale, H, I, (double)H / (double)I, (int)t.active, awake);
+  fprintf(stderr, "tier_update: iterated A %zu (%zu before rounding)  watched %zu  asleep %zu  watched wake-ups since the last renumbering %llu\n",
+          A, A_raw, H - A, I - H, counters[3]);
 #endif
   if (t.active) {
     t.service_blocks = tier_service_blocks(static_cast<size_t>(awake));
-    if (100 * H >= (100 - MHIP_TIER_RETIER_PERCENT) * (t.H + static_cast<size_t>(awake))) return MHIP_SUCCESS;
-  } else if (10 * H > 9 * I) {
+    if (100.0 * tier_swept(op, A, H) >=
+        (100 - MHIP_TIER_RETIER_PERCENT) * (tier_swept(op, t.A, t.H) + static_cast<double>(awake)))
+      return MHIP_SUCCESS;
+  } else if (10 * H > 9 * I &&
+             (iters_done < kTierWatchFrom || 10.0 * tier_swept(op, A, H) > 9.0 * static_cast<double>(I))) {
     return MHIP_SUCCESS;
   }
   const int dst_set = t.active ? (t.set ^ 1) : 0;
@@ -2534,7 +2647,7 @@
   if (int e = mhip_fill(N, m.fire_at, __builtin_huge_val(), reinterpret_cast<mhip_stream_t>(s))) return e;
   with_kin(op, [&](auto kin) {
     k_tier_permute<decltype(kin)::value><<<grid_for(C), kBlock, 0, s>>>(
-        C, I, H, cur_is_p1 ? 1 : 0, v.pairs, v.normal, v.arc_s, v.arc_t, v.ra, v.rb, cur.q, orig_src, v.pos, dst,
+        C, I, H, A, A_raw, watch ? m.wflags : nullptr, watch ? m.wrank : nullptr, cur_is_p1 ? 1 : 0, v.pairs, v.normal, v.arc_s, v.arc_t, v.ra, v.rb, cur.q, orig_src, v.pos, dst,
         reinterpret_cast<const double2*>(cur.P0), reinterpret_cast<const double2*>(cur.P1), P0d, P1d, m.flags, m.rank,
         m.new_of, wake_old, H_old, m.wake[dst_set], t.drift.as<double>(), m.fire_at);
   });
@@ -2542,6 +2655,7 @@
   k_tier_remap_inc<<<grid_for(2 * C), kBlock, 0, s>>>(2 * C, op->inc.as<int32_t>(), m.new_of);
   MHIP_LAUNCH_CHECK();
   MHIP_HIP(hipMemsetAsync(m.counters, 0, 4 * sizeof(unsigned long long), s));
+  if (watch) MHIP_HIP(hipMemsetAsync(m.woken, 0, C, s));
   v.pairs = dst.pairs;
   v.normal = dst.normal;
   v.arc_s = dst.arc_s;
@@ -2558,10 +2672,12 @@
   cur.P1 = reinterpret_cast<double*>(P1d);
   cur.q = dst.q;
   t.wakeups += static_cast<size_t>(awake);
+  t.watched_wakeups += static_cast<size_t>(counters[3]);
   t.active = true;
   t.service_blocks = kTierFireBlocks;
   t.set = dst_set;
   t.H = H;
+  t.A = A;
   t.I = I;
   t.retiers += 1;
   return MHIP_SUCCESS;
@@ -2591,7 +2707,7 @@
   const SolverState* st = op->state.as<SolverState>();
   double2* T0 = reinterpret_cast<double2*>(cur.P0);
   double2* T1 = reinterpret_cast<double2*>(cur.P1);
-  if (t.H < t.I) {
+  if (t.A < t.I) {
     const SolverState& hs = *op->host_state;
     const bool conv = hs.converged && !hs.converged_at_init;
     const unsigned cur1 = conv ? ((hs.flips + 1u) & 1u) : (hs.flips & 1u);
@@ -2623,10 +2739,10 @@
       vcur = v.vel;
       vprev = rows;
     }
-    const unsigned grid = grid_for(t.I - t.H);
+    const unsigned grid = grid_for(t.I - t.A);
     with_kin(op, [&](auto kin) {
-      k_tier_refresh_sleepers<decltype(kin)::value>
-          <<<grid, kBlock, 0, s>>>(v, t.H, t.I, static_cast<int>(cur1), vcur, vprev, cur.q, m.wake[t.set], T0, T1);
+      k_tier_refresh_sleepers<decltype(kin)::value><<<grid, kBlock, 0, s>>>(
+          v, t.A, t.H, t.I, static_cast<int>(cur1), vcur, vprev, cur.q, m.wake[t.set], m.woken, T0, T1);
     });
     MHIP_LAUNCH_CHECK();
   }
@@ -2638,10 +2754,11 @@
   MHIP_LAUNCH_CHECK();
   k_tier_remap_inc<<<grid_for(2 * C), kBlock, 0, s>>>(2 * C, op->inc.as<int32_t>(), geo.orig);
   MHIP_LAUNCH_CHECK();
-  unsigned long long awake = 0;
-  MHIP_HIP(hipMemcpyAsync(&awake, m.counters, sizeof(awake), hipMemcpyDeviceToHost, s));
+  unsigned long long counters[4] = {0, 0, 0, 0};
+  MHIP_HIP(hipMemcpyAsync(counters, m.counters, sizeof(counters), hipMemcpyDeviceToHost, s));
   MHIP_HIP(hipStreamSynchronize(s));
-  t.wakeups += static_cast<size_t>(awake);
+  t.wakeups += static_cast<size_t>(counters[0]);
+  t.watched_wakeups += static_cast<size_t>(counters[3]);
   const OpView keep = v;
   v = t.saved;
   v.xcd_aware = keep.xcd_aware;
@@ -2666,10 +2783,10 @@
   double* parts = op->partials.as<double>();
   const TierMisc m = tier_misc_at(t.misc.ptr, C, N);
   const unsigned ghot = t.H ? constraint_grid(t.H) : 0u;
-  const unsigned gcheck = t.H < t.I ? t.service_blocks : 0u;
+  const unsigned gcheck = t.A < t.I ? t.service_blocks : 0u;
   OpView hot = op->view;
   hot.c_first = 0; hot.c_end = t.H; hot.part_offset = 0; hot.part_stride = kStageStride;
-  const TierCheck tc{t.H, t.I, m.wake[t.set], m.list, m.counters, m.fired, m.fire_at, gcheck};
+  const TierCheck tc{t.H, t.I, m.wake[t.set], m.list, m.counters, m.fired, m.fire_at, gcheck, t.A, m.woken};
   if (ghot + gcheck) {
     with_kin(op, [&](auto kin) {
       k_constraint<X_SOLVE, decltype(kin)::value, true><<<ghot + gcheck, kBlock, 0, s>>>(
@@ -3339,8 +3456,8 @@
   }
   mhip_contact_op::Tier& tier = op->tier;
   tier.disabled = !tier_eligible(op, sp, rk) || op->tiering == 0;
-  tier.tiered_iterations = tier.retiers = tier.wakeups = 0;
-  tier.hot_sum = 0.0;
+  tier.tiered_iterations = tier.retiers = tier.wakeups = tier.watched_wakeups = 0;
+  tier.hot_sum = tier.watch_sum = 0.0;
   TierPairs cur{P0, P1, q};
   struct TierGuard {
     mhip_contact_op* op;
@@ -3383,7 +3500,8 @@
       unsigned ran = op->host_state->iter - iter_before + ((op->host_state->converged && op->host_state->iter < config->max_iters) ? 1u : 0u);
       if (ran > last_todo) ran = last_todo;
       tier.tiered_iterations += ran;
-      tier.hot_sum += ran * (static_cast<double>(tier.H) / static_cast<double>(C));
+      tier.hot_sum += ran * (tier_swept(op, tier.A, tier.H) / static_cast<double>(C));
+      tier.watch_sum += ran * (static_cast<double>(tier.H - tier.A) / static_cast<double>(C));
     }
     if (op->host_state->done == 2) {
       if (int e = tier_release(op, cur, false, P0, P1, q, nullptr, nullptr, nullptr, nullptr, s)) return e;
@@ -3467,6 +3585,15 @@
   if (mean_hot_fraction) *mean_hot_fraction = t.tiered_iterations ? t.hot_sum / static_cast<double>(t.tiered_iterations) : 0.0;
   if (renumberings) *renumberings = t.retiers;
   if (wakeups) *wakeups = t.wakeups;
+  return MHIP_SUCCESS;
+}
+
+int mhip_contact_op_tier_watch_stats(mhip_contact_op_t op, double* mean_watched_fraction, size_t* watched_wakeups) {
+  MHIP_REQUIRE(op != nullptr, MHIP_ERR_INVALID_ARGUMENT, "operator handle is null");
+  const mhip_contact_op::Tier& t = op->tier;
+  if (mean_watched_fraction)
+    *mean_watched_fraction = t.tiered_iterations ? t.watch_sum / static_cast<double>(t.tiered_iterations) : 0.0;
+  if (watched_wakeups) *watched_wakeups = t.watched_wakeups;
   return MHIP_SUCCESS;
 }
 
@@ -3695,8 +3822,8 @@
   tier.active = tier.tracking = false;
   tier.disabled = !op->stage.pause_on_bad_step || op->view.body_mask == nullptr ||
                   !(C >= kTierMinContacts || op->tiering >= 2);
-  tier.tiered_iterations = tier.retiers = tier.wakeups = 0;
-  tier.hot_sum = 0.0;
+  tier.tiered_iterations = tier.retiers = tier.wakeups = tier.watched_wakeups = 0;
+  tier.hot_sum = tier.watch_sum = 0.0;
   return MHIP_SUCCESS;
 }
 
diff --git a/mundy_amd/ops.py b/mundy_amd/ops.py
--- a/mundy_amd/ops.py
+++ b/mundy_amd/ops.py
@@ -703,6 +703,11 @@
         it, rn, wk, hot = C.c_size_t(0), C.c_size_t(0), C.c_size_t(0), C.c_double(0.0)
         capi.check(capi.load().mhip_contact_op_tier_stats(self._h, C.byref(it), C.byref(hot), C.byref(rn), C.byref(wk)))
         return dict(tiered_iterations=it.value, mean_hot_fraction=hot.value, renumberings=rn.value, wakeups=wk.value)
+
+    def tier_watch_stats(self):
+        frac, wk = C.c_double(0.0), C.c_size_t(0)
+        capi.check(capi.load().mhip_contact_op_tier_watch_stats(self._h, C.byref(frac), C.byref(wk)))
+        return dict(mean_watched_fraction=frac.value, watched_wakeups=wk.value)
 
     def set_profiling(self, enable=True):
         capi.check(capi.load().mhip_contact_op_set_profiling(self._h, 1 if enable else 0))
```

New measurement: 7.914 timesteps/s. 5.2% lower.
